# dylandreimerink/mimic

Measured on AMD Instinct MI355X. Metric: Mpkts/s (device-resident, one XDP program over 64-1500B batches), higher is better.
Workload: dtype u64; 1 GPU; cfg2: 1M x 64B xdp_md, 36-slot parse+hash DROP/PASS classifier, per-CPU array E=4 S=8; packets_per_gpu=1048576, vcpus_per_gpu=262144, schedule=interleaved, parallelism=dp1, batches_rotated=8, working_set_bytes=713031680, program_slots=36, engine=spread_own, batches_per_launch=8

## Files before the change

include/mimic_amd.h:

```cpp
#ifndef MIMIC_AMD_H
#define MIMIC_AMD_H

#if !defined(__HIPCC_RTC__)
#include <stddef.h>
#include <stdint.h>
#endif

#ifdef __cplusplus
extern "C" {
#endif

#define MIMIC_ABI_VERSION 4

#define MIMIC_EINVAL (-1)
#define MIMIC_ENOMEM (-2)
#define MIMIC_EDEVICE (-3)
#define MIMIC_ENOTSUP (-4)
#define MIMIC_ENOENT (-5)
#define MIMIC_EFAULT (-6)
#define MIMIC_ECANCELED (-7)
#define MIMIC_EDEADLINE (-8)

enum mimic_status {
    MIMIC_OK = 0,
// ... 79 lines not shown
    const uint32_t *pkt_len;
    const uint32_t *headroom;  uint32_t headroom_all;
    const uint32_t *tailroom;  uint32_t tailroom_all;
    const int32_t *ingress_ifindex; int32_t ingress_all;
    const int32_t *rx_queue_index;  int32_t rxq_all;
    const int32_t *egress_ifindex;  int32_t egress_all;
    const int32_t *cpu;
    uint64_t step_budget;
} mimic_xdp_batch;

typedef struct {
    uint64_t *r0;
    uint8_t *status;
    uint32_t *steps;
    int32_t *err_pc;
} mimic_xdp_results;

int mimic_abi_version(void);
const char *mimic_last_error(const mimic_vm *vm);

int mimic_vm_create(const mimic_vm_settings *settings, mimic_vm **out);
void mimic_vm_destroy(mimic_vm *vm);

int mimic_map_create(mimic_vm *vm, const mimic_map_spec *spec, uint32_t *map_id);
int mimic_map_update(mimic_vm *vm, uint32_t map_id, const void *key, const void *value, uint32_t flags, int32_t cpu);
int mimic_map_update_batch(mimic_vm *vm, uint32_t map_id, const void *keys, const void *values, uint32_t n,
                           uint32_t flags, int32_t cpu, int32_t *rc_out);
int mimic_map_lookup(mimic_vm *vm, uint32_t map_id, const void *key, int32_t cpu, uint32_t *addr_out);
int mimic_map_delete(mimic_vm *vm, uint32_t map_id, const void *key);
int mimic_map_keys(mimic_vm *vm, uint32_t map_id, void *out, size_t cap, uint32_t *n_out);
int mimic_map_entries(mimic_vm *vm, uint32_t map_id, void *keys_out, int32_t *slots_out, size_t cap_entries,
                      uint32_t *n_out);
int mimic_map_read_values(mimic_vm *vm, uint32_t map_id, int32_t cpu, void *out, size_t cap);
int mimic_map_reset(mimic_vm *vm, uint32_t map_id, void *hip_stream);
int mimic_map_read_values_range(mimic_vm *vm, uint32_t map_id, int32_t cpu_begin, int32_t cpu_end, void *out,
                                size_t cap);
int mimic_map_sum_u64(mimic_vm *vm, uint32_t map_id, int32_t cpu_begin, int32_t cpu_end, uint64_t *out, size_t cap);
int mimic_map_share(mimic_vm *vm, uint32_t map_id, mimic_vm *owner, uint32_t owner_map_id);
int mimic_map_addr(mimic_vm *vm, uint32_t map_id, uint32_t *addr_out);

int mimic_program_load(mimic_vm *vm, const char *name, const void *insns, uint32_t n_slots,
                       const mimic_reloc *relocs, uint32_t n_relocs, uint32_t *prog_id);
int mimic_program_addr(mimic_vm *vm, uint32_t prog_id, uint32_t *addr_out);

int mimic_mem_read(mimic_vm *vm, uint32_t addr, void *buf, uint32_t len);
int mimic_mem_load(mimic_vm *vm, uint32_t addr, int32_t size, uint64_t *out);
int mimic_stack_addr(mimic_vm *vm, uint32_t *addr_out);

int mimic_run_xdp(mimic_vm *vm, uint32_t prog_id, const mimic_xdp_batch *batch,
                  const mimic_xdp_results *results, void *hip_stream);
int mimic_run_xdp_many(mimic_vm *vm, uint32_t prog_id, const mimic_xdp_batch *batches,
                       const mimic_xdp_results *results, uint32_t k, void *hip_stream);
#define MIMIC_CTX_XDP 0
#define MIMIC_CTX_SKB 1
#define MIMIC_SKB_CUSTOM_SK 1u
#define MIMIC_SKB_CUSTOM_FLOWKEYS 2u
typedef struct {
    uint32_t flags;
    uint32_t sk_bound_dev_if, sk_family, sk_type, sk_protocol, sk_mark, sk_priority;
    uint32_t sk_src_port, sk_dst_port, sk_state;
    int32_t sk_rx_queue_mapping;
    uint8_t sk_ip_len[4];
    uint8_t sk_ip[4][16];
    uint16_t fk_nhoff, fk_thoff, fk_addr_proto;
    uint8_t fk_is_frag, fk_is_first_frag, fk_is_encap, fk_ip_proto;
    uint16_t fk_n_proto, fk_sport, fk_dport;
    uint32_t fk_flags, fk_flow_label;
} mimic_skb_custom;

typedef struct {
    uint32_t n;
    uint32_t schedule;
    uint8_t *pkt_data;
    const uint64_t *pkt_off;
    const uint32_t *pkt_len;
    uint32_t ifindex;
    int32_t pad;
    const int32_t *cpu;
    uint64_t step_budget;
    const mimic_skb_custom *custom;
    uint32_t *rooms_state;
} mimic_skb_batch;

int mimic_run_skb(mimic_vm *vm, uint32_t prog_id, const mimic_skb_batch *batch,
                  const mimic_xdp_results *results, void *hip_stream);
int mimic_skb_release(mimic_vm *vm);

typedef struct mimic_process mimic_process;
typedef struct {
    uint64_t r[11];
    int32_t pc;
    uint32_t prog_id;
    uint64_t steps;
    int32_t status;
    uint32_t exited;
} mimic_process_regs;
int mimic_process_new(mimic_vm *vm, uint32_t prog_id, const void *packet, uint32_t len, uint32_t headroom,
                      uint32_t tailroom, int32_t ingress_ifindex, int32_t rx_queue_index, int32_t egress_ifindex,
                      mimic_process **out);
int mimic_process_new_skb(mimic_vm *vm, uint32_t prog_id, const void *packet, uint32_t len, uint32_t ifindex,
                          mimic_process **out);
int mimic_process_new_skb_ctx(mimic_vm *vm, uint32_t prog_id, const void *packet, uint32_t len, uint32_t ifindex,
                              const mimic_skb_custom *custom, mimic_process **out);
int mimic_process_set_cpu(mimic_process *p, int32_t id);
int mimic_process_step(mimic_process *p, uint32_t n, mimic_process_regs *out);
int mimic_process_run(mimic_process *p, uint64_t budget, mimic_process_regs *out);
typedef struct mimic_ctx mimic_ctx;
int mimic_ctx_new(uint64_t timeout_ns, mimic_ctx **out);
void mimic_ctx_cancel(mimic_ctx *c);
int mimic_ctx_err(const mimic_ctx *c);
int mimic_ctx_pinned(const mimic_ctx *c);
void mimic_ctx_free(mimic_ctx *c);
int mimic_run_xdp_ctx(mimic_vm *vm, uint32_t prog_id, const mimic_xdp_batch *batch, const mimic_xdp_results *results,
                      void *hip_stream, mimic_ctx *ctx, mimic_ctx *const *ctx_per_packet);
int mimic_run_skb_ctx(mimic_vm *vm, uint32_t prog_id, const mimic_skb_batch *batch, const mimic_xdp_results *results,
                      void *hip_stream, mimic_ctx *ctx, mimic_ctx *const *ctx_per_packet);
int mimic_process_run_ctx(mimic_process *p, uint64_t budget, mimic_ctx *ctx, mimic_process_regs *out);
int mimic_process_run_many(mimic_process *const *ps, uint32_t n, const int32_t *cpus, mimic_ctx *const *ctxs,
                           mimic_process_regs *out);
void mimic_process_free_many(mimic_process *const *ps, uint32_t n);

int mimic_process_packet(mimic_process *p, void *buf, size_t cap);
void mimic_process_free(mimic_process *p);

int mimic_sync(mimic_vm *vm, void *hip_stream);
int mimic_last_steps(mimic_vm *vm, uint64_t *steps_out);

typedef struct {
    uint32_t n;
    uint32_t schedule;
    const uint8_t *pkt_data;
    const uint64_t *pkt_off;
    const uint32_t *pkt_len;
    uint32_t headroom_all, tailroom_all;
    int32_t ingress_all, rxq_all, egress_all;
    int32_t pad;
    const int32_t *cpu;
    uint64_t step_budget;
    uint8_t *pkt_out;
    uint64_t *r0;
    uint8_t *status;
} mimic_xdp_host_batch;
int mimic_run_xdp_host(mimic_vm *vm, uint32_t prog_id, const mimic_xdp_host_batch *hb, uint32_t chunks);
int mimic_run_xdp_host_ctx(mimic_vm *vm, uint32_t prog_id, const mimic_xdp_host_batch *hb, uint32_t chunks,
                           mimic_ctx *ctx);
int mimic_run_xdp_host_ctx_pp(mimic_vm *vm, uint32_t prog_id, const mimic_xdp_host_batch *hb, uint32_t chunks,
                              mimic_ctx *const *ctx_per_packet);
int mimic_host_register(void *p, size_t bytes);
int mimic_host_unregister(void *p);

int mimic_exec_mode(const mimic_vm *vm);
int mimic_set_spread(mimic_vm *vm, int32_t mode);
int mimic_last_exec(const mimic_vm *vm);
long mimic_jit_source_for(const void *const *progs, const uint32_t *n_slots, uint32_t n_progs, char *buf, size_t cap);
int mimic_jit_check(const char *src, char *log, size_t cap, size_t *code_size);
int mimic_jit_prebuild(const void *const *progs, const uint32_t *n_slots, uint32_t n_progs);
long mimic_jit_source_for_ctx(const void *const *progs, const uint32_t *n_slots, uint32_t n_progs, int32_t ctx_kind,
                              char *buf, size_t cap);
int mimic_jit_prebuild_ctx(const void *const *progs, const uint32_t *n_slots, uint32_t n_progs, int32_t ctx_kind);
long mimic_jit_source_vc(const void *const *progs, const uint32_t *n_slots, uint32_t n_progs, int32_t ctx_kind,
                         const uint32_t *vc_slots, uint32_t n_vc, char *buf, size_t cap);
long mimic_jit_source_spread(const void *const *progs, const uint32_t *n_slots, uint32_t n_progs, const uint32_t *pc,
                             uint32_t n_pc, const uint32_t *shapes, uint32_t n_shapes, uint32_t lds_rows,
                             int32_t *spread_out, char *buf, size_t cap);
int mimic_jit_cache_source(const char *src);
int mimic_jit_code(const char *src, void *code, size_t cap, size_t *code_size);

#ifdef __cplusplus
}
#endif
#endif
```

mimic_amd/_lib.py:

```python
from __future__ import annotations

import ctypes as C
import os

_HERE = os.path.dirname(os.path.abspath(__file__))
LIB_PATH = os.path.join(_HERE, os.path.basename(os.environ.get("MIMIC_LIB", "libmimic_amd.so")))

ABI_VERSION = 4

STATUS_NAMES = [
    "OK", "ERR_PC_OOB", "ERR_UNSUPPORTED_OP", "ERR_MEM_UNRESOLVED", "ERR_MEM_NOT_VMMEM",
    "ERR_MEM_BOUNDS", "ERR_MEM_NOT_DATASEC", "ERR_R10_WRITE", "ERR_HELPER_MAP_PTR",
    "ERR_HELPER_KEY", "ERR_HELPER_VALUE", "ERR_HELPER_MAP_OP", "ERR_HELPER_TAILCALL",
    "ERR_HELPER_UNIMPLEMENTED", "ERR_HELPER_CANT_EMULATE", "ERR_LDABS", "PANIC_DIV0",
    "PANIC_SHIFT", "PANIC_BADREG", "PANIC_CALLX", "PANIC_PC", "PANIC_HELPER_NEG",
    "ERR_STEP_LIMIT", "ERR_CALL_DEPTH", "ERR_ENGINE_HELPER", "ERR_NO_CPU", "ERR_CTX_ACCESS", "PANIC_SLICE",
    "ERR_CTX_LOAD", "ERR_CANCELED", "ERR_DEADLINE", "ERR_ENGINE_STATE",
]
STATUS = {n: i for i, n in enumerate(STATUS_NAMES)}
ECANCELED, EDEADLINE = -7, -8

SCHED_CHUNKED, SCHED_INTERLEAVED, SCHED_EXPLICIT = 0, 1, 2
MAP_F_DATASEC = 1


class VMSettings(C.Structure):
    _fields_ = [("vcpus", C.c_int32), ("stack_frame_size", C.c_int32), ("stack_frame_count", C.c_int32),
                ("max_tail_calls", C.c_int32), ("device", C.c_int32), ("vcpu_begin", C.c_int32),
                ("vcpu_count", C.c_int32), ("exec_mode", C.c_int32)]


class MapSpecC(C.Structure):
    _fields_ = [("name", C.c_char_p), ("type", C.c_uint32), ("key_size", C.c_uint32),
                ("value_size", C.c_uint32), ("max_entries", C.c_uint32), ("flags", C.c_uint32)]


class ProcessRegs(C.Structure):
    _fields_ = [("r", C.c_uint64 * 11), ("pc", C.c_int32), ("prog_id", C.c_uint32), ("steps", C.c_uint64),
                ("status", C.c_int32), ("exited", C.c_uint32)]


class Reloc(C.Structure):
    _fields_ = [("slot", C.c_uint32), ("map_id", C.c_uint32)]


class XDPBatch(C.Structure):
    _fields_ = [("n", C.c_uint32), ("schedule", C.c_uint32), ("pkt_data", C.c_void_p),
                ("pkt_off", C.c_void_p), ("pkt_len", C.c_void_p),
                ("headroom", C.c_void_p), ("headroom_all", C.c_uint32),
                ("tailroom", C.c_void_p), ("tailroom_all", C.c_uint32),
                ("ingress_ifindex", C.c_void_p), ("ingress_all", C.c_int32),
                ("rx_queue_index", C.c_void_p), ("rxq_all", C.c_int32),
                ("egress_ifindex", C.c_void_p), ("egress_all", C.c_int32),
                ("cpu", C.c_void_p), ("step_budget", C.c_uint64)]


class SKBBatch(C.Structure):
    _fields_ = [("n", C.c_uint32), ("schedule", C.c_uint32), ("pkt_data", C.c_void_p),
                ("pkt_off", C.c_void_p), ("pkt_len", C.c_void_p), ("ifindex", C.c_uint32), ("pad", C.c_int32),
                ("cpu", C.c_void_p), ("step_budget", C.c_uint64), ("custom", C.c_void_p), ("rooms_state", C.c_void_p)]


SKB_CUSTOM_SK, SKB_CUSTOM_FLOWKEYS = 1, 2
try:
    import numpy as _np

    SKB_CUSTOM_DTYPE = _np.dtype([
        ("flags", "<u4"), ("sk_bound_dev_if", "<u4"), ("sk_family", "<u4"), ("sk_type", "<u4"), ("sk_protocol", "<u4"),
        ("sk_mark", "<u4"), ("sk_priority", "<u4"), ("sk_src_port", "<u4"), ("sk_dst_port", "<u4"), ("sk_state", "<u4"),
        ("sk_rx_queue_mapping", "<i4"), ("sk_ip_len", "u1", (4,)), ("sk_ip", "u1", (4, 16)),
        ("fk_nhoff", "<u2"), ("fk_thoff", "<u2"), ("fk_addr_proto", "<u2"), ("fk_is_frag", "u1"),
        ("fk_is_first_frag", "u1"), ("fk_is_encap", "u1"), ("fk_ip_proto", "u1"), ("fk_n_proto", "<u2"),
        ("fk_sport", "<u2"), ("fk_dport", "<u2"), ("fk_flags", "<u4"), ("fk_flow_label", "<u4")])
    assert SKB_CUSTOM_DTYPE.itemsize == 136
except ImportError:
    SKB_CUSTOM_DTYPE = None


CTX_XDP, CTX_SKB = 0, 1


class XDPResults(C.Structure):
    _fields_ = [("r0", C.c_void_p), ("status", C.c_void_p), ("steps", C.c_void_p), ("err_pc", C.c_void_p)]


class XDPHostBatch(C.Structure):
    _fields_ = [("n", C.c_uint32), ("schedule", C.c_uint32), ("pkt_data", C.c_void_p),
                ("pkt_off", C.c_void_p), ("pkt_len", C.c_void_p),
                ("headroom_all", C.c_uint32), ("tailroom_all", C.c_uint32),
                ("ingress_all", C.c_int32), ("rxq_all", C.c_int32), ("egress_all", C.c_int32), ("pad", C.c_int32),
                ("cpu", C.c_void_p), ("step_budget", C.c_uint64), ("pkt_out", C.c_void_p),
                ("r0", C.c_void_p), ("status", C.c_void_p)]


EXPORTS = {
    "mimic_abi_version": (C.c_int, []),
    "mimic_last_error": (C.c_char_p, [C.c_void_p]),
    "mimic_vm_create": (C.c_int, [C.POINTER(VMSettings), C.POINTER(C.c_void_p)]),
    "mimic_vm_destroy": (None, [C.c_void_p]),
    "mimic_map_create": (C.c_int, [C.c_void_p, C.POINTER(MapSpecC), C.POINTER(C.c_uint32)]),
    "mimic_map_update": (C.c_int, [C.c_void_p, C.c_uint32, C.c_void_p, C.c_void_p, C.c_uint32, C.c_int32]),
    "mimic_map_lookup": (C.c_int, [C.c_void_p, C.c_uint32, C.c_void_p, C.c_int32, C.POINTER(C.c_uint32)]),
    "mimic_map_update_batch": (C.c_int, [C.c_void_p, C.c_uint32, C.c_void_p, C.c_void_p, C.c_uint32, C.c_uint32,
                                         C.c_int32, C.c_void_p]),
    "mimic_map_delete": (C.c_int, [C.c_void_p, C.c_uint32, C.c_void_p]),
    "mimic_exec_mode": (C.c_int, [C.c_void_p]),
    "mimic_set_spread": (C.c_int, [C.c_void_p, C.c_int32]),
    "mimic_process_new_skb_ctx": (C.c_int, [C.c_void_p, C.c_uint32, C.c_char_p, C.c_uint32, C.c_uint32, C.c_void_p,
                                            C.POINTER(C.c_void_p)]),
    "mimic_run_xdp_host": (C.c_int, [C.c_void_p, C.c_uint32, C.POINTER(XDPHostBatch), C.c_uint32]),
    "mimic_host_register": (C.c_int, [C.c_void_p, C.c_size_t]),
    "mimic_host_unregister": (C.c_int, [C.c_void_p]),
    "mimic_last_exec": (C.c_int, [C.c_void_p]),
    "mimic_jit_source_for": (C.c_long, [C.POINTER(C.c_void_p), C.POINTER(C.c_uint32), C.c_uint32, C.c_char_p,
                                         C.c_size_t]),
    "mimic_jit_check": (C.c_int, [C.c_char_p, C.c_char_p, C.c_size_t, C.POINTER(C.c_size_t)]),
    "mimic_jit_prebuild": (C.c_int, [C.POINTER(C.c_void_p), C.POINTER(C.c_uint32), C.c_uint32]),
    "mimic_map_keys": (C.c_int, [C.c_void_p, C.c_uint32, C.c_void_p, C.c_size_t, C.POINTER(C.c_uint32)]),
    "mimic_map_entries": (C.c_int, [C.c_void_p, C.c_uint32, C.c_void_p, C.c_void_p, C.c_size_t,
                                    C.POINTER(C.c_uint32)]),
    "mimic_map_read_values": (C.c_int, [C.c_void_p, C.c_uint32, C.c_int32, C.c_void_p, C.c_size_t]),
    "mimic_map_reset": (C.c_int, [C.c_void_p, C.c_uint32, C.c_void_p]),
    "mimic_map_read_values_range": (C.c_int, [C.c_void_p, C.c_uint32, C.c_int32, C.c_int32, C.c_void_p, C.c_size_t]),
    "mimic_map_sum_u64": (C.c_int, [C.c_void_p, C.c_uint32, C.c_int32, C.c_int32, C.c_void_p, C.c_size_t]),
    "mimic_map_addr": (C.c_int, [C.c_void_p, C.c_uint32, C.POINTER(C.c_uint32)]),
    "mimic_program_load": (C.c_int, [C.c_void_p, C.c_char_p, C.c_void_p, C.c_uint32, C.POINTER(Reloc),
                                     C.c_uint32, C.POINTER(C.c_uint32)]),
    "mimic_program_addr": (C.c_int, [C.c_void_p, C.c_uint32, C.POINTER(C.c_uint32)]),
    "mimic_mem_read": (C.c_int, [C.c_void_p, C.c_uint32, C.c_void_p, C.c_uint32]),
    "mimic_mem_load": (C.c_int, [C.c_void_p, C.c_uint32, C.c_int32, C.POINTER(C.c_uint64)]),
    "mimic_stack_addr": (C.c_int, [C.c_void_p, C.POINTER(C.c_uint32)]),
    "mimic_run_xdp": (C.c_int, [C.c_void_p, C.c_uint32, C.POINTER(XDPBatch), C.POINTER(XDPResults), C.c_void_p]),
    "mimic_run_xdp_many": (C.c_int, [C.c_void_p, C.c_uint32, C.POINTER(XDPBatch), C.POINTER(XDPResults), C.c_uint32,
                                     C.c_void_p]),
    "mimic_map_share": (C.c_int, [C.c_void_p, C.c_uint32, C.c_void_p, C.c_uint32]),
    "mimic_run_skb": (C.c_int, [C.c_void_p, C.c_uint32, C.POINTER(SKBBatch), C.POINTER(XDPResults), C.c_void_p]),
    "mimic_skb_release": (C.c_int, [C.c_void_p]),
    "mimic_jit_source_for_ctx": (C.c_long, [C.POINTER(C.c_void_p), C.POINTER(C.c_uint32), C.c_uint32, C.c_int32,
                                             C.c_char_p, C.c_size_t]),
    "mimic_jit_source_vc": (C.c_long, [C.POINTER(C.c_void_p), C.POINTER(C.c_uint32), C.c_uint32, C.c_int32,
                                       C.POINTER(C.c_uint32), C.c_uint32, C.c_char_p, C.c_size_t]),
    "mimic_jit_source_spread": (C.c_long, [C.POINTER(C.c_void_p), C.POINTER(C.c_uint32), C.c_uint32,
                                           C.POINTER(C.c_uint32), C.c_uint32, C.POINTER(C.c_uint32), C.c_uint32,
                                           C.c_uint32, C.POINTER(C.c_int32), C.c_char_p, C.c_size_t]),
    "mimic_jit_prebuild_ctx": (C.c_int, [C.POINTER(C.c_void_p), C.POINTER(C.c_uint32), C.c_uint32, C.c_int32]),
    "mimic_jit_cache_source": (C.c_int, [C.c_char_p]),
    "mimic_process_new": (C.c_int, [C.c_void_p, C.c_uint32, C.c_char_p, C.c_uint32, C.c_uint32, C.c_uint32,
                                    C.c_int32, C.c_int32, C.c_int32, C.POINTER(C.c_void_p)]),
    "mimic_process_new_skb": (C.c_int, [C.c_void_p, C.c_uint32, C.c_char_p, C.c_uint32, C.c_uint32, C.c_void_p]),
    "mimic_process_set_cpu": (C.c_int, [C.c_void_p, C.c_int32]),
    "mimic_process_step": (C.c_int, [C.c_void_p, C.c_uint32, C.c_void_p]),
    "mimic_process_run": (C.c_int, [C.c_void_p, C.c_uint64, C.c_void_p]),
    "mimic_process_packet": (C.c_int, [C.c_void_p, C.c_void_p, C.c_size_t]),
    "mimic_process_free": (None, [C.c_void_p]),
    "mimic_jit_code": (C.c_int, [C.c_char_p, C.c_void_p, C.c_size_t, C.POINTER(C.c_size_t)]),
    "mimic_sync": (C.c_int, [C.c_void_p, C.c_void_p]),
    "mimic_ctx_new": (C.c_int, [C.c_uint64, C.POINTER(C.c_void_p)]),
    "mimic_ctx_cancel": (None, [C.c_void_p]),
    "mimic_ctx_err": (C.c_int, [C.c_void_p]),
    "mimic_ctx_pinned": (C.c_int, [C.c_void_p]),
    "mimic_ctx_free": (None, [C.c_void_p]),
    "mimic_run_xdp_ctx": (C.c_int, [C.c_void_p, C.c_uint32, C.POINTER(XDPBatch), C.POINTER(XDPResults), C.c_void_p,
                                    C.c_void_p, C.c_void_p]),
    "mimic_run_skb_ctx": (C.c_int, [C.c_void_p, C.c_uint32, C.POINTER(SKBBatch), C.POINTER(XDPResults), C.c_void_p,
                                    C.c_void_p, C.c_void_p]),
    "mimic_process_run_ctx": (C.c_int, [C.c_void_p, C.c_uint64, C.c_void_p, C.POINTER(ProcessRegs)]),
    "mimic_process_run_many": (C.c_int, [C.c_void_p, C.c_uint32, C.c_void_p, C.c_void_p, C.POINTER(ProcessRegs)]),
    "mimic_process_free_many": (None, [C.c_void_p, C.c_uint32]),
    "mimic_run_xdp_host_ctx": (C.c_int, [C.c_void_p, C.c_uint32, C.POINTER(XDPHostBatch), C.c_uint32, C.c_void_p]),
    "mimic_run_xdp_host_ctx_pp": (C.c_int, [C.c_void_p, C.c_uint32, C.POINTER(XDPHostBatch), C.c_uint32, C.c_void_p]),
    "mimic_last_steps": (C.c_int, [C.c_void_p, C.POINTER(C.c_uint64)]),
}

_lib = None


def load() -> C.CDLL:
    global _lib
    if _lib is not None:
        return _lib
    if not os.path.exists(LIB_PATH):
        raise ImportError(f"{LIB_PATH} is missing: run __graft_entry__.build() (hipcc --offload-arch=gfx950)")
    try:
        import torch
    except ImportError:
        pass
    lib = C.CDLL(LIB_PATH)
    for name, (res, args) in EXPORTS.items():
        fn = getattr(lib, name)
        fn.restype = res
        fn.argtypes = args
    if lib.mimic_abi_version() != ABI_VERSION:
        raise ImportError("libmimic_amd.so ABI version mismatch")
    _lib = lib
    return lib
```

mimic_amd/csrc/engine.cpp:

```cpp
#include <hip/hip_runtime.h>

#include <algorithm>
#include <atomic>
#include <cstdarg>
#include <cstdlib>
#include <cstdio>
#include <cstring>
#include <map>
#include <string>
#include <chrono>
#include <condition_variable>
#include <memory>
#include <mutex>
#include <thread>
#include <unordered_map>
#include <vector>

#include "../../include/mimic_amd.h"
#include "blkcache.h"
#include "layout.h"
#include "hashmap.h"
#include "jit.h"
#include "skb.h"

extern "C" int mimic_launch_xdp(const KParams *kp, const KParams *d_kp, hipStream_t st);
extern "C" int mimic_launch_xdp_resume(const KParams *kp, hipStream_t st);

extern "C" int mimic_launch_hash_rebuild(uint8_t *arena, const DMap *m, uint32_t force, hipStream_t st);
extern "C" int mimic_launch_hash_reset(uint8_t *arena, const DMap *m, hipStream_t st);
extern "C" int mimic_launch_hash_normalize(uint8_t *arena, const DMap *m, hipStream_t st);
extern "C" int mimic_launch_hash_compact(uint8_t *arena, const DMap *m, hipStream_t st);
extern "C" int mimic_launch_spread_reduce(const void *part, uint32_t nblocks, uint32_t lanes, uint32_t roww, uint32_t n,
                                          uint8_t *dst, uint64_t stride, hipStream_t st);
extern "C" int mimic_launch_sum_u64(const uint8_t *base, uint64_t stride, uint32_t nvals, uint32_t cpus, uint64_t *out,
                                    hipStream_t st);
extern "C" int mimic_launch_skb_gather(const uint8_t *const *mem, uint32_t n, uint64_t *drv, uint64_t *prefix,
                                       mimic_skb_custom *cust, const uint8_t *has_cust, hipStream_t st);
extern "C" int mimic_launch_skb_prep(const uint8_t *pkt_data, const uint64_t *pkt_off, const uint32_t *pkt_len,
                                     uint32_t n, uint64_t *rec, uint32_t rec_q, uint64_t *prefix, uint64_t *state,
                                     uint64_t init_base, uint32_t use_init, uint32_t *rooms_state, hipStream_t st);

namespace {

#define MIRROR_PAGE 8192u
#define MIRROR_BULK 32u
struct HashMirror {
    bool valid = false, dirty = false;
    std::vector<uint64_t> rec;
    std::vector<int32_t> ring;
    HashCtl ctl{};
    std::vector<uint8_t> rec_pg, ring_pg;
    bool all = true;
    uint32_t faults = 0;
};

struct ShareGroup {
    struct Member {
        void *vm;
        uint32_t map;
        uint8_t *arena;
    };
    std::vector<Member> members;
    bool owner_gone = false;
};

struct HostMap {
    std::string name;
    uint32_t type, family, key_size, value_size, max_entries, datasec;
    uint32_t obj_addr;
    uint32_t backing_addr;
    uint32_t addr_period;
    uint32_t ncpu;
    uint64_t dev_off;
    uint64_t dev_stride;
    uint64_t keys_dev_off, ht_dev_off;
    uint32_t keys_addr, ht_cap, rec_q, nlocks, fl_cap;
    mutable bool may_tomb = false;
    mutable bool pop_dirty = false;
    std::shared_ptr<HashMirror> mir;
    mutable std::shared_ptr<ShareGroup> share;
    mutable bool chunk = false;
};

bool vc_row_ok(uint32_t family, uint32_t max_entries, uint32_t value_size) {
    const uint64_t rb = (uint64_t)max_entries * value_size;
    return family == FAM_PERCPU_ARRAY && rb > 0 && rb <= MIMIC_VC_MAX_ROW && (rb & 7) == 0;
}

struct HostProg {
    std::string name;
    std::vector<DInsn> ins;
    uint32_t addr;
};

struct HipFence : BlkFence {
    hipEvent_t ev = nullptr;
    hipStream_t st = nullptr;
    void wait() override {
        if (hipEventSynchronize(ev) != hipSuccess) {
            (void)hipGetLastError();
            hipStreamSynchronize(st);
        }
    }
    ~HipFence() override {
        if (ev) hipEventDestroy(ev);
    }
};

}

struct mimic_vm {
    mimic_vm_settings s;
    std::string err;
    hipStream_t stream = nullptr;
    uint32_t next_addr = MIMIC_MEM_START;
    std::vector<HostMap> maps;
    std::vector<HostProg> progs;
    std::vector<Seg> segs;
    uint8_t *arena = nullptr;
    uint64_t arena_size = 0, arena_cap = 0;
    DInsn *d_insns = nullptr;
    DProg *d_progs = nullptr;
    Seg *d_segs = nullptr;
    DMap *d_maps = nullptr;
    bool tables_dirty = true;
    bool prog_deletes = false;
    bool prog_updates = false;
    uint8_t *priv = nullptr;
    uint64_t priv_bytes = 0;
    uint32_t priv_lanes = 0;
    uint32_t *d_sched_start = nullptr, *d_sched_pkts = nullptr;
    uint64_t sched_cap_start = 0, sched_cap_pkts = 0;
    uint64_t *d_lane_steps = nullptr;
    uint32_t lane_steps_cap = 0;
    DeferRec *d_defer = nullptr;
    uint32_t *d_defer_any = nullptr;
    uint32_t defer_cap = 0, defer_epoch = 0;
    uint32_t last_lanes = 0;
    hipStream_t last_stream = nullptr;
    int exec_mode = MIMIC_EXEC_JIT;
    std::vector<DInsn> h_all;
    std::vector<DProg> h_dp;
    hipFunction_t jit_fn[2] = {nullptr, nullptr};
    JitInfo jit_info[2]{};
    hipFunction_t jit_fn_cx[2] = {nullptr, nullptr};
    JitInfo jit_info_cx[2]{};
    int64_t proc_jit_after = 32;
    uint64_t proc_runs = 0;
    int proc_jit = 0;
    hipFunction_t jit_fn_proc = nullptr;
    JitInfo jit_info_proc{};
    int spread_state = 0;
    hipFunction_t jit_fn_spread = nullptr;
    JitInfo jit_info_spread{};
    int spread_own_state = 0;
    hipFunction_t jit_fn_spread_own = nullptr;
    JitInfo jit_info_spread_own{};
    uint32_t spread_own_rows = 0;
    uint32_t *d_spread_bad = nullptr;
    void *d_spread_part = nullptr;
    uint64_t spread_part_cap = 0;
    bool spread_used = false;
    bool comb_used = false;
    struct PendWrite {
        uint64_t off;
        uint32_t n, at;
    };
    std::vector<PendWrite> pend;
    std::vector<uint8_t> pend_data;
    std::unordered_map<uint64_t, size_t> pend_at;
    bool host_dirty = false;
    int spread_mode = -1;
    bool spread_lds = false;
    int last_exec = 0;
    static constexpr int KP_SLOTS = 64;
    KParams *d_kp = nullptr, *h_kp = nullptr;
    hipEvent_t kp_ev[KP_SLOTS] = {};
    bool kp_used[KP_SLOTS] = {};
    int kp_next = 0, kp_last = -1;
    hipStream_t kp_last_stream = nullptr;
    static constexpr int NB = 4;
    struct Slot {
        uint8_t *buf = nullptr;
        uint64_t *off = nullptr;
        uint32_t *len = nullptr;
        uint64_t *r0 = nullptr;
        uint8_t *st = nullptr;
        size_t cap_bytes = 0, cap_n = 0;
        hipEvent_t e_in = nullptr, e_k = nullptr, e_out = nullptr;
        bool used = false;
    } slot[NB];
    hipStream_t s_h2d = nullptr, s_h2d2 = nullptr, s_d2h = nullptr;
    hipStream_t kp_copy_stream = nullptr;
    hipEvent_t kp_copy_ev = nullptr;
    hipStream_t s_kp = nullptr;
    hipEvent_t kp_side_ev = nullptr;
    SkbRec *d_skb_rec = nullptr;
    uint64_t *d_skb_drv = nullptr;
    uint64_t *d_skb_prefix = nullptr, *d_skb_state = nullptr;
    size_t skb_cap = 0;
    uint8_t *d_many = nullptr;
    size_t many_cap = 0;
    BlkCache blk{256ull << 20};
    std::recursive_mutex run_mu;
    SeqClock seq;
    uint32_t proc_gen = 0;
    bool skb_leaked = false;
    hipStream_t skb_stream = nullptr;
    bool skb_release_pending = false;
    hipEvent_t skb_ev = nullptr;
    const uint32_t **d_cancel_pp = nullptr;
    size_t cancel_pp_cap = 0;
    hipStream_t cancel_pp_stream = nullptr;
};

struct mimic_ctx {
    uint32_t *word = nullptr;
    uint32_t *dword = nullptr;
    bool pinned = false;
    std::mutex mu;
    std::condition_variable cv;
    bool closing = false;
    std::thread timer;
    std::vector<hipEvent_t> uses;
};
static void ctx_set(mimic_ctx *c, uint32_t v) {
    uint32_t z = 0;
    __atomic_compare_exchange_n(c->word, &z, v, false, __ATOMIC_SEQ_CST, __ATOMIC_SEQ_CST);
}
static uint32_t ctx_get(const mimic_ctx *c) { return __atomic_load_n(c->word, __ATOMIC_SEQ_CST); }


static int fail(mimic_vm *vm, int code, const char *fmt, ...) {
    if (vm) {
        char buf[512];
        va_list ap;
        va_start(ap, fmt);
        vsnprintf(buf, sizeof buf, fmt, ap);
        va_end(ap);
        vm->err = buf;
    }
    return code;
}

#define HIP_OK(vm, call)                                                                        \
    do {                                                                                        \
        hipError_t e_ = (call);                                                                 \
        if (e_ != hipSuccess) return fail((vm), MIMIC_EDEVICE, "%s: %s", #call, hipGetErrorString(e_)); \
    } while (0)

static int skb_settle(mimic_vm *vm);

static int kp_slot(mimic_vm *vm, const KParams &kp, hipStream_t st, const KParams **out) {
    if (!vm->d_kp) {
        HIP_OK(vm, hipMalloc(&vm->d_kp, sizeof(KParams) * mimic_vm::KP_SLOTS));
        HIP_OK(vm, hipHostMalloc(&vm->h_kp, sizeof(KParams) * mimic_vm::KP_SLOTS));
        for (auto &e : vm->kp_ev) HIP_OK(vm, hipEventCreateWithFlags(&e, hipEventDisableTiming));
    }
    int slot = vm->kp_last;
    if (slot < 0 || st != vm->kp_last_stream || memcmp(&vm->h_kp[slot], &kp, sizeof kp) != 0) {
        slot = vm->kp_next;
        vm->kp_next = (slot + 1) % mimic_vm::KP_SLOTS;
        if (vm->kp_used[slot]) HIP_OK(vm, hipEventSynchronize(vm->kp_ev[slot]));
        vm->h_kp[slot] = kp;
        if (vm->kp_copy_stream) {
            HIP_OK(vm, hipMemcpyAsync(vm->d_kp + slot, vm->h_kp + slot, sizeof kp, hipMemcpyHostToDevice, vm->kp_copy_stream));
            HIP_OK(vm, hipEventRecord(vm->kp_copy_ev, vm->kp_copy_stream));
            HIP_OK(vm, hipStreamWaitEvent(st, vm->kp_copy_ev, 0));
        } else {
            if (!vm->s_kp) {
                HIP_OK(vm, hipStreamCreateWithFlags(&vm->s_kp, hipStreamNonBlocking));
                HIP_OK(vm, hipEventCreateWithFlags(&vm->kp_side_ev, hipEventDisableTiming));
            }
            HIP_OK(vm, hipMemcpyAsync(vm->d_kp + slot, vm->h_kp + slot, sizeof kp, hipMemcpyHostToDevice, vm->s_kp));
            HIP_OK(vm, hipEventRecord(vm->kp_side_ev, vm->s_kp));
            HIP_OK(vm, hipStreamWaitEvent(st, vm->kp_side_ev, 0));
        }
        vm->kp_last = slot;
        vm->kp_last_stream = st;
    }
    *out = vm->d_kp + slot;
    return slot;
}

static uint32_t stack_size(const mimic_vm *vm) {
    return (uint32_t)(vm->s.stack_frame_size * vm->s.stack_frame_count);
}

static uint32_t add_entry(mimic_vm *vm, uint32_t size) {
    uint32_t a = vm->next_addr;
    vm->next_addr = a + size + 1;
    return a;
}

static int arena_reserve(mimic_vm *vm, uint64_t bytes, uint64_t *off) {
    uint64_t need = (vm->arena_size + 255) & ~255ull;
    uint64_t end = need + bytes;
    if (end > vm->arena_cap) {
        uint64_t cap = std::max<uint64_t>(end, vm->arena_cap * 2);
        cap = std::max<uint64_t>(cap, 1 << 20);
        uint8_t *n = nullptr;
        HIP_OK(vm, hipMalloc(&n, cap));
        HIP_OK(vm, hipMemset(n, 0, cap));
        if (vm->arena) {
            HIP_OK(vm, hipMemcpy(n, vm->arena, vm->arena_size, hipMemcpyDeviceToDevice));
            HIP_OK(vm, hipFree(vm->arena));
        }
        vm->arena = n;
        vm->arena_cap = cap;
    }
    *off = need;
    vm->arena_size = end;
    return 0;
}

static int helper_class(int32_t n) {
    static const int ce[] = {4, 14, 15, 16, 17, 22, 24, 27, 35, 36, 42, 45, 46, 47, 55, 56, 67, 69, 80,
                             112, 113, 114, 115, 119, 120, 122, 123, 128, 129, 141, 148, 151};
    static const int em[] = {1, 2, 3, 5, 7, 8, 9, 12, 25, 38, 65, 87, 88, 89, 125, 160};
    for (int v : ce) if (v == n) return 2;
    for (int v : em) if (v == n) return 1;
    return 0;
}

static uint32_t predecode(const DInsn &x, int64_t i, int64_t n) {
    const uint32_t op = x.w & 0xff, dst = (x.w >> 8) & 0xf, src = (x.w >> 12) & 0xf;
    const int64_t off = (int16_t)(x.w >> 16);
// ... 1565 lines not shown
    kp.priv = step ? step->priv : vm->priv;
    kp.priv_xdp_q = xdp_q;
    kp.priv_frame_q = frame_q;
    kp.priv_key_q = key_q;
    kp.budget = step ? step->budget : (b->step_budget ? b->step_budget : MIMIC_DEFAULT_BUDGET);
    kp.step = step ? step->state : nullptr;
    kp.step_gen = step ? step->gen : 0u;
    if (step) {
        kp.step_img = step->img;
        kp.step_dst = step->img_dst;
        kp.step_img_n = step->img_n;
        kp.step_ins_n = (uint32_t)std::min<size_t>(vm->h_all.size(), 2048);
    }
    kp.n = b->n;
    kp.sched = b->schedule;
    kp.pkt_data = b->pkt_data;
    kp.pkt_off = b->pkt_off;
    kp.pkt_len = b->pkt_len;
    kp.headroom_arr = b->headroom;
    kp.tailroom_arr = b->tailroom;
    kp.ingress_arr = b->ingress_ifindex;
    kp.rxq_arr = b->rx_queue_index;
    kp.egress_arr = b->egress_ifindex;
    kp.headroom = b->headroom_all;
    kp.tailroom = b->tailroom_all;
    kp.ingress = b->ingress_all;
    kp.rxq = b->rxq_all;
    kp.egress = b->egress_all;
    kp.r0 = res->r0;
    kp.status = res->status;
    kp.steps = res->steps;
    kp.err_pc = res->err_pc;
    kp.lane_steps = vm->d_lane_steps;
    if (cx && cx->all) {
        kp.cancel = cx->all->dword;
        kp.cancel_any = 1;
    } else if (cx && cx->dev_pp && b->n) {
        kp.cancel_pp = cx->dev_pp;
        kp.cancel_any = 1;
    } else if (cx && cx->per_packet && b->n) {
        std::vector<const uint32_t *> w(b->n);
        bool any = false;
        for (uint32_t i = 0; i < b->n; i++) {
            w[i] = cx->per_packet[i] ? cx->per_packet[i]->dword : nullptr;
            any |= w[i] != nullptr;
        }
        if (any) {
            if (vm->cancel_pp_stream) hipStreamSynchronize(vm->cancel_pp_stream);
            hipStreamSynchronize(st);
            vm->cancel_pp_stream = st;
            if (b->n > vm->cancel_pp_cap) {
                hipFree(vm->d_cancel_pp);
                vm->d_cancel_pp = nullptr;
                HIP_OK(vm, hipMalloc(&vm->d_cancel_pp, (size_t)b->n * sizeof(void *)));
                vm->cancel_pp_cap = b->n;
            }
            HIP_OK(vm, hipMemcpy(vm->d_cancel_pp, w.data(), (size_t)b->n * sizeof(void *), hipMemcpyHostToDevice));
            kp.cancel_pp = vm->d_cancel_pp;
            kp.cancel_any = 1;
        }
    }
    switch (b->schedule) {
    case MIMIC_SCHED_CHUNKED:
        kp.per_lane = lanes ? (uint32_t)(((uint64_t)b->n + lanes - 1) / lanes) : 0;
        break;
    case MIMIC_SCHED_INTERLEAVED:
        kp.sched_shift = lanes ? (uint32_t)(first_index % lanes) : 0;
        kp.per_lane = lanes ? (uint32_t)(((uint64_t)b->n + kp.sched_shift + lanes - 1) / lanes) : 0;
        break;
    case MIMIC_SCHED_EXPLICIT: {
        if (!b->cpu && b->n) return fail(vm, MIMIC_EINVAL, "explicit schedule needs cpu[]");
        std::vector<uint32_t> start(lanes + 1, 0), pk(b->n);
        std::vector<uint32_t> lane_of(b->n);
        for (uint32_t i = 0; i < b->n; i++) {
            const int32_t id = b->cpu[i];
            int64_t c = (int64_t)id - vm->s.vcpu_begin;
            if (id == -1) c = cpu_lanes;
            else if (id == vm->s.vcpus) c = cpu_lanes + 1;
            else if (c < 0 || c >= (int64_t)cpu_lanes)
                return fail(vm, MIMIC_EINVAL, "packet %u: cpu %d not on this engine", i, id);
            lane_of[i] = (uint32_t)c;
            start[c + 1]++;
        }
        uint32_t mx = 0;
        for (uint32_t c = 0; c < lanes; c++) {
            mx = std::max(mx, start[c + 1]);
            start[c + 1] += start[c];
        }
        std::vector<uint32_t> fill(start.begin(), start.end() - 1);
        for (uint32_t i = 0; i < b->n; i++) pk[fill[lane_of[i]]++] = i;
        hipStreamSynchronize(st);
        if (start.size() > vm->sched_cap_start) {
            hipFree(vm->d_sched_start);
            vm->d_sched_start = nullptr;
            HIP_OK(vm, hipMalloc(&vm->d_sched_start, start.size() * 4));
            vm->sched_cap_start = start.size();
        }
        if (pk.size() > vm->sched_cap_pkts || !vm->d_sched_pkts) {
            hipFree(vm->d_sched_pkts);
            vm->d_sched_pkts = nullptr;
            HIP_OK(vm, hipMalloc(&vm->d_sched_pkts, std::max<size_t>(pk.size(), 1) * 4));
            vm->sched_cap_pkts = std::max<size_t>(pk.size(), 1);
        }
        HIP_OK(vm, hipMemcpy(vm->d_sched_start, start.data(), start.size() * 4, hipMemcpyHostToDevice));
        if (!pk.empty()) HIP_OK(vm, hipMemcpy(vm->d_sched_pkts, pk.data(), pk.size() * 4, hipMemcpyHostToDevice));
        kp.sched_start = vm->d_sched_start;
        kp.sched_pkts = vm->d_sched_pkts;
        kp.per_lane = mx;
        break;
    }
    default:
        return fail(vm, MIMIC_EINVAL, "unknown schedule %u", b->schedule);
    }
    bool jit = vm->exec_mode == MIMIC_EXEC_JIT && (!step || proc_jit);
    if (jit && !proc_jit && !vm->jit_fn[ctx]) {
        std::string log;
        const std::vector<std::pair<uint32_t, uint32_t>> vc = vc_slots_of(vm);
        if (mimic_jit_compile(vm->s.device, mimic_jit_source(vm->h_dp, vm->h_all, ctx, &vm->jit_info[ctx], &vc),
                              &vm->jit_fn[ctx], &log))
            return fail(vm, MIMIC_EDEVICE, "JIT build failed: %s", log.c_str());
        const JitInfo &j0 = vm->jit_info[ctx];
        int ls0 = 0;
        if (j0.early_loads && j0.cold_inline &&
            hipFuncGetAttribute(&ls0, HIP_FUNC_ATTRIBUTE_LOCAL_SIZE_BYTES, vm->jit_fn[ctx]) == hipSuccess && ls0 > 0) {
            JitInfo j1;
            hipFunction_t f1 = nullptr;
            int ls1 = 0;
            if (!mimic_jit_compile(vm->s.device, mimic_jit_source(vm->h_dp, vm->h_all, ctx, &j1, &vc, true), &f1, &log) &&
                hipFuncGetAttribute(&ls1, HIP_FUNC_ATTRIBUTE_LOCAL_SIZE_BYTES, f1) == hipSuccess && ls1 < ls0) {
                vm->jit_fn[ctx] = f1;
                vm->jit_info[ctx] = j1;
            }
        }
    }
    if (jit && !proc_jit) {
        const uint64_t bound = mimic_jit_step_bound(vm->jit_info[ctx], kp.max_tail_calls);
        if (bound && kp.budget < bound) jit = false;
    }
    bool spread = false, own = false;
    if (jit && !step && !skb && b->n > 0 && (b->schedule == MIMIC_SCHED_CHUNKED || b->schedule == MIMIC_SCHED_INTERLEAVED)) {
        const char *sv = getenv("MIMIC_SPREAD");
        const int knob = vm->spread_mode >= 0 ? vm->spread_mode : sv && *sv ? atoi(sv) : -1;
        const char *ov = getenv("MIMIC_SPREAD_OWN");
        const bool own_pref = !(ov && ov[0] == '0');
        if (knob != 0 && own_pref && kp.per_lane >= 2 && kp.per_lane <= 256) {
            rc = spread_build_own(vm);
            if (rc) return rc;
            const uint32_t P = kp.per_lane, cl = chip_lanes(vm);
            const char *qv = getenv("MIMIC_SPREAD_OWN_Q");
            uint32_t q = qv && *qv ? (uint32_t)atoi(qv) : (uint32_t)std::max<uint64_t>(1, ((uint64_t)b->n + cl - 1) / cl);
            q = std::max<uint32_t>(1, std::min(q, P));
            while (q > 1 && (P % q || 256u * q / P > vm->spread_own_rows)) q--;
            kp.own_q = q;
            own = vm->spread_own_state > 0 && P % q == 0 && 256u * q / P <= vm->spread_own_rows && 256u * q / P >= 1u &&
                  mimic_jit_step_bound(vm->jit_info_spread_own, kp.max_tail_calls) <= kp.budget;
            spread = own;
        }
        if (!own && (knob == 1 || (knob != 0 && (uint64_t)b->n >= 8ull * cpu_lanes))) {
            rc = spread_build(vm);
            if (rc) return rc;
            spread = vm->spread_state > 0 && mimic_jit_step_bound(vm->jit_info_spread, kp.max_tail_calls) <= kp.budget;
            if (knob != 1 && !vm->spread_lds && cpu_lanes > 16384) spread = false;
        }
    }
    const bool cxk = jit && kp.cancel_any;
    if (cxk) {
        spread = own = false;
        if (!vm->jit_fn_cx[ctx]) {
            const std::vector<std::pair<uint32_t, uint32_t>> vc = vc_slots_of(vm);
            std::string log;
            if (mimic_jit_compile(vm->s.device,
                                  mimic_jit_source(vm->h_dp, vm->h_all, ctx, &vm->jit_info_cx[ctx], &vc,
                                                   !vm->jit_info[ctx].early_loads, nullptr, true),
                                  &vm->jit_fn_cx[ctx], &log))
                return fail(vm, MIMIC_EDEVICE, "JIT build failed: %s", log.c_str());
        }
    }
    const JitInfo &ji = proc_jit ? vm->jit_info_proc : own ? vm->jit_info_spread_own : spread ? vm->jit_info_spread
                        : cxk ? vm->jit_info_cx[ctx] : vm->jit_info[ctx];
    hipFunction_t jfn = proc_jit ? vm->jit_fn_proc : own ? vm->jit_fn_spread_own : spread ? vm->jit_fn_spread
                        : cxk ? vm->jit_fn_cx[ctx] : vm->jit_fn[ctx];
    if (proc_jit && (!jfn || !ji.proc_ok)) return fail(vm, MIMIC_EDEVICE, "process: no single-process JIT kernel (engine)");
    uint32_t run_lanes = lanes;
    if (spread) {
        const uint32_t orows = own ? 256u / (kp.per_lane / kp.own_q) : 1u;
        const uint32_t blocks = own ? (cpu_lanes + orows - 1) / orows
                                    : (uint32_t)(((uint64_t)b->n + spread_ppb() - 1) / spread_ppb());
        run_lanes = blocks * 256u;
        rc = priv_ensure(vm, q_per_lane, run_lanes, st);
        if (rc) return rc;
        if (run_lanes > vm->lane_steps_cap) {
            hipStreamSynchronize(st);
            hipFree(vm->d_lane_steps);
            vm->d_lane_steps = nullptr;
            HIP_OK(vm, hipMalloc(&vm->d_lane_steps, (uint64_t)run_lanes * sizeof(uint64_t)));
            vm->lane_steps_cap = run_lanes;
        }
        if (!vm->d_spread_bad) {
            HIP_OK(vm, hipMalloc(&vm->d_spread_bad, 64));
            HIP_OK(vm, hipMemset(vm->d_spread_bad, 0, 64));
        }
        kp.lanes = run_lanes;
        kp.priv = vm->priv;
        kp.priv_lanes = vm->priv_lanes;
        kp.lane_steps = vm->d_lane_steps;
        kp.spread_bad = vm->d_spread_bad;
        vm->spread_used = true;
        kp.spread_part = nullptr;
        if (!own && ji.spread_rows && ji.spread_rows == cpu_lanes && ji.spread_n &&
            (uint64_t)cpu_lanes * ji.spread_roww <= spread_ppb()) {
            const uint64_t need = (uint64_t)blocks * ji.spread_rows * ji.spread_roww * ji.spread_n;
            if (need > vm->spread_part_cap) {
                HIP_OK(vm, hipStreamSynchronize(st));
                hipFree(vm->d_spread_part);
                vm->d_spread_part = nullptr;
                HIP_OK(vm, hipMalloc(&vm->d_spread_part, need));
                vm->spread_part_cap = need;
            }
            kp.spread_part = vm->d_spread_part;
        }
    }
    if (skb && step && step->skb_rec) {
        kp.ctx_kind = CTX_SKB;
        kp.skb_ifindex = skb->ifindex;
        kp.skb_rec = step->skb_rec;
        kp.skb_prefix = step->skb_prefix;
        kp.skb_base = step->skb_base;
        kp.skb_custom = step->skb_custom;
    } else if (skb && skb->pre_drv) {
        rc = skb_ensure(vm, b->n, st);
        if (rc) return rc;
        kp.ctx_kind = CTX_SKB;
        kp.skb_ifindex = skb->ifindex;
        kp.skb_rec = vm->d_skb_rec;
        kp.skb_drv = skb->pre_drv;
        kp.skb_prefix = skb->pre_prefix;
        kp.skb_base = skb->pre_base;
        kp.skb_custom = skb->custom;
        vm->skb_stream = st;
    } else if (skb) {
        rc = skb_prepare(vm, b, st, nullptr, skb->rooms_state);
        if (rc) return rc;
        kp.skb_rooms_state = skb->rooms_state;
        kp.ctx_kind = CTX_SKB;
        kp.skb_ifindex = skb->ifindex;
        kp.skb_rec = vm->d_skb_rec;
        kp.skb_drv = vm->d_skb_drv;
        kp.skb_prefix = vm->d_skb_prefix;
        kp.skb_base = vm->d_skb_state + 1;
        kp.skb_custom = skb->custom;
    }
    kp.hash_pop_only = vm->prog_deletes ? 0u : 1u;
    kp.hash_ro = (vm->prog_deletes || vm->prog_updates) ? 0u : 1u;
    for (auto &m : vm->maps) {
        if (!is_hash(m)) continue;
        if (m.share) {
            if ((rc = share_check(vm, m))) return rc;
            for (auto &mb : m.share->members) {
                mimic_vm *o = (mimic_vm *)mb.vm;
                if (o != vm && o->host_dirty && (rc = flush_host(o))) return fail(vm, rc, "shared map: %s", o->err.c_str());
            }
            share_stale(m);
        }
        const DMap dm = to_dmap(m);
        if (vm->prog_deletes && m.pop_dirty) {
            if (mimic_launch_hash_normalize(vm->arena, &dm, st))
                return fail(vm, MIMIC_EDEVICE, "launch: %s", hipGetErrorString(hipGetLastError()));
            m.pop_dirty = false;
        }
        if (!vm->prog_deletes) m.pop_dirty = true;
        if (vm->prog_deletes) m.may_tomb = true;
        if (m.mir && (vm->prog_updates || vm->prog_deletes || m.may_tomb)) m.mir->valid = false;
        if (!m.may_tomb) continue;
        if (mimic_launch_hash_rebuild(vm->arena, &dm, 0, st))
            return fail(vm, MIMIC_EDEVICE, "launch: %s", hipGetErrorString(hipGetLastError()));
    }
    vm->last_exec = jit ? (own ? MIMIC_EXEC_SPREAD_OWN : spread ? MIMIC_EXEC_SPREAD : MIMIC_EXEC_JIT) : MIMIC_EXEC_INTERP;
    if (jit && ji.defer) {
        if (lanes > vm->defer_cap || !vm->d_defer_any) {
            hipStreamSynchronize(st);
            hipFree(vm->d_defer);
            vm->d_defer = nullptr;
            HIP_OK(vm, hipMalloc(&vm->d_defer, (uint64_t)plan * sizeof(DeferRec)));
            HIP_OK(vm, hipMemset(vm->d_defer, 0, (uint64_t)plan * sizeof(DeferRec)));
            vm->defer_cap = plan;
            if (!vm->d_defer_any) {
                HIP_OK(vm, hipMalloc(&vm->d_defer_any, 64));
                HIP_OK(vm, hipMemset(vm->d_defer_any, 0, 64));
            }
        }
        if (++vm->defer_epoch == 0) vm->defer_epoch = 1;
        kp.defer = vm->d_defer;
        kp.defer_any = vm->d_defer_any;
        kp.defer_epoch = vm->defer_epoch;
    }
    if (jit && ji.hash_combine) vm->comb_used = true;
    if (mr) {
        mr->used = jit && own && !ji.defer && mr->k >= 1 && mr->k <= MIMIC_MANY_MAX;
        if (mr->used) {
            kp.many_n = mr->k;
            for (uint32_t q = 0; q < mr->k; q++)
                kp.many[q] = BatchRef{mr->b[q].pkt_data, mr->b[q].pkt_off, mr->b[q].pkt_len, mr->r[q].r0, mr->r[q].status,
                                      mr->r[q].steps, mr->r[q].err_pc, 0};
        }
    }
    if (jit) {
        if (mimic_jit_launch(jfn, &kp, st))
            return fail(vm, MIMIC_EDEVICE, "launch: %s", hipGetErrorString(hipGetLastError()));
        if (ji.defer && mimic_launch_xdp_resume(&kp, st))
            return fail(vm, MIMIC_EDEVICE, "launch: %s", hipGetErrorString(hipGetLastError()));
    } else if (step) {
        if (mimic_launch_xdp(&kp, nullptr, st))
            return fail(vm, MIMIC_EDEVICE, "launch: %s", hipGetErrorString(hipGetLastError()));
    } else {
        const KParams *dkp = nullptr;
        const int slot = kp_slot(vm, kp, st, &dkp);
        if (slot < 0) return slot;
        if (mimic_launch_xdp(&kp, dkp, st))
            return fail(vm, MIMIC_EDEVICE, "launch: %s", hipGetErrorString(hipGetLastError()));
        HIP_OK(vm, hipEventRecord(vm->kp_ev[slot], st));
        vm->kp_used[slot] = true;
    }
    if (jit && ji.hash_chunk) {
        for (const HostMap &m : vm->maps) {
            if (!m.chunk) continue;
            const DMap dm = to_dmap(m);
            if (mimic_launch_hash_compact(vm->arena, &dm, st))
                return fail(vm, MIMIC_EDEVICE, "launch: %s", hipGetErrorString(hipGetLastError()));
        }
    }
    if (jit && kp.spread_part) {
        const DMap dm = to_dmap(vm->maps[ji.spread_map]);
        if (mimic_launch_spread_reduce(kp.spread_part, kp.lanes / 256u, kp.cpu_lanes, ji.spread_roww, ji.spread_n,
                                       vm->arena + dm.dev_off + (uint64_t)kp.vcpu_begin * dm.dev_stride, dm.dev_stride, st))
            return fail(vm, MIMIC_EDEVICE, "launch: %s", hipGetErrorString(hipGetLastError()));
    }
    if (kp.cancel_any) {
        auto mark = [&](mimic_ctx *c) -> int {
            std::lock_guard<std::mutex> lk(c->mu);
            std::vector<hipEvent_t> keep;
            for (hipEvent_t e : c->uses) {
                if (hipEventQuery(e) == hipSuccess) hipEventDestroy(e);
                else keep.push_back(e);
            }
            c->uses.swap(keep);
            hipEvent_t ev = nullptr;
            HIP_OK(vm, hipEventCreateWithFlags(&ev, hipEventDisableTiming));
            HIP_OK(vm, hipEventRecord(ev, st));
            c->uses.push_back(ev);
            return 0;
        };
        if (cx->all) {
            if ((rc = mark(cx->all))) return rc;
        } else {
            std::vector<mimic_ctx *> u;
            for (uint32_t i = 0; i < b->n; i++)
                if (cx->per_packet[i]) u.push_back(cx->per_packet[i]);
            std::sort(u.begin(), u.end());
            u.erase(std::unique(u.begin(), u.end()), u.end());
            for (mimic_ctx *c : u)
                if ((rc = mark(c))) return rc;
        }
    }
    vm->last_lanes = run_lanes;
    vm->last_stream = st;
    return 0;
}

}

namespace {
constexpr size_t PD_LEN = 8, PD_SKB = 64;
constexpr size_t PD_PKT = (PD_SKB + sizeof(SkbRec) + 24 + sizeof(mimic_skb_custom) + 63) & ~(size_t)63;
constexpr size_t PH_RES = (sizeof(StepState) + 63) & ~(size_t)63;
constexpr size_t PH_R0 = PH_RES, PH_ST = PH_RES + 8, PH_STEPS = PH_RES + 16, PH_EPC = PH_RES + 20, PH_WORD = PH_RES + 24;
constexpr size_t PH_IMG = PH_RES + 64;
}

struct mimic_process {
    mimic_vm *vm = nullptr;
    uint32_t prog = 0;
    uint32_t H = 0, T = 0, len = 0;
    int32_t ingress = 0, rxq = 0, egress = 0;
    uint8_t *d_pkt = nullptr;
    uint8_t *d_skbmem = nullptr;
    StepState *hs = nullptr;
    StepState *hs_dev = nullptr;
    uint8_t *hres = nullptr, *hres_dev = nullptr;
    uint64_t priv_bytes = 0;
    StepState h;
    int32_t cpu = -1;
    uint32_t gen = 0;
    uint32_t static_next = 0;
    uint8_t *arena = nullptr;
    bool skb = false;
    bool skb_custom = false;
    uint32_t ifindex = 0;
    Blk mem;
    Blk priv;
    uint64_t last_seq = 0;
    bool uploaded = false;
    size_t img_n = 0;
};

static bool proc_alloc(mimic_vm *vm, size_t n, bool host, Blk *out) {
    if (vm->blk.take(n, host, out)) return true;
    out->cls = BlkCache::size_class(n);
    if (hipMalloc(&out->dev, out->cls) != hipSuccess) {
        (void)hipGetLastError();
        *out = Blk{};
        return false;
    }
    if (host) {
        void *h = nullptr, *d = nullptr;
        if (hipHostMalloc(&h, out->cls, hipHostMallocMapped | hipHostMallocCoherent) != hipSuccess) {
            (void)hipGetLastError();
            hipFree(out->dev);
            *out = Blk{};
            return false;
        }
        if (hipHostGetDevicePointer(&d, h, 0) != hipSuccess) {
            (void)hipGetLastError();
            d = h;
        }
        out->host = (uint8_t *)h;
        out->hdev = (uint8_t *)d;
    }
    return true;
}
// ... 389 lines not shown
                 o_steps = o_st + al(n), o_epc = o_steps + al((size_t)n * 4), total = o_epc + al((size_t)n * 4);
    if (total > vm->many_cap) {
        HIP_OK(vm, hipStreamSynchronize(st));
        hipFree(vm->d_many);
        vm->d_many = nullptr;
        HIP_OK(vm, hipMalloc(&vm->d_many, total));
        vm->many_cap = total;
    }
    uint8_t *D = vm->d_many;
    std::vector<uint8_t> host(o_drv);
    std::vector<int32_t> cpu(n);
    std::vector<uint8_t> hc(n);
    for (uint32_t i = 0; i < n; i++) {
        const mimic_process *p = ps[i];
        const uint64_t off = (uint64_t)(p->d_pkt - lo);
        const uint32_t len = p->len;
        const uint8_t *m = p->d_skbmem;
        memcpy(host.data() + o_off + 8 * (size_t)i, &off, 8);
        memcpy(host.data() + o_len + 4 * (size_t)i, &len, 4);
        memcpy(host.data() + o_mem + 8 * (size_t)i, &m, 8);
        cpu[i] = p->cpu;
        hc[i] = p->skb_custom ? 1 : 0;
    }
    HIP_OK(vm, hipMemcpyAsync(D, host.data(), o_drv, hipMemcpyHostToDevice, st));
    HIP_OK(vm, hipMemsetAsync(D + o_base, 0, 8, st));
    if (any_cust) HIP_OK(vm, hipMemcpyAsync(D + o_hc, hc.data(), n, hipMemcpyHostToDevice, st));
    if (mimic_launch_skb_gather((const uint8_t *const *)(D + o_mem), n, (uint64_t *)(D + o_drv), (uint64_t *)(D + o_pre),
                                any_cust ? (mimic_skb_custom *)(D + o_cu) : nullptr, D + o_hc, st))
        return fail(vm, MIMIC_EDEVICE, "gather: %s", hipGetErrorString(hipGetLastError()));
    mimic_xdp_batch b{};
    b.n = n;
    b.schedule = MIMIC_SCHED_EXPLICIT;
    b.pkt_data = lo;
    b.pkt_off = (const uint64_t *)(D + o_off);
    b.pkt_len = (const uint32_t *)(D + o_len);
    b.cpu = cpu.data();
    b.step_budget = ~0ull >> 1;
    mimic_xdp_results r{};
    r.r0 = (uint64_t *)(D + o_r0);
    r.status = D + o_st;
    r.steps = (uint32_t *)(D + o_steps);
    r.err_pc = (int32_t *)(D + o_epc);
    SkbRun skr{ifindex, any_cust ? (const mimic_skb_custom *)(D + o_cu) : nullptr};
    skr.pre_drv = (const uint64_t *)(D + o_drv);
    skr.pre_prefix = (const uint64_t *)(D + o_pre);
    skr.pre_base = (const uint64_t *)(D + o_base);
    CtxRun cx{nullptr, ctxs};
    int rc = run_xdp_impl(vm, prog, &b, &r, st, 0, &skr, nullptr, ctxs ? &cx : nullptr);
    if (rc) return rc;
    std::vector<uint8_t> res(total - o_r0);
    HIP_OK(vm, hipMemcpyAsync(res.data(), D + o_r0, res.size(), hipMemcpyDeviceToHost, st));
    HIP_OK(vm, proc_sync(vm));
    for (uint32_t i = 0; i < n; i++) {
        mimic_process *p = ps[i];
        uint64_t r0;
        uint32_t steps;
        int32_t epc;
        memcpy(&r0, res.data() + 8 * (size_t)i, 8);
        memcpy(&steps, res.data() + (o_steps - o_r0) + 4 * (size_t)i, 4);
        memcpy(&epc, res.data() + (o_epc - o_r0) + 4 * (size_t)i, 4);
        const uint8_t status = res[(o_st - o_r0) + i];
        memset(p->h.r, 0, sizeof p->h.r);
        p->h.r[0] = r0;
        p->h.pc = status ? epc : -1;
        p->h.prog = prog;
        p->h.steps = steps;
        p->h.status = status;
        p->h.started = 1;
        p->h.finished = 1;
        p->static_next = vm->next_addr;
        p->arena = vm->arena;
        process_regs(p, out ? out + i : nullptr);
    }
    return 0;
}

int mimic_process_packet(mimic_process *p, void *buf, size_t cap) {
    if (!p || !buf) return MIMIC_EINVAL;
    const uint64_t M = (uint64_t)p->H + p->len + p->T;
    if (cap < M) return fail(p->vm, MIMIC_EINVAL, "buffer too small");
    mimic_vm *vm = p->vm;
    std::lock_guard<std::recursive_mutex> lk(vm->run_mu);
    if (!p->uploaded) {
        memcpy(buf, p->mem.host + PH_IMG + PD_PKT, M);
        return (int)M;
    }
    hipSetDevice(vm->s.device);
    const hipError_t e = hipMemcpyAsync(buf, p->d_pkt, M, hipMemcpyDeviceToHost, vm->stream);
    proc_enq(p);
    const hipError_t es = proc_sync(vm);
    if (e != hipSuccess || es != hipSuccess) return fail(vm, MIMIC_EDEVICE, "packet: %s", hipGetErrorString(e != hipSuccess ? e : es));
    return (int)M;
}

void mimic_process_free(mimic_process *p) {
    if (!p) return;
    hipSetDevice(p->vm->s.device);
    process_release(p, proc_fence(p->vm, p->last_seq));
    delete p;
}

void mimic_process_free_many(mimic_process *const *ps, uint32_t n) {
    mimic_vm *last = nullptr;
    std::shared_ptr<BlkFence> f;
    bool have = false;
    for (uint32_t i = 0; i < n; i++) {
        mimic_process *p = ps[i];
        if (!p) continue;
        if (p->vm != last) {
            last = p->vm;
            hipSetDevice(last->s.device);
            have = false;
            f.reset();
        }
        const bool busy = !last->seq.idle(p->last_seq);
        if (busy && !have) {
            f = proc_fence(last, p->last_seq);
            have = true;
        }
        process_release(p, busy ? f : nullptr);
        delete p;
    }
}

int mimic_sync(mimic_vm *vm, void *hip_stream) {
    if (!vm) return MIMIC_EINVAL;
    hipSetDevice(vm->s.device);
    hipStream_t st = hip_stream ? (hipStream_t)hip_stream : vm->stream;
    HIP_OK(vm, hipStreamSynchronize(st));
    return spread_check(vm);
}

int mimic_last_steps(mimic_vm *vm, uint64_t *steps_out) {
    if (!vm || !steps_out) return MIMIC_EINVAL;
    hipSetDevice(vm->s.device);
    *steps_out = 0;
    if (!vm->last_lanes) return 0;
    if (vm->last_stream) HIP_OK(vm, hipStreamSynchronize(vm->last_stream));
    std::vector<uint64_t> h(vm->last_lanes);
    HIP_OK(vm, hipMemcpy(h.data(), vm->d_lane_steps, h.size() * 8, hipMemcpyDeviceToHost));
    uint64_t t = 0;
    for (uint64_t v : h) t += v;
    *steps_out = t;
    return spread_check(vm);
}

int mimic_exec_mode(const mimic_vm *vm) { return vm ? vm->exec_mode : MIMIC_EINVAL; }
int mimic_set_spread(mimic_vm *vm, int32_t mode) {
    if (!vm || mode < -1 || mode > 1) return MIMIC_EINVAL;
    vm->spread_mode = mode;
    return 0;
}
int mimic_last_exec(const mimic_vm *vm) { return vm ? vm->last_exec : MIMIC_EINVAL; }

long mimic_jit_source_for(const void *const *progs, const uint32_t *n_slots, uint32_t n_progs, char *buf, size_t cap) {
    return mimic_jit_source_for_ctx(progs, n_slots, n_progs, MIMIC_CTX_XDP, buf, cap);
}

long mimic_jit_source_for_ctx(const void *const *progs, const uint32_t *n_slots, uint32_t n_progs, int32_t ctx_kind,
                              char *buf, size_t cap) {
    return mimic_jit_source_vc(progs, n_slots, n_progs, ctx_kind, nullptr, 0, buf, cap);
}

long mimic_jit_source_vc(const void *const *progs, const uint32_t *n_slots, uint32_t n_progs, int32_t ctx_kind,
                         const uint32_t *vc_slots, uint32_t n_vc, char *buf, size_t cap) {
    const bool proc = (ctx_kind & 0x100) != 0, no_early_loads = (ctx_kind & 0x200) != 0;
    ctx_kind &= 0xff;
    if (ctx_kind != MIMIC_CTX_XDP && ctx_kind != MIMIC_CTX_SKB) return MIMIC_EINVAL;
    if (proc && ctx_kind != MIMIC_CTX_XDP) return MIMIC_EINVAL;
    std::vector<HostProg> hp(n_progs);
    for (uint32_t p = 0; p < n_progs; p++) {
        std::string err;
        if (decode_program((const uint8_t *)progs[p], n_slots[p], hp[p].ins, &err)) return MIMIC_EINVAL;
    }
    std::vector<DInsn> all;
    std::vector<DProg> dp;
    build_host_tables(hp, all, dp);
    std::vector<std::pair<uint32_t, uint32_t>> vc;
    for (uint32_t q = 0; q < n_vc; q++) {
        const uint32_t p = vc_slots[3 * q], s = vc_slots[3 * q + 1], rb = vc_slots[3 * q + 2];
        if (p >= dp.size() || s >= dp[p].n) return MIMIC_EINVAL;
        vc.push_back({dp[p].base + s, rb});
    }
    const std::string src = mimic_jit_source(dp, all, (uint32_t)ctx_kind, nullptr, &vc, no_early_loads, nullptr, false, proc);
    if (buf && cap > src.size()) memcpy(buf, src.c_str(), src.size() + 1);
    return (long)src.size();
}

long mimic_jit_source_spread(const void *const *progs, const uint32_t *n_slots, uint32_t n_progs, const uint32_t *pc,
                             uint32_t n_pc, const uint32_t *shapes, uint32_t n_shapes, uint32_t lds_rows,
                             int32_t *spread_out, char *buf, size_t cap) {
    std::vector<HostProg> hp(n_progs);
    for (uint32_t p = 0; p < n_progs; p++) {
        std::string err;
        if (decode_program((const uint8_t *)progs[p], n_slots[p], hp[p].ins, &err)) return MIMIC_EINVAL;
    }
    std::vector<DInsn> all;
    std::vector<DProg> dp;
    build_host_tables(hp, all, dp);
    SpreadReq req;
    for (uint32_t q = 0; q < n_pc; q++) {
        const uint32_t p = pc[3 * q], sl = pc[3 * q + 1];
        if (p >= dp.size() || sl >= dp[p].n) return MIMIC_EINVAL;
        req.slot_map[dp[p].base + sl] = pc[3 * q + 2];
    }
    for (uint32_t q = 0; q < n_shapes; q++) req.shape[shapes[3 * q]] = {shapes[3 * q + 1], shapes[3 * q + 2]};
    req.lds_rows = lds_rows & 0x7fffffffu;
    req.own = (lds_rows >> 31) != 0;
    JitInfo info{};
    const std::string src = mimic_jit_source(dp, all, MIMIC_CTX_XDP, &info, nullptr, false, &req);
    if (spread_out) *spread_out = info.spread ? 1 : 0;
    if (buf && cap > src.size()) memcpy(buf, src.c_str(), src.size() + 1);
    return (long)src.size();
}

int mimic_jit_prebuild(const void *const *progs, const uint32_t *n_slots, uint32_t n_progs) {
    return mimic_jit_prebuild_ctx(progs, n_slots, n_progs, MIMIC_CTX_XDP);
}

int mimic_jit_prebuild_ctx(const void *const *progs, const uint32_t *n_slots, uint32_t n_progs, int32_t ctx_kind) {
    if (ctx_kind != MIMIC_CTX_XDP && ctx_kind != MIMIC_CTX_SKB) return MIMIC_EINVAL;
    std::vector<HostProg> hp(n_progs);
    for (uint32_t p = 0; p < n_progs; p++) {
        std::string err;
        if (decode_program((const uint8_t *)progs[p], n_slots[p], hp[p].ins, &err)) return MIMIC_EINVAL;
    }
    std::vector<DInsn> all;
    std::vector<DProg> dp;
    build_host_tables(hp, all, dp);
    std::string log;
    return mimic_jit_prebuild_source(mimic_jit_source(dp, all, (uint32_t)ctx_kind, nullptr), &log) ? MIMIC_EINVAL : 0;
}

int mimic_jit_check(const char *src, char *log, size_t cap, size_t *code_size) {
    std::string lg;
    const int rc = mimic_jit_check_source(src ? src : "", &lg, code_size);
    if (log && cap) {
        const size_t n = std::min(cap - 1, lg.size());
        memcpy(log, lg.data(), n);
        log[n] = 0;
    }
    return rc ? MIMIC_EINVAL : 0;
}

int mimic_jit_cache_source(const char *src) {
    if (!src) return MIMIC_EINVAL;
    std::string log;
    return mimic_jit_prebuild_source(src, &log) ? MIMIC_EINVAL : 0;
}

int mimic_jit_code(const char *src, void *code, size_t cap, size_t *code_size) {
    if (!src || !code_size) return MIMIC_EINVAL;
    std::vector<char> co;
    std::string log;
    if (mimic_jit_build_code(src, co, &log)) return MIMIC_EINVAL;
    *code_size = co.size();
    if (code && cap >= co.size()) memcpy(code, co.data(), co.size());
    return 0;
}

int mimic_host_register(void *p, size_t bytes) {
    if (!p || !bytes) return MIMIC_EINVAL;
    return hipHostRegister(p, bytes, hipHostRegisterDefault) == hipSuccess ? 0 : MIMIC_EDEVICE;
}

int mimic_host_unregister(void *p) {
    if (!p) return MIMIC_EINVAL;
    return hipHostUnregister(p) == hipSuccess ? 0 : MIMIC_EDEVICE;
}

struct HostWindow {
    uint64_t lo = ~0ull, hi = 0;
    bool ascending = true;
};
__attribute__((target("avx2"))) static HostWindow host_window(const mimic_xdp_host_batch *hb, uint32_t a, uint32_t m,
                                                             uint64_t room) {
    const uint64_t *off = hb->pkt_off + a;
    const uint32_t *len = hb->pkt_len + a;
    uint64_t lo = ~0ull, hi = 0, bad = 0;
    for (uint32_t i = 0; i < m; i++) {
        const uint64_t o = off[i], e = o + len[i] + room;
        lo = o < lo ? o : lo;
        hi = e > hi ? e : hi;
    }
    for (uint32_t i = 1; i < m; i++) bad |= (uint64_t)(off[i] < off[i - 1] + len[i - 1] + room);
    HostWindow w;
    w.lo = lo;
    w.hi = hi;
    w.ascending = bad == 0;
    return w;
}

static int slot_reserve(mimic_vm *vm, mimic_vm::Slot &sl, size_t bytes, size_t n) {
    if (bytes <= sl.cap_bytes && n <= sl.cap_n) return 0;
    if (sl.used) HIP_OK(vm, hipEventSynchronize(sl.e_out));
    if (bytes > sl.cap_bytes) {
        hipFree(sl.buf);
        sl.buf = nullptr;
        sl.cap_bytes = std::max(bytes, sl.cap_bytes + sl.cap_bytes / 2);
        HIP_OK(vm, hipMalloc(&sl.buf, sl.cap_bytes));
    }
    if (n > sl.cap_n) {
        for (void *q : {(void *)sl.off, (void *)sl.len, (void *)sl.r0, (void *)sl.st}) hipFree(q);
        sl.off = nullptr;
        sl.len = nullptr;
        sl.r0 = nullptr;
        sl.st = nullptr;
        sl.cap_n = std::max(n, sl.cap_n + sl.cap_n / 2);
        HIP_OK(vm, hipMalloc(&sl.off, 8 * sl.cap_n));
        HIP_OK(vm, hipMalloc(&sl.len, 4 * sl.cap_n));
        HIP_OK(vm, hipMalloc(&sl.r0, 8 * sl.cap_n));
        HIP_OK(vm, hipMalloc(&sl.st, sl.cap_n));
    }
    return 0;
}

static int run_xdp_host_impl(mimic_vm *vm, uint32_t prog_id, const mimic_xdp_host_batch *hb, uint32_t chunks,
                             mimic_ctx *ctx, mimic_ctx *const *ctx_per_packet);
int mimic_run_xdp_host(mimic_vm *vm, uint32_t prog_id, const mimic_xdp_host_batch *hb, uint32_t chunks) {
    return run_xdp_host_impl(vm, prog_id, hb, chunks, nullptr, nullptr);
}
int mimic_run_xdp_host_ctx(mimic_vm *vm, uint32_t prog_id, const mimic_xdp_host_batch *hb, uint32_t chunks,
                           mimic_ctx *ctx) {
    return run_xdp_host_impl(vm, prog_id, hb, chunks, ctx, nullptr);
}
int mimic_run_xdp_host_ctx_pp(mimic_vm *vm, uint32_t prog_id, const mimic_xdp_host_batch *hb, uint32_t chunks,
                              mimic_ctx *const *ctx_per_packet) {
    return run_xdp_host_impl(vm, prog_id, hb, chunks, nullptr, ctx_per_packet);
}
static int run_xdp_host_impl(mimic_vm *vm, uint32_t prog_id, const mimic_xdp_host_batch *hb, uint32_t chunks,
                             mimic_ctx *ctx, mimic_ctx *const *ctx_pp) {
    if (!vm || !hb) return MIMIC_EINVAL;
    const uint32_t n = hb->n;
    if (n == 0) return 0;
    if (!hb->pkt_data || !hb->pkt_off || !hb->pkt_len || !hb->r0 || !hb->status)
        return fail(vm, MIMIC_EINVAL, "missing host arrays");
    hipSetDevice(vm->s.device);
    const uint64_t room = (uint64_t)hb->headroom_all + hb->tailroom_all;
    if (chunks == 0) {
        const uint64_t first = hb->pkt_off[0], last = hb->pkt_off[n - 1] + hb->pkt_len[n - 1] + room;
        const uint64_t bytes = last > first ? last - first : (uint64_t)n * (room + 1500);
        chunks = (uint32_t)std::min<uint64_t>(64, std::max<uint64_t>(2, bytes >> 24));
    }
    chunks = std::max<uint32_t>(1, std::min(chunks, n));
    if (hb->pkt_out && !host_window(hb, 0, n, room).ascending)
        return fail(vm, MIMIC_EINVAL, "pkt_out needs ascending, non-overlapping packets");
    std::vector<int32_t> cpu_chunked;
    uint32_t sched = hb->schedule;
    const int32_t *cpu = hb->cpu;
    if (sched == MIMIC_SCHED_CHUNKED) {
        const uint32_t lanes = (uint32_t)vm->s.vcpu_count;
        const uint64_t per = ((uint64_t)n + lanes - 1) / lanes;
        cpu_chunked.resize(n);
        for (uint32_t i = 0; i < n; i++) cpu_chunked[i] = vm->s.vcpu_begin + (int32_t)(i / per);
        cpu = cpu_chunked.data();
        sched = MIMIC_SCHED_EXPLICIT;
    }
    if (sched == MIMIC_SCHED_EXPLICIT && !cpu) return fail(vm, MIMIC_EINVAL, "explicit schedule needs cpu[]");
    bool pp_any = false;
    if (ctx_pp) {
        std::vector<const uint32_t *> w(n);
        for (uint32_t i = 0; i < n; i++) {
            w[i] = ctx_pp[i] ? ctx_pp[i]->dword : nullptr;
            pp_any |= w[i] != nullptr;
// ... 92 lines not shown
```

mimic_amd/csrc/jit.cpp:

```cpp
#include <hip/hip_runtime.h>
#include <hip/hiprtc.h>

#include <algorithm>
#include <cinttypes>
#include <cstdarg>
#include <cstdio>
#include <cstring>
#include <cstdlib>
#include <unistd.h>
#include <map>
#include <mutex>
#include <set>
#include <string>
#include <vector>

#include "../../include/mimic_amd.h"
#include "layout.h"
#include "jit.h"

namespace {

#include "jit_headers.inc"

struct Emitter {
    std::string s;
    void line(const char *fmt, ...) __attribute__((format(printf, 2, 3))) {
        char buf[1024];
        va_list ap;
        va_start(ap, fmt);
        vsnprintf(buf, sizeof buf, fmt, ap);
        va_end(ap);
        s += buf;
        s += '\n';
    }
};

struct ProgView {
    uint32_t id, n, base;
    const DInsn *ins;
};

uint32_t insn_op(const DInsn &x) { return x.w & 0xff; }
uint32_t insn_dst(const DInsn &x) { return (x.w >> 8) & 0xf; }
uint32_t insn_src(const DInsn &x) { return (x.w >> 12) & 0xf; }
int32_t insn_off(const DInsn &x) { return (int16_t)(x.w >> 16); }

bool ends_block(const DInsn &x) {
    switch (AUX_H(x.aux)) {
    case H_ERR: case H_JA: case H_JCC: case H_EXIT: case H_CALL_LOCAL: return true;
    case H_CALL: return (uint32_t)x.k == 12;
    default: return false;
    }
}

int64_t jump_target(const DInsn &x, int64_t i) {
    return insn_op(x) == 0x85 ? i + (int64_t)(int32_t)(uint32_t)x.k : i + insn_off(x) + 1;
}

bool off(const char *name) { const char *v = getenv(name); return !(v && v[0] == '0'); }
bool on(const char *name) { const char *v = getenv(name); return v && v[0] == '1'; }
int num(const char *name, int dflt) { const char *v = getenv(name); return v ? atoi(v) : dflt; }

class Gen {
  public:
    Gen(const std::vector<ProgView> &progs, uint32_t ctx_kind) : P(progs), ctx(ctx_kind) {
        fast_paths = off("MIMIC_JIT_FAST");
        prefetch = off("MIMIC_JIT_PREFETCH");
        xpf_knob = on("MIMIC_JIT_XPF");
        lpf_knob = on("MIMIC_JIT_LPF");
        lds_stack_q = (uint32_t)std::min(32, std::max(0, num("MIMIC_JIT_LDSSTK", 16)));
        dispatch_knob = off("MIMIC_JIT_DISPATCH");
        vc_knob = off("MIMIC_JIT_VC");
        forward = off("MIMIC_JIT_FWD");
        ntres = off("MIMIC_JIT_NTRES");
        combine_knob = off("MIMIC_JIT_COMBINE");
        hchunk_knob = num("MIMIC_JIT_HCHUNK", 32);
        skb_fields = off("MIMIC_JIT_SKBFIELD");
        skb_lds_knob = off("MIMIC_JIT_SKBLDS");
        sm_lds_knob = off("MIMIC_JIT_SMLDS");
        inc_knob = off("MIMIC_JIT_INC");
        hash_fast = off("MIMIC_JIT_HASH");
        ret_dispatch = getenv("MIMIC_JIT_RETDISPATCH") ? on("MIMIC_JIT_RETDISPATCH") : !fast_paths;
        tail_inline = off("MIMIC_JIT_TAIL");
        census = on("MIMIC_JIT_CENSUS");
        elide = off("MIMIC_JIT_ELIDE");
        window = off("MIMIC_JIT_WINDOW");
        speculate = num("MIMIC_JIT_SPEC", 8);
        waves = num("MIMIC_JIT_WAVES", 0);
        const char *cm = getenv("MIMIC_JIT_COLD");
        cold_mode = !cm ? 0 : !strcmp(cm, "call") ? 1 : !strcmp(cm, "inline") ? 2 : !strcmp(cm, "defer") ? 3 : 0;
        for (auto &p : P)
            for (uint32_t i = 0; i < p.n; i++) {
                const DInsn &x = p.ins[i];
                if (AUX_H(x.aux) == H_CALL && (uint32_t)x.k == 12) any_tail = true;
                if (AUX_H(x.aux) == H_CALL_LOCAL) any_local = true;
            }
        all_leaders = any_tail && any_local;
        bool back = false;
        uint32_t mx = 0;
        for (auto &p : P) {
            mx = std::max(mx, p.n);
            for (uint32_t i = 0; i < p.n; i++) {
                const DInsn &x = p.ins[i];
                const uint32_t h = AUX_H(x.aux);
                if ((h == H_JA || h == H_JCC) && (x.aux & AUX_JT_OK) && jump_target(x, i) <= (int64_t)i) back = true;
            }
        }
        careful_copies = back || any_local;
        max_n = mx;
    }

    bool careful_copies = true;
    uint32_t max_n = 0;
    bool fast_paths = true;
    int cold_mode = 0;
    bool skb_fields = true;
    bool skb_lds_knob = true;
    bool skb_lds = false;
    bool inc_knob = true;
    bool sm_lds_knob = true;
    static constexpr uint32_t kSrecQ = 21;
    bool hash_fast = true;
    bool tail_inline = true;
    bool ret_dispatch = false;
    bool census = false;
    bool elide = true;
    bool window = true;
    int speculate = 8;
    bool combine_knob = true;
    bool hash_combine = false;
    int hchunk_knob = 32;
    bool hash_chunk = false;
    bool ntres = true;
    bool forward = true;
    int waves = 0;
    bool prefetch = true;
    bool xpf_knob = false;
    bool lpf_knob = false;
    bool lpf_on = false;
    bool lds_stack_on = false;
    static constexpr uint32_t kLpfD = 4;
    bool vc_knob = true;
    uint32_t lds_stack_q = 16;
    bool vc_on = false;
    const SpreadReq *spread_req = nullptr;
    bool ctx_check = false;
    bool proc = false;
    bool spread_on = false;
    bool spread_own = false;
    uint32_t spread_map = 0, spread_n = 0, spread_row = 0;
    std::map<uint32_t, uint32_t> vc_ok;
    uint32_t vc_slot = 0;
    uint32_t vc_rb = 0;
    bool vc_lds = false;
    struct Xpf {
        bool on = false;
        uint32_t prog = 0, hp = 0, base = 0, words = 0;
        int64_t off = 0;
    } xpf;
    bool cold_inline = true;
    bool defer_mode = false;
    std::vector<std::vector<uint16_t>> live;
    uint32_t cold_sites = 0;
    static constexpr uint32_t kColdInlineSites = 48;
    bool has_tail() const { return any_tail; }
    bool has_early_loads() const { return !spec_use.empty(); }
    bool dispatch_knob = true;
    bool dispatch_on() const { return dispatch_knob && any_tail; }
    std::string nonempty_cases() const {
        std::string c;
        for (auto &q : P)
            if (q.n) c += "    case " + std::to_string(q.id) + "u:";
        return c;
    }
    uint32_t ctx = CTX_XDP;

    std::string source() {
        uint32_t sites = 0;
        for (auto &p : P)
            for (uint32_t i = 0; i < p.n; i++) {
                const uint32_t h = AUX_H(p.ins[i].aux);
                if (h == H_LDX || h == H_ST || h == H_STX || h == H_CALL || h == H_LDABS || h == H_SLOW) sites++;
            }
        if (careful_copies) sites *= 2;
        cold_sites = sites;
        cold_inline = !proc && (cold_mode == 2 || (cold_mode == 0 && sites <= kColdInlineSites));
        defer_mode = !cold_inline && (cold_mode == 3 || cold_mode == 0) && !census && fast_paths && !proc;
        if (fast_paths) analyze_live();
        analyze_vc();
        if (forward)
            for (auto &p : P) analyze_fwd(p);
        if (forward && elide)
            for (auto &p : P) analyze_elide(p);
        if (speculate && fast_paths && !all_leaders)
            for (auto &p : P) analyze_spec(p);
        spread_on = analyze_spread();
        spread_own = spread_on && spread_req->own;
        if (spread_on) vc_on = false;
        const bool skb_lds_planned = ctx == CTX_SKB && fast_paths && skb_fields && skb_lds_knob;
        if (lds_stack_q && fast_paths && !skb_lds_planned) {
            bool any = false;
            for (auto &p : P)
                for (uint32_t i = 0; i < p.n; i++) {
                    const DInsn &x = p.ins[i];
                    const uint32_t h = AUX_H(x.aux);
                    if ((h == H_ST || h == H_STX) && insn_dst(x) == 10 && !elided.count({p.id, i})) any = true;
                }
            if (any) E.line("#define MIMIC_LDS_STACK_Q %u", lds_stack_q);
            lds_stack_on = any;
        }
        if (defer_mode && sm_lds_knob) E.line("#define MIMIC_SM_LDS 1");
        if (const char *dv = getenv("MIMIC_JIT_DEFS")) {
            std::string all(dv), d;
            for (size_t a = 0; a <= all.size(); a++) {
                if (a < all.size() && all[a] != ',') { d += all[a]; continue; }
                const size_t eq = d.find('=');
                if (!d.empty()) E.line("#define %s %s", d.substr(0, eq).c_str(), eq == std::string::npos ? "" : d.substr(eq + 1).c_str());
                d.clear();
            }
        }
        E.line("#define PKT_ST(p_, n_, v_) st_n(p_, n_, v_)");
        E.line("#define CNT_ADD(p_, n_, v_) atomic_add_n(p_, n_, v_)");
        if (spread_on) E.line("#define MIMIC_SPREAD 1");
        if (spread_own) E.line("#define MIMIC_SPREAD_OWN 1");
        E.line("#define MIMIC_CTX_FIXED %u", ctx);
        E.line("#define MIMIC_COLD_INLINE %d", cold_inline ? 1 : 0);
        {
            bool writes = false;
            for (auto &p : P)
                for (uint32_t i = 0; i < p.n; i++)
                    if (AUX_H(p.ins[i].aux) == H_CALL && ((uint32_t)p.ins[i].k == 2 || (uint32_t)p.ins[i].k == 3)) writes = true;
            E.line("#define MIMIC_HASH_RO %d", writes ? 0 : 1);
            bool deletes = false;
            for (auto &p : P)
                for (uint32_t i = 0; i < p.n; i++)
                    if (AUX_H(p.ins[i].aux) == H_CALL && (uint32_t)p.ins[i].k == 3) deletes = true;
            E.line("#define MIMIC_HASH_POPONLY %d", deletes ? 0 : 1);
            hash_combine = combine_knob && writes && !deletes && cold_inline && fast_paths;
            if (hash_combine) E.line("#define MIMIC_HASH_COMBINE 1");
            hash_chunk = hash_combine && !proc && hchunk_knob > 0;
            if (hash_chunk) E.line("#define MIMIC_HASH_CHUNK 1\n#define MIMIC_HCHUNK %uu", (uint32_t)hchunk_knob);
        }
        E.line("#include \"runtime.h\"");
        if (spread_on) {
            E.line("#define SPREAD_MAP %uu        // the per-CPU array the fused increments go to", spread_map);
            E.line("#define SPREAD_N %uu          // counter width (bytes)", spread_n);
            E.line("#define SPREAD_ROWW %uu       // counters per vCPU row (E * S / N)", spread_row / spread_n);
            E.line("#define SPREAD_ROWS %uu       // LDS table rows (0: agent-scope atomics into the map)", spread_req->lds_rows);
            E.line("#define SPREAD_PPB %uu        // packets per block", spread_req->ppb);
            E.line("typedef %s spread_t;", spread_n == 8 ? "unsigned long long" : "uint32_t");
            E.line("#if SPREAD_ROWS");
            E.line("#define spread_add(k_) __hip_atomic_fetch_add(&sacc_[srow_ * SPREAD_ROWW + (uint32_t)(ga_ - L.t_lo) / SPREAD_N], (spread_t)(k_), __ATOMIC_RELAXED, __HIP_MEMORY_SCOPE_WORKGROUP)");
            E.line("#else");
            E.line("#define spread_add(k_) __hip_atomic_fetch_add((GAS spread_t *)(L.t_ptr + (uint32_t)(ga_ - L.t_lo)), (spread_t)(k_), __ATOMIC_RELAXED, __HIP_MEMORY_SCOPE_AGENT)");
            E.line("#endif");
        }
        if (proc) {
            E.line("#define PGID_ kp.entry_prog");
            E.line("#define TERM(s_, pc_) do { st_ = (int)(s_); epc_ = (int32_t)(pc_); pg_ = PGID_; goto L_term; } while (0)");
        } else {
            E.line("#define TERM(s_, pc_) do { st_ = (int)(s_); epc_ = (int32_t)(pc_); goto L_term; } while (0)");
        }
        E.line("#define SPILL() do { sp_.L = L; sp_.r[0] = r0; sp_.r[1] = r1; sp_.r[2] = r2; sp_.r[3] = r3; sp_.r[4] = r4; "
               "sp_.r[5] = r5; sp_.r[6] = r6; } while (0)");
        E.line("#define FILL() do { r0 = sp_.r[0]; r1 = sp_.r[1]; r2 = sp_.r[2]; r3 = sp_.r[3]; r4 = sp_.r[4]; r5 = sp_.r[5]; "
               "L.sm0 = sp_.L.sm0; L.sm1 = sp_.L.sm1; L.xdp_dirty = sp_.L.xdp_dirty; L.t_lo = sp_.L.t_lo; L.t_n = sp_.L.t_n; "
               "L.t_ptr = sp_.L.t_ptr; } while (0)");
        E.line("#define COLD_CALL(call_, pc_) do { VC_FLUSH(); SPILL(); call_; FILL(); if (sp_.st) TERM(sp_.st, pc_); } while (0)");
        E.line("#define DFR(pc_, prog_) do { dr_->pc = (int32_t)(pc_); dr_->prog = (prog_); dr_->steps = steps - 1u; goto L_defer; } while (0)");
        if (vc_on && vc_lds)
            E.line("#define VC_FLUSH() do { if (vcd_) { lvc_writeback(vcp_, vcb_, lvt_); vcd_ = 0u; } vcv_ = 0u; } while (0)");
        else if (vc_on)
            E.line("#define VC_FLUSH() do { if (vcd_) { vc_writeback(vcp_, vcb_, vc0_, vc1_, vc2_, vc3_); vcd_ = 0u; } vcv_ = 0u; } while (0)");
        else
            E.line("#define VC_FLUSH() do { } while (0)");
        const int wv = proc ? 0 : waves > 0 ? waves : (cold_inline ? 4 : 0);
        E.line("extern \"C\" __global__ __launch_bounds__(256) %svoid mimic_jit_kernel(const KParams kp_arg_) {",
               wv > 0 ? ("__attribute__((amdgpu_waves_per_eu(" + std::to_string(wv) + "))) ").c_str() : "");
        E.line("  (void)kp_arg_;   // the first (only) kernel argument: at offset 0 of the kernarg segment");
        E.line("  const KParams __attribute__((address_space(4))) *kp4_ = (const KParams __attribute__((address_space(4))) *)__builtin_amdgcn_kernarg_segment_ptr();");
        E.line("  asm volatile(\"\" : \"+s\"(kp4_));");
        E.line("  const KParams *kpp = (const KParams *)kp4_;");
        E.line("  const KParams &kp = *kpp;");
        E.line("  const uint32_t g = blockIdx.x * blockDim.x + threadIdx.x;");
        if (hash_chunk) E.line("  h_chunk_init(%s);   // (its waves: those the early return below keeps)", spread_on ? "0xffffffffu" : "kp.lanes");
        if (hash_combine) E.line("  h_comb_init();   // before any thread of the block can leave");
        if (!spread_on) E.line("  if (g >= kp.lanes) return;");
        skb_lds = ctx == CTX_SKB && fast_paths && skb_fields && skb_lds_knob;
        if (skb_lds) E.line("  __shared__ uint64_t srec_[%uu * 256u];", kSrecQ);
        E.line("  Lane L;");
        E.line("  Spill sp_;");
        if (census) {
            E.line("  uint32_t coldn_ = 0;");
            E.line("#define COLD_CALL_K(k_, call_, pc_) do { coldn_ += 1u << (k_); COLD_CALL(call_, pc_); } while (0)");
        }
        E.line("  L.lane = g;");
        if (spread_own) {
            E.line("  const uint32_t oP_ = kp.per_lane, oQ_ = kp.own_q, oS_ = oP_ / oQ_, oR_ = 256u / oS_;");
            E.line("  const uint32_t orow_ = threadIdx.x %% oR_, oj_ = threadIdx.x / oR_, olane_ = blockIdx.x * oR_ + orow_;");
            E.line("  const uint32_t osh_ = olane_ >= kp.sched_shift ? olane_ - kp.sched_shift : olane_ + kp.cpu_lanes - kp.sched_shift;");
            E.line("#define OWN_IDX_I(k_) ((oj_ < oS_ && olane_ < kp.cpu_lanes && (uint64_t)(oj_ + (k_) * oS_) * kp.cpu_lanes + osh_ < kp.n) ? (uint32_t)((uint64_t)(oj_ + (k_) * oS_) * kp.cpu_lanes + osh_) : NO_PKT)");
            E.line("#define OWN_IDX_C(k_) ((threadIdx.x + 256u * (k_) < oR_ * oP_ && (uint64_t)blockIdx.x * oR_ * oP_ + threadIdx.x + 256u * (k_) < kp.n) ? (uint32_t)((uint64_t)blockIdx.x * oR_ * oP_ + threadIdx.x + 256u * (k_)) : NO_PKT)");
            E.line("#define OWN_IDX(k_) (kp.sched == SCHED_CHUNKED ? OWN_IDX_C(k_) : OWN_IDX_I(k_))");
            E.line("  const uint32_t oi_ = OWN_IDX(0u);");
            E.line("  const bool ochk_ = kp.sched == SCHED_CHUNKED;");
            E.line("  const uint64_t ostr64_ = ochk_ ? 256ull : (uint64_t)oS_ * kp.cpu_lanes;");
            E.line("  const uint64_t oend_ = (uint64_t)blockIdx.x * oR_ * oP_ + (uint32_t)(oR_ * oP_);");
            E.line("  uint32_t ofl_ = __builtin_amdgcn_readfirstlane((kp.headroom_arr || kp.tailroom_arr || kp.ingress_arr || kp.rxq_arr || kp.egress_arr ? 1u : 0u) | (kp.headroom | kp.tailroom ? 2u : 0u));");
            E.line("  uint32_t ocpu_ = kp.vcpu_begin + olane_, oep_ = kp.entry_prog, or10_ = kp.static_next + kp.frame_size;");
            E.line("  uint32_t ostr_ = ostr64_ < 0xffffffffull ? (uint32_t)ostr64_ : 0xffffffffu;");
            E.line("  uint32_t olim_ = ochk_ && oend_ < kp.n ? (uint32_t)oend_ : kp.n;");
            E.line("  asm volatile(\"\" : \"+s\"(ostr_), \"+s\"(olim_), \"+s\"(ofl_), \"+s\"(oep_), \"+s\"(or10_));");
            E.line("  asm volatile(\"\" : \"+v\"(ocpu_));");
            E.line("  uint32_t oin_ = (uint32_t)kp.ingress, orx_ = (uint32_t)kp.rxq, oeg_ = (uint32_t)kp.egress;");
            E.line("  asm volatile(\"\" : \"+s\"(oin_), \"+s\"(orx_), \"+s\"(oeg_));");
            E.line("%s", kOwnHoist);
            E.line("  const DMap SM_ = cget(kp.maps, SPREAD_MAP);");
            E.line("  __shared__ spread_t sacc_[SPREAD_ROWS * SPREAD_ROWW];");
            E.line("  for (uint32_t w_ = threadIdx.x; w_ < SPREAD_ROWS * SPREAD_ROWW; w_ += 256u) sacc_[w_] = 0;");
            E.line("  __shared__ BatchRef obr_[MIMIC_MANY_MAX];");
            E.line("  if (threadIdx.x < (kp.many_n ? kp.many_n : 1u)) obr_[threadIdx.x] = kp.many_n ? cget(kp.many, threadIdx.x) : BatchRef{kp.pkt_data, kp.pkt_off, kp.pkt_len, kp.r0, kp.status, kp.steps, kp.err_pc, 0};");
            E.line("  __syncthreads();");
            E.line("  uint32_t srow_ = orow_, sbase_ = 0;");
            E.line("  const bool ofw_ = threadIdx.x < oR_ * SPREAD_ROWW && blockIdx.x * oR_ + threadIdx.x / SPREAD_ROWW < kp.cpu_lanes;");
            E.line("  GAS spread_t *const ofd_ = (GAS spread_t *)(kp.arena + SM_.dev_off + (size_t)(kp.vcpu_begin + blockIdx.x * oR_ + threadIdx.x / SPREAD_ROWW) * SM_.dev_stride) + threadIdx.x %% SPREAD_ROWW;");
            E.line("  const spread_t ofv_ = ofw_ ? *ofd_ : (spread_t)0;");
        } else if (spread_on) {
            E.line("  const uint32_t blo_ = blockIdx.x * SPREAD_PPB, bhi_ = blo_ + SPREAD_PPB < kp.n ? blo_ + SPREAD_PPB : kp.n;");
            E.line("  const uint32_t lam0_ = spread_lane(kp, blo_);");
            E.line("  const DMap SM_ = cget(kp.maps, SPREAD_MAP);");
            E.line("#if SPREAD_ROWS");
            E.line("  __shared__ spread_t sacc_[SPREAD_ROWS * SPREAD_ROWW];");
            E.line("  for (uint32_t w_ = threadIdx.x; w_ < SPREAD_ROWS * SPREAD_ROWW; w_ += 256u) sacc_[w_] = 0;");
            E.line("  __syncthreads();");
            E.line("#endif");
            E.line("  uint32_t srow_ = 0, sbase_ = 0;");
            E.line("  const uint32_t lstep_ = 256u %% kp.cpu_lanes;");
            E.line("  uint32_t lam_ = spread_lane(kp, blo_ + threadIdx.x);");
        } else {
            E.line("  L.cpu = lane_cpu(kp, g);");
        }
        if (vc_on) {
            if (vc_lds) {
                E.line("  __shared__ uint32_t lvc_[(%uu / 4u + 2u) * 256u];", vc_rb);
                E.line("  uint32_t *const lvt_ = lvc_ + threadIdx.x;");
                E.line("  constexpr uint32_t vcb_ = %uu;   // the row's bytes", vc_rb);
                E.line("  uint32_t vcv_ = 0u, vcd_ = 0u, vclo_ = 0u; uint8_t *vcp_ = nullptr;");
                E.line("  { const uint32_t mh_ = AUX_MAPHINT(cget(kp.insns, %uu).aux);", vc_slot);
                E.line("    if (mh_) lvc_open(kp, cget(kp.maps, mh_ - 1u), L.cpu, vcb_, vcp_, vclo_, vcv_, lvt_); }");
            } else {
                E.line("  uint64_t vc0_ = 0, vc1_ = 0, vc2_ = 0, vc3_ = 0; uint32_t vcv_ = 0u, vcd_ = 0u, vclo_ = 0u, vcb_ = 0u; uint8_t *vcp_ = nullptr;");
                E.line("  { const uint32_t mh_ = AUX_MAPHINT(cget(kp.insns, %uu).aux);", vc_slot);
                E.line("    if (mh_) vc_open(kp, cget(kp.maps, mh_ - 1u), L.cpu, vcp_, vclo_, vcb_, vcv_, vc0_, vc1_, vc2_, vc3_); }");
            }
        }
        E.line("  uint32_t ex_begin = 0, ex_count = 0;");
        E.line("  if (kp.sched == SCHED_EXPLICIT) { ex_begin = *gp(kp.sched_start + g); ex_count = *gp(kp.sched_start + g + 1) - ex_begin; }");
        E.line("  uint64_t lane_steps = 0;");
        E.line("  const uint32_t P = kp.static_next + kp.stack_size + 1;");
        if (ctx == CTX_SKB) E.line("  const uint32_t SK_ = P;   // the sk_buff entry (skb.h)");
        E.line("  uint32_t ga_ = 0;   // the address of the current memory access");
        if (ret_dispatch && any_local) E.line("  uint32_t ret_ = 0;   // the slot a popped frame returns to (R<p>_)");
        for (auto &f : fwd_store) E.line("  uint32_t fwd%u_%u_ = 0;   // value of the stack store at P%u slot %u", f.first, f.second, f.first, f.second);
        for (auto &u : spec_use)
            E.line("  %s sp%u_%u_ = 0;   // packet load of P%u slot %u, issued early", u.second == 8 ? "uint64_t" : "uint32_t",
                   u.first.first, u.first.second, u.first.first, u.first.second);
        if (!spec_use.empty()) E.line("  uint32_t spv_ = 1;   // 0 once a store through R10 left the stack: early values void");
        const bool pf = ctx == CTX_XDP && prefetch;
        if (!spec_use.empty() && !spread_on) analyze_xpf();
        lpf_on = pf && xpf.on && lpf_knob && !xpf_knob && !spread_on && !vc_lds && !lds_stack_on && !defer_mode &&
                 !hash_combine && lpf_safe();
        if (!lpf_on && !xpf_knob) xpf.on = false;
        if (spread_own) {
            if (pf) E.line("  uint64_t noff_ = 0, poff_ = 0; uint32_t nlen_ = 0, plen_ = 0;");
            E.line("  const uint32_t nb_ = kp.many_n ? kp.many_n : 1u;");
            E.line("  bool bpre_ = false;   // this batch's first descriptor came with the previous batch's last packet");
            E.line("  for (uint32_t bt_ = 0; bt_ < nb_; bt_++) {");
            E.line("  const BatchRef br_ = kp.many_n ? cget(kp.many, bt_) : BatchRef{kp.pkt_data, kp.pkt_off, kp.pkt_len, kp.r0, kp.status, kp.steps, kp.err_pc, 0};");
        }
        if (lpf_on) {
            const uint32_t D = kLpfD, XW = xpf.words;
            E.line("  // lane prefetch: packets 0..%u of the lane, descriptors + P%u slot %u window (data + %u, %u words)", D - 1,
                   xpf.prog, xpf.hp, (uint32_t)xpf.off, XW);
            E.line("  __shared__ uint64_t lpfo_[%uu * 256u];", D);
            E.line("  __shared__ uint32_t lpfl_[%uu * 256u];", D);
            E.line("  __shared__ uint64_t lpfw_[%uu * 256u];", D * XW);
            E.line("  uint32_t lpf_n_ = 0u, xc_ok_ = 0u;");
            E.line("  if (kp.entry_prog == %uu && !kp.headroom_arr && !kp.tailroom_arr && kp.headroom == 0u && kp.tailroom == 0u) {", xpf.prog);
            for (uint32_t d = 0; d < D; d++) {
                E.line("    const uint32_t lx%u_ = pkt_index(kp, g, %uu, ex_begin, ex_count);", d, d);
                E.line("    uint64_t lo%u_ = 0; uint32_t ll%u_ = 0;", d, d);
                E.line("    if (lx%u_ != NO_PKT) { lo%u_ = *gp(kp.pkt_off + lx%u_); ll%u_ = *gp(kp.pkt_len + lx%u_); }", d, d, d, d, d);
            }
            for (uint32_t d = 0; d < D; d++) {
                for (uint32_t q = 0; q < XW; q++) E.line("    uint64_t lw%u_%u_ = 0;", d, q);
                E.line("    const bool lk%u_ = lx%u_ != NO_PKT && %uu <= ll%u_;", d, d, (uint32_t)xpf.off + 8 * XW, d);
                E.line("    if (lk%u_) {", d);
                E.line("      const uint8_t *xp_ = kp.pkt_data + lo%u_ + %uu;", d, (uint32_t)xpf.off);
                for (uint32_t q = 0; q < XW; q++) E.line("      lw%u_%u_ = ld_n(xp_ + %uu, 8u);", d, q, 8 * q);
                E.line("    }");
            }
            for (uint32_t d = 0; d < D; d++) {
                E.line("    lpfo_[%uu * 256u + threadIdx.x] = lo%u_;", d, d);
                E.line("    lpfl_[%uu * 256u + threadIdx.x] = ll%u_ | (lk%u_ ? 0x80000000u : 0u);", d, d, d);
                for (uint32_t q = 0; q < XW; q++) E.line("    lpfw_[%uu * 256u + threadIdx.x] = lw%u_%u_;", d * XW + q, d, q);
            }
            E.line("    lpf_n_ = lx0_ == NO_PKT ? 0u : lx1_ == NO_PKT ? 1u : lx2_ == NO_PKT ? 2u : lx3_ == NO_PKT ? 3u : 4u;");
            E.line("  }");
            static_assert(kLpfD == 4, "the lpf_n_ line above");
        } else if (pf && xpf.on) {
            E.line("  const bool xpf_on_ = kp.entry_prog == %uu && !kp.headroom_arr;   // P%u slot %u window, data + %u, %u words",
                   xpf.prog, xpf.prog, xpf.hp, (uint32_t)xpf.off, xpf.words);
            E.line("  uint64_t noff_ = 0, noff2_ = 0; uint32_t nlen_ = 0, nlen2_ = 0, nidx_ = NO_PKT, nidx2_ = NO_PKT, xn_ok_ = 0u, xc_ok_ = 0u;");
            for (uint32_t q = 0; q < xpf.words; q++) E.line("  uint64_t xn%u_ = 0;", q);
            E.line("  nidx_ = pkt_index(kp, g, 0u, ex_begin, ex_count);");
            E.line("  if (nidx_ != NO_PKT) { noff_ = *gp(kp.pkt_off + nidx_); nlen_ = *gp(kp.pkt_len + nidx_); }");
            emit_xpf_issue("  ");
            E.line("  nidx2_ = nidx_ != NO_PKT ? pkt_next(kp, nidx_, 1u, ex_begin, ex_count) : NO_PKT;");
            E.line("  if (nidx2_ != NO_PKT) { noff2_ = *gp(kp.pkt_off + nidx2_); nlen2_ = *gp(kp.pkt_len + nidx2_); }");
        } else if (pf) {
            if (spread_own)
                E.line("  if (!bpre_ && oi_ != NO_PKT) { poff_ = *gp(br_.pkt_off + oi_); plen_ = *gp(br_.pkt_len + oi_); } bpre_ = false;");
            else
                E.line("  uint64_t noff_ = 0; uint32_t nlen_ = 0;");
            if (spread_own) {
            } else if (spread_on)
                E.line("  { const uint32_t n_ = blo_ + threadIdx.x; if (n_ < bhi_) { noff_ = *gp(kp.pkt_off + n_); nlen_ = *gp(kp.pkt_len + n_); } }");
            else
                E.line("  { const uint32_t n_ = pkt_index(kp, g, 0u, ex_begin, ex_count); if (n_ != NO_PKT) { noff_ = *gp(kp.pkt_off + n_); nlen_ = *gp(kp.pkt_len + n_); } }");
        }
        if (spread_own) {
            E.line("  uint32_t oni_ = oi_;   // the thread's next packet");
            E.line("  for (uint32_t j = 0; j < oQ_; j++) {   // the thread's packets of its lane, in order");
            E.line("    const uint32_t i = oni_;");
            E.line("    if (i == NO_PKT) break;");
            E.line("    oni_ = NO_PKT;");
            E.line("    if (j + 1u < oQ_) { const uint64_t x_ = (uint64_t)i + ostr_; if (x_ < olim_) oni_ = (uint32_t)x_; }");
        } else if (spread_on) {
            E.line("  for (uint32_t j = 0; j < SPREAD_PPB / 256u; j++) {");
            E.line("    const uint32_t i = blo_ + j * 256u + threadIdx.x;");
            E.line("    if (i >= bhi_) break;");
        } else {
            E.line("  for (uint32_t j = 0; j < kp.per_lane; j++) {");
            E.line("    uint32_t i;");
            E.line("    if (kp.sched == SCHED_CHUNKED) { const uint64_t ii = (uint64_t)g * kp.per_lane + j; if (ii >= kp.n) break; i = (uint32_t)ii; }");
            E.line("    else if (kp.sched == SCHED_INTERLEAVED) { const uint64_t ii = (uint64_t)j * kp.lanes + (g >= kp.sched_shift ? g - kp.sched_shift : g + kp.lanes - kp.sched_shift); if (ii >= kp.n) break; i = (uint32_t)ii; }");
            E.line("    else { if (j >= ex_count) break; i = ld_nt(kp.sched_pkts + ex_begin + j); }");
        }
        if (lpf_on) {
            E.line("    uint64_t poff_; uint32_t plen_;");
            for (uint32_t q = 0; q < xpf.words; q++) E.line("    uint64_t xc%u_ = 0;", q);
            E.line("    if (j < lpf_n_) {   // parked in LDS when the lane started");
            E.line("      poff_ = lpfo_[j * 256u + threadIdx.x];");
            E.line("      const uint32_t lw_ = lpfl_[j * 256u + threadIdx.x];");
            E.line("      plen_ = lw_ & 0x7fffffffu;");
            E.line("      xc_ok_ = lw_ >> 31;");
            for (uint32_t q = 0; q < xpf.words; q++)
                E.line("      if (xc_ok_) xc%u_ = lpfw_[(j * %uu + %uu) * 256u + threadIdx.x];", q, xpf.words, q);
            E.line("    } else {");
            E.line("      poff_ = *gp(kp.pkt_off + i); plen_ = *gp(kp.pkt_len + i); xc_ok_ = 0u;");
            E.line("    }");
        } else if (pf && xpf.on) {
            E.line("    const uint64_t poff_ = noff_; const uint32_t plen_ = nlen_;");
            E.line("    xc_ok_ = xn_ok_;");
            for (uint32_t q = 0; q < xpf.words; q++) E.line("    const uint64_t xc%u_ = xn%u_;", q, q);
            E.line("    noff_ = noff2_; nlen_ = nlen2_; nidx_ = nidx2_;");
            emit_xpf_issue("    ");
            E.line("    nidx2_ = nidx_ != NO_PKT ? pkt_next(kp, nidx_, j + 2u, ex_begin, ex_count) : NO_PKT;");
            E.line("    if (nidx2_ != NO_PKT) { noff2_ = *gp(kp.pkt_off + nidx2_); nlen2_ = *gp(kp.pkt_len + nidx2_); }");
        } else if (pf) {
            if (!spread_own) E.line("    const uint64_t poff_ = noff_; const uint32_t plen_ = nlen_;");
            if (spread_own) {
                E.line("    if (j + 1u < oQ_) { if (oni_ != NO_PKT) { noff_ = *gp(br_.pkt_off + oni_); nlen_ = *gp(br_.pkt_len + oni_); } }");
                E.line("    else if (bt_ + 1u < nb_ && oi_ != NO_PKT) { const BatchRef &nx_ = obr_[bt_ + 1u]; noff_ = *gp(nx_.pkt_off + oi_); nlen_ = *gp(nx_.pkt_len + oi_); bpre_ = true; }");
            }
            else if (spread_on) E.line("    { const uint32_t n_ = i + 256u; if (n_ < bhi_) { noff_ = *gp(kp.pkt_off + n_); nlen_ = *gp(kp.pkt_len + n_); } }");
            else E.line("    { const uint32_t n_ = pkt_next(kp, i, j + 1, ex_begin, ex_count); if (n_ != NO_PKT) { noff_ = *gp(kp.pkt_off + n_); nlen_ = *gp(kp.pkt_len + n_); } }");
        }
        E.line("    const KParams &kq_ = kp;");
        if (spread_own) {
            E.line("    { const uint32_t ol_ = ochk_ ? i / oP_ : olane_;");
            E.line("      srow_ = ol_ - blockIdx.x * oR_;");
            E.line("      L.cpu = (int32_t)(ocpu_ - olane_ + ol_);");
            E.line("      sbase_ = SM_.backing_addr + (uint32_t)L.cpu * SM_.addr_period; }");
        } else if (spread_on) {
            E.line("    { if (kp.sched == SCHED_CHUNKED) lam_ = i / kp.per_lane;");
            E.line("      else if (j) { lam_ += lstep_; if (lam_ >= kp.cpu_lanes) lam_ -= kp.cpu_lanes; }");
            E.line("      L.cpu = (int32_t)(kp.vcpu_begin + lam_);");
            E.line("      srow_ = lam_ >= lam0_ ? lam_ - lam0_ : lam_ + kp.cpu_lanes - lam0_;");
            E.line("      sbase_ = SM_.backing_addr + (uint32_t)L.cpu * SM_.addr_period; }");
        }
        if (ctx == CTX_SKB) {
            E.line("    uint64_t r1 = 0;");
            if (skb_lds)
                E.line("    const int ls_ = skb_load_lds(kp, L, i, r1, srec_ + %uu * threadIdx.x);", kSrecQ);
            else
                E.line("    const int ls_ = skb_load(kp, L, i, r1);");
        } else {
            if (spread_own) {
                E.line("    uint32_t H = 0u, T = 0u;");
                E.line("    L.ingress = oin_; L.rxq = orx_; L.egress = oeg_;");
                E.line("    if (ofl_) {");
                E.line("      H = kq_.headroom_arr ? ld_nt(kq_.headroom_arr + i) : kq_.headroom;");
                E.line("      T = kq_.tailroom_arr ? ld_nt(kq_.tailroom_arr + i) : kq_.tailroom;");
                E.line("      if (kq_.ingress_arr) L.ingress = (uint32_t)ld_nt(kq_.ingress_arr + i);");
                E.line("      if (kq_.rxq_arr) L.rxq = (uint32_t)ld_nt(kq_.rxq_arr + i);");
                E.line("      if (kq_.egress_arr) L.egress = (uint32_t)ld_nt(kq_.egress_arr + i);");
                E.line("    }");
            } else {
            E.line("    const uint32_t H = kq_.headroom_arr ? ld_nt(kq_.headroom_arr + i) : kq_.headroom;");
            E.line("    const uint32_t T = kq_.tailroom_arr ? ld_nt(kq_.tailroom_arr + i) : kq_.tailroom;");
            }
            if (pf) {
                E.line("    const uint32_t len = plen_;");
                E.line("    L.pkt = %s + poff_;", spread_own ? "br_.pkt_data" : "kq_.pkt_data");
            } else if (spread_own) {
                E.line("    const uint32_t len = *gp(br_.pkt_len + i);");
                E.line("    L.pkt = br_.pkt_data + *gp(br_.pkt_off + i);");
            } else {
                E.line("    const uint32_t len = *gp(kq_.pkt_len + i);");
                E.line("    L.pkt = kq_.pkt_data + *gp(kq_.pkt_off + i);");
            }
            E.line("    L.M = H + len + T;");
            E.line("    L.pa = P;");
            E.line("    L.rec = nullptr;");
            if (spread_own) E.line("    if (ofl_) {");
            E.line("    for (uint32_t b = 0; b < H; b++) *gp(L.pkt + b) = 0;");
            E.line("    for (uint32_t b = 0; b < T; b++) *gp(L.pkt + H + len + b) = 0;");
            if (spread_own) E.line("    }");
            E.line("    L.data = P + H;");
            E.line("    L.data_end = P + H + len;");
            if (!spread_own) {
            E.line("    L.ingress = (uint32_t)(kq_.ingress_arr ? ld_nt(kq_.ingress_arr + i) : kq_.ingress);");
            E.line("    L.rxq = (uint32_t)(kq_.rxq_arr ? ld_nt(kq_.rxq_arr + i) : kq_.rxq);");
            E.line("    L.egress = (uint32_t)(kq_.egress_arr ? ld_nt(kq_.egress_arr + i) : kq_.egress);");
            }
            E.line("    uint64_t r1 = P + L.M + 1;");
        }
        E.line("    SM0(L) = 0; SM1(L) = 0; L.xdp_dirty = 0; L.nframes = 0; L.tailcalls = 0; L.t_lo = 0; L.t_n = 0; L.t_ptr = nullptr;");
        E.line("    uint64_t r0 = 0, r2 = 0, r3 = 0, r4 = 0, r5 = 0, r6 = 0, r7 = 0, r8 = 0, r9 = 0;");
        if (spread_own) E.line("    uint32_t lr10_ = or10_; asm volatile(\"\" : \"+s\"(lr10_));");
        E.line("    uint64_t r10 = %s;", spread_own ? "lr10_" : "kp.static_next + kp.frame_size");
        E.line("    uint32_t steps = 0;");
        if (census) E.line("    coldn_ = 0;");
        if (!spec_use.empty()) E.line("    spv_ = 1;");
        E.line("    int st_ = 0;");
        E.line("    int32_t epc_ = -1;");
        if (proc) E.line("    uint32_t pg_ = kp.entry_prog;");
        if (ctx == CTX_SKB) E.line("    if (ls_) TERM(ls_, -1);");
        if (ctx_check) E.line("    { const uint32_t cz_ = ctx_done(kq_, i); if (cz_) TERM(MIMIC_ERR_CANCELED - 1u + cz_, 0); }");
        if (dispatch_on()) {
            E.line("    uint32_t cur_;   // no initializer: the TERM gotos above jump past it");
            E.line("    cur_ = %s;", spread_own ? "oep_" : "kp.entry_prog");
            E.line("    switch (cur_) {");
            for (auto &p : P)
                if (p.n == 0) E.line("    case %u: steps = 1; TERM(MIMIC_ERR_PC_OOB, 0);", p.id);
            E.line("%s", nonempty_cases().c_str());
            E.line("      break;");
            E.line("    default: TERM(MIMIC_ERR_PC_OOB, 0);");
            E.line("    }");
            E.line("  D_:");
            E.line("    switch (cur_) {");
            for (auto &p : P)
                if (p.n) E.line("    case %u: goto P%u_0;", p.id, p.id);
            E.line("    default: TERM(MIMIC_ERR_ENGINE_HELPER, -1);");
            E.line("    }");
        } else {
            E.line("    switch (%s) {", spread_own ? "oep_" : "kp.entry_prog");
            for (auto &p : P) {
                if (p.n == 0) E.line("    case %u: steps = 1; TERM(MIMIC_ERR_PC_OOB, 0);", p.id);
                else E.line("    case %u: goto P%u_0;", p.id, p.id);
            }
            E.line("    default: TERM(MIMIC_ERR_PC_OOB, 0);");
            E.line("    }");
        }
        for (auto &p : P) program(p);
        E.line("    TERM(MIMIC_ERR_ENGINE_HELPER, -1);");
        if (defer_mode) {
            E.line("  L_defer:");
            E.line("    VC_FLUSH();");
            E.line("    defer_finish(kp, L, g, i, j, lane_steps);");
            E.line("    break;");
        }
        E.line("  L_term:");
        if (spread_own && pf) E.line("    poff_ = noff_; plen_ = nlen_; asm volatile(\"\" : \"+v\"(poff_), \"+v\"(plen_));");
        E.line("    {");
        {
            const char *rb = spread_own ? "lb_" : "kq_";
            if (spread_own) E.line("    const BatchRef &lb_ = obr_[bt_];");
            if (ntres) {
                E.line("    if (%s.r0) st_nt(%s.r0 + i, r0);", rb, rb);
                E.line("    if (%s.status) st_nt(%s.status + i, (uint8_t)st_);", rb, rb);
            } else {
                E.line("    if (%s.r0) *gp(%s.r0 + i) = r0;", rb, rb);
                E.line("    if (%s.status) *gp(%s.status + i) = (uint8_t)st_;", rb, rb);
            }
            if (census) E.line("    if (%s.steps) st_nt(%s.steps + i, coldn_);   // census: slow-path calls, not steps", rb, rb);
            else E.line("    if (%s.steps) st_nt(%s.steps + i, steps);", rb, rb);
            E.line("    if (%s.err_pc) st_nt(%s.err_pc + i, epc_);", rb, rb);
        }
        E.line("    }");
        if (proc) {
            E.line("    if (kq_.step) { StepState *S_ = kq_.step;");
            E.line("      S_->r[0] = r0; S_->r[1] = r1; S_->r[2] = r2; S_->r[3] = r3; S_->r[4] = r4; S_->r[5] = r5;");
            E.line("      S_->r[6] = r6; S_->r[7] = r7; S_->r[8] = r8; S_->r[9] = r9; S_->r[10] = r10;");
            E.line("      S_->pc = epc_; S_->prog = pg_; S_->steps = steps; S_->status = st_; S_->started = 1u; S_->finished = 1u; }");
        }
        E.line("    lane_steps += steps;");
        E.line("  }");
        if (spread_own) E.line("  }   // batches");
        if (vc_on) E.line("  VC_FLUSH();");
        if (spread_own) {
            E.line("  __syncthreads();");
            E.line("  if (ofw_ && sacc_[threadIdx.x]) *ofd_ = ofv_ + sacc_[threadIdx.x];");
            E.line("  for (uint32_t w_ = threadIdx.x + 256u; w_ < oR_ * SPREAD_ROWW; w_ += 256u) {   // rows past 256 words");
            E.line("    const spread_t v_ = sacc_[w_];");
            E.line("    if (!v_) continue;");
            E.line("    const uint32_t r_ = w_ / SPREAD_ROWW, q_ = w_ - r_ * SPREAD_ROWW;");
            E.line("    GAS spread_t *d_ = (GAS spread_t *)(kp.arena + SM_.dev_off + (size_t)(kp.vcpu_begin + blockIdx.x * oR_ + r_) * SM_.dev_stride) + q_;");
            E.line("    *d_ += v_;");
            E.line("  }");
        } else if (spread_on) {
            E.line("#if SPREAD_ROWS");
            E.line("  __syncthreads();");
            E.line("  if (kp.spread_part && kp.cpu_lanes == SPREAD_ROWS) {");
            E.line("    spread_t *pt_ = (spread_t *)kp.spread_part + (size_t)blockIdx.x * (SPREAD_ROWS * SPREAD_ROWW);");
            E.line("    for (uint32_t w_ = threadIdx.x; w_ < SPREAD_ROWS * SPREAD_ROWW; w_ += 256u) {");
            E.line("      const uint32_t r_ = w_ / SPREAD_ROWW, q_ = w_ - r_ * SPREAD_ROWW;");
            E.line("      const uint32_t lr_ = lam0_ + r_ < SPREAD_ROWS ? lam0_ + r_ : lam0_ + r_ - SPREAD_ROWS;");
            E.line("      pt_[lr_ * SPREAD_ROWW + q_] = sacc_[w_];");
            E.line("    }");
            E.line("  } else");
            E.line("  for (uint32_t w_ = threadIdx.x; w_ < SPREAD_ROWS * SPREAD_ROWW; w_ += 256u) {");
            E.line("    const spread_t v_ = sacc_[w_];");
            E.line("    if (!v_) continue;");
            E.line("    const uint32_t r_ = w_ / SPREAD_ROWW, q_ = w_ - r_ * SPREAD_ROWW;");
            E.line("    const uint32_t lr_ = lam0_ + r_ < kp.cpu_lanes ? lam0_ + r_ : lam0_ + r_ - kp.cpu_lanes;");
            E.line("    spread_t *d_ = (spread_t *)(kp.arena + SM_.dev_off + (size_t)(kp.vcpu_begin + lr_) * SM_.dev_stride) + q_;");
            E.line("    __hip_atomic_fetch_add((GAS spread_t *)d_, v_, __ATOMIC_RELAXED, __HIP_MEMORY_SCOPE_AGENT);");
            E.line("  }");
            E.line("#endif");
        }
        E.line("  if (kp.lane_steps) st_nt(kp.lane_steps + g, lane_steps);");
        if (hash_chunk) E.line("  h_chunk_fini();   // the block's last wave hands its chunk's remainder back");
        E.line("}");
        if (spread_own) {
            std::string hs;
            char b[512];
            for (uint32_t s : own_k) {
                snprintf(b, sizeof b, "  uint64_t hk%u_ = cget(kp.insns, %uu).k; asm volatile(\"\" : \"+s\"(hk%u_));\n", s, s, s);
                hs += b;
            }
            for (uint32_t s : own_h) {
                snprintf(b, sizeof b, "  uint32_t hh%u_ = AUX_MAPHINT(cget(kp.insns, %uu).aux); asm volatile(\"\" : \"+s\"(hh%u_));\n", s, s, s);
                hs += b;
            }
            if (!hs.empty()) hs.pop_back();
            const size_t q = E.s.find(kOwnHoist);
            E.s.replace(q, strlen(kOwnHoist), hs);
        }
        if (census) {
            static const char *kinds[] = {"cold_load(", "cold_store(", "cold_lookup(", "cold_update(", "cold_delete(",
                                          "cold_tailcall(", "cold_ldabs(", "cold_adjust_tail("};
            for (int k = 0; k < 8; k++) {
                const std::string from = std::string("COLD_CALL(") + kinds[k], to = "COLD_CALL_K(" + std::to_string(4 * k) + ", " + kinds[k];
                for (size_t q = E.s.find(from); q != std::string::npos; q = E.s.find(from, q + to.size())) E.s.replace(q, from.size(), to);
            }
        }
        return E.s;
    }

  private:
    const std::vector<ProgView> &P;
    Emitter E;
    const char *pa() const { return ctx == CTX_SKB ? "L.pa" : "P"; }
    std::string ord(const std::string &v, uint32_t n) const {
        return ctx == CTX_SKB && n > 1 ? "bswap_n(" + v + ", " + std::to_string(n) + "u)" : v;
    }
    static constexpr uint32_t SKB_HEADROOM_J = 32;
    bool any_tail = false, any_local = false, all_leaders = false;
    static constexpr const char *kOwnHoist = "  //@own_hoist@";
    std::set<uint32_t> own_k, own_h;
    uint32_t blk_start = 0;
    uint32_t cur_prog = 0;

    std::vector<uint32_t> leaders(const ProgView &p) const {
        std::set<uint32_t> lead = {0};
        for (uint32_t i = 0; i < p.n; i++) {
            const DInsn &x = p.ins[i];
            const uint32_t h = AUX_H(x.aux);
            if ((h == H_JA || h == H_JCC || h == H_CALL_LOCAL) && (x.aux & AUX_JT_OK))
                lead.insert((uint32_t)jump_target(x, i));
            if (ends_block(x) && i + 1 < p.n) lead.insert(i + 1);
            if (all_leaders) lead.insert(i);
        }
        return std::vector<uint32_t>(lead.begin(), lead.end());
    }

    std::map<std::pair<uint32_t, uint32_t>, uint32_t> fwd_call;
    std::set<std::pair<uint32_t, uint32_t>> fwd_store;
    std::set<std::pair<uint32_t, uint32_t>> elided;
    void analyze_elide(const ProgView &p) {
        if (any_tail || any_local || p.n == 0) return;
        const std::vector<uint32_t> Lb = leaders(p);
        std::map<uint32_t, size_t> blk;
        for (size_t b = 0; b < Lb.size(); b++) blk[Lb[b]] = b;
        std::vector<uint32_t> in(Lb.size(), 0);
        std::vector<bool> seen(Lb.size(), false);
        in[0] = 1u << 10;
        seen[0] = true;
        auto transfer = [&](uint32_t t, const DInsn &x) {
            const uint32_t h = AUX_H(x.aux), d = insn_dst(x), sr = insn_src(x), op = insn_op(x);
            if (d > 10) return t;
            if (h == H_ALU64 || h == H_ALU32) {
                const bool mov = (op & 0xf0) == 0xb0;
                const bool src_t = (x.aux & AUX_X) && sr <= 10 && ((t >> sr) & 1);
                const bool res = mov ? src_t : (((t >> d) & 1) || src_t);
                return res ? (t | (1u << d)) : (t & ~(1u << d));
            }
            if (h == H_LDX || h == H_LDIMM) return t & ~(1u << d);
            if (h == H_CALL) return t & ~1u;
            return t;
        };
        for (bool changed = true; changed;) {
            changed = false;
            for (size_t b = 0; b < Lb.size(); b++) {
                if (!seen[b]) continue;
                const uint32_t s0 = Lb[b], e = b + 1 < Lb.size() ? Lb[b + 1] : p.n;
                uint32_t t = in[b];
                for (uint32_t i = s0; i < e; i++) {
                    const DInsn &x = p.ins[i];
                    const uint32_t h = AUX_H(x.aux), sr = insn_src(x);
                    if (h == H_LDX && sr <= 10 && ((t >> sr) & 1)) return;
                    if (h == H_STX && sr <= 10 && ((t >> sr) & 1)) return;
                    if (h == H_SLOW || h == H_LDABS || h == H_CALL_LOCAL) return;
                    if (h == H_CALL && !((uint32_t)x.k == 1 && fwd_call.count({p.id, i})) && (uint32_t)x.k != 8) return;
                    t = transfer(t, x);
                }
                const DInsn &last = p.ins[e - 1];
                const uint32_t h = AUX_H(last.aux);
                std::vector<int64_t> succ;
                if ((!ends_block(last) || h == H_JCC) && (last.aux & AUX_FALL_OK)) succ.push_back(e);
                if ((h == H_JA || h == H_JCC) && (last.aux & AUX_JT_OK)) succ.push_back(jump_target(last, e - 1));
                for (int64_t sx : succ) {
                    auto it = blk.find((uint32_t)sx);
                    if (it == blk.end()) continue;
                    const uint32_t nin = in[it->second] | t;
                    if (!seen[it->second] || nin != in[it->second]) {
                        in[it->second] = nin;
                        seen[it->second] = true;
                        changed = true;
                    }
                }
            }
        }
        for (auto &f : fwd_store)
            if (f.first == p.id && AUX_H(p.ins[f.second].aux) == H_STX && insn_dst(p.ins[f.second]) == 10) elided.insert(f);
    }
    void analyze_fwd(const ProgView &p) {
        if (!fast_paths || p.n == 0) return;
        const std::vector<uint32_t> Lb = leaders(p);
        for (size_t b = 0; b < Lb.size(); b++) {
            const uint32_t s0 = Lb[b], e = b + 1 < Lb.size() ? Lb[b + 1] : p.n;
// ... 1091 lines not shown
        E.line("    r1 = 0; r2 = 0; r3 = 0; r4 = 0; r5 = 0;");
    }

    void slow(const ProgView &p, uint32_t i) {
        (void)p;
        const DInsn &x = p.ins[i];
        const uint32_t op = insn_op(x), d = insn_dst(x), s = insn_src(x), cls = op & 7, hi = op & 0xf0;
        const bool xsrc = (op & 0x08) != 0;
        const int32_t off = insn_off(x);
        if (cls == 1) {
            static const uint32_t szs[4] = {4, 2, 1, 8};
            E.line("    %s", cold("cold_load(kp, sp_, " + addr(s, off) + ", " + std::to_string(szs[(op >> 3) & 3]) + "u)", i).c_str());
            E.line("    TERM(%s, %u);", d > 10 ? "MIMIC_PANIC_BADREG" : "MIMIC_ERR_R10_WRITE", i);
            return;
        }
        if (hi == 0xd0) {
            if (d > 10) {
                E.line("    TERM(MIMIC_PANIC_BADREG, %u);", i);
                return;
            }
            const std::string D = reg(d);
            std::string v = D;
            if (x.k == 16) v = xsrc ? "(" + D + " & 0xffffull)" : "(((" + D + " >> 8) & 0xffull) | ((" + D + " & 0xffull) << 8))";
            else if (x.k == 32) v = xsrc ? "(" + D + " & 0xffffffffull)" : "(uint64_t)__builtin_bswap32((uint32_t)" + D + ")";
            else if (x.k == 64) v = xsrc ? "(" + D + " >> 32)" : "(uint64_t)__builtin_bswap32((uint32_t)(" + D + " >> 32))";
            if (d == 10) E.line("    TERM(MIMIC_ERR_R10_WRITE, %u);", i);
            else E.line("    %s = %s;", D.c_str(), v.c_str());
            return;
        }
        const bool is64 = cls == 7;
        E.line("    if (%s == 0) TERM(MIMIC_PANIC_DIV0, %u);", is64 ? reg(s).c_str() : ("(uint32_t)" + reg(s)).c_str(), i);
        if (d == 10) E.line("    TERM(MIMIC_ERR_R10_WRITE, %u);", i);
        else E.line("    %s = %s(0x%02xu, %s, %s);", reg(d).c_str(), is64 ? "alu64" : "alu32", hi, reg(d).c_str(), reg(s).c_str());
    }
};

std::string cache_name(const std::string &src, const char *const *opts, int nopts) {
    uint64_t a = 1469598103934665603ull, b = 0x9e3779b97f4a7c15ull;
    auto mix = [&](const char *p, size_t n) {
        for (size_t i = 0; i < n; i++) {
            a = (a ^ (uint8_t)p[i]) * 1099511628211ull;
            b = (b + (uint8_t)p[i]) * 0xff51afd7ed558ccdull;
            b ^= b >> 29;
        }
    };
    mix(src.data(), src.size());
    for (int i = 0; i < nopts; i++) mix(opts[i], strlen(opts[i]) + 1);
    for (int i = 0; i < kJitHeaderCount; i++) mix(kJitHeaderSrc[i], strlen(kJitHeaderSrc[i]));
    int maj = 0, min = 0;
    hiprtcVersion(&maj, &min);
    char v[32];
    snprintf(v, sizeof v, "rtc%d.%d", maj, min);
    mix(v, strlen(v));
    char out[48];
    snprintf(out, sizeof out, "%016" PRIx64 "%016" PRIx64 ".hsaco", a, b);
    return out;
}

std::string cache_path(const std::string &name) {
    const char *d = getenv("MIMIC_JIT_CACHE");
    if (!d || !*d) return "";
    return std::string(d) + "/" + name;
}

bool read_file(const std::string &path, std::vector<char> &out) {
    FILE *f = fopen(path.c_str(), "rb");
    if (!f) return false;
    fseek(f, 0, SEEK_END);
    const long n = ftell(f);
    fseek(f, 0, SEEK_SET);
    out.resize(n > 0 ? (size_t)n : 0);
    const bool ok = n > 0 && fread(out.data(), 1, (size_t)n, f) == (size_t)n;
    fclose(f);
    return ok;
}

void write_file_atomic(const std::string &path, const std::vector<char> &data) {
    const std::string tmp = path + ".tmp" + std::to_string((long)getpid());
    FILE *f = fopen(tmp.c_str(), "wb");
    if (!f) return;
    const bool ok = fwrite(data.data(), 1, data.size(), f) == data.size();
    fclose(f);
    if (ok) rename(tmp.c_str(), path.c_str());
    else remove(tmp.c_str());
}

const char *const kOpts[] = {"--offload-arch=gfx950", "-O3", "-std=c++17", "-Wno-unused-label", "-Wno-unused-variable", "-Wno-c++20-extensions"};
const int kNOpts = (int)(sizeof kOpts / sizeof *kOpts);

int build_code(const std::string &src, std::vector<char> &code, std::string *log) {
    const std::string path = cache_path(cache_name(src, kOpts, kNOpts));
    if (!path.empty() && read_file(path, code)) return 0;
    setenv("AMD_COMGR_CACHE", "0", 0);
    hiprtcProgram prog;
    if (hiprtcCreateProgram(&prog, src.c_str(), "mimic_jit.hip", kJitHeaderCount, kJitHeaderSrc, kJitHeaderNames) !=
        HIPRTC_SUCCESS) {
        *log = "hiprtcCreateProgram failed";
        return -1;
    }
    const hiprtcResult rc = hiprtcCompileProgram(prog, kNOpts, kOpts);
    size_t ls = 0;
    hiprtcGetProgramLogSize(prog, &ls);
    std::string lg(ls + 1, '\0');
    if (ls) hiprtcGetProgramLog(prog, &lg[0]);
    if (rc != HIPRTC_SUCCESS) {
        *log = "hipRTC: " + std::string(hiprtcGetErrorString(rc)) + "\n" + lg;
        hiprtcDestroyProgram(&prog);
        return -1;
    }
    size_t cs = 0;
    hiprtcGetCodeSize(prog, &cs);
    code.resize(cs);
    hiprtcGetCode(prog, code.data());
    hiprtcDestroyProgram(&prog);
    if (!path.empty()) write_file_atomic(path, code);
    return 0;
}

struct CacheKey {
    int device;
    std::string src;
    bool operator<(const CacheKey &o) const { return device != o.device ? device < o.device : src < o.src; }
};
std::mutex g_mu;
std::map<CacheKey, hipFunction_t> g_cache;

}

std::string mimic_jit_source(const std::vector<DProg> &progs, const std::vector<DInsn> &all, uint32_t ctx_kind,
                             JitInfo *info, const std::vector<std::pair<uint32_t, uint32_t>> *vc_slots, bool no_early_loads,
                             const SpreadReq *spread, bool ctx_check, bool proc) {
    std::vector<ProgView> v;
    for (size_t p = 0; p < progs.size(); p++) v.push_back(ProgView{(uint32_t)p, progs[p].n, progs[p].base, all.data() + progs[p].base});
    Gen g(v, ctx_kind);
    if (vc_slots)
        for (auto &v : *vc_slots)
            if (v.second > 0 && v.second <= MIMIC_VC_MAX_ROW && !(v.second & 7)) g.vc_ok[v.first] = v.second;
    if (no_early_loads) g.speculate = 0;
    g.spread_req = spread;
    static const bool ctx_env = getenv("MIMIC_JIT_CTXCHECK") && getenv("MIMIC_JIT_CTXCHECK")[0] == '1';
    g.ctx_check = ctx_check || ctx_env;
    g.proc = proc;
    if (proc) g.inc_knob = false;
    std::string src = g.source();
    if (info) {
        info->checks_budget = g.careful_copies;
        info->max_n = g.max_n;
        info->tail_calls = g.has_tail();
        info->early_loads = g.has_early_loads();
        info->cold_inline = g.cold_inline;
        info->defer = g.defer_mode;
        info->spread = g.spread_on;
        info->spread_own = g.spread_own;
        info->hash_combine = g.hash_combine;
        info->hash_chunk = g.hash_chunk;
        info->proc = proc;
        info->proc_ok = proc && ctx_kind == CTX_XDP && !g.careful_copies && !g.defer_mode && !g.spread_on && !g.census;
        info->spread_map = g.spread_map;
        info->spread_n = g.spread_n;
        info->spread_roww = g.spread_n ? g.spread_row / g.spread_n : 0;
        info->spread_rows = g.spread_on && spread ? spread->lds_rows : 0;
    }
    return src;
}

uint64_t mimic_jit_step_bound(const JitInfo &info, uint32_t max_tail_calls) {
    if (info.checks_budget) return 0;
    return (info.tail_calls ? (uint64_t)max_tail_calls + 1 : 1) * ((uint64_t)info.max_n + 1);
}

int mimic_jit_compile(int device, const std::string &src, hipFunction_t *fn, std::string *log) {
    std::lock_guard<std::mutex> lk(g_mu);
    const CacheKey key{device, src};
    auto it = g_cache.find(key);
    if (it != g_cache.end()) {
        *fn = it->second;
        return 0;
    }
    std::vector<char> code;
    if (build_code(src, code, log)) return -1;
    hipModule_t mod;
    hipError_t e = hipModuleLoadData(&mod, code.data());
    if (e != hipSuccess) {
        *log = std::string("hipModuleLoadData: ") + hipGetErrorString(e);
        return -1;
    }
    e = hipModuleGetFunction(fn, mod, "mimic_jit_kernel");
    if (e != hipSuccess) {
        *log = std::string("hipModuleGetFunction: ") + hipGetErrorString(e);
        return -1;
    }
    g_cache[key] = *fn;
    return 0;
}

int mimic_jit_build_code(const std::string &src, std::vector<char> &code, std::string *log) {
    return build_code(src, code, log);
}

int mimic_jit_prebuild_source(const std::string &src, std::string *log) {
    std::vector<char> code;
    return build_code(src, code, log);
}

int mimic_jit_launch(hipFunction_t fn, const KParams *kp, hipStream_t st) {
    const uint32_t blocks = (kp->lanes + 255) / 256;
    if (blocks == 0) return 0;
    void *args[] = {(void *)kp};
    return hipModuleLaunchKernel(fn, blocks, 1, 1, 256, 1, 1, 0, st, args, nullptr) == hipSuccess ? 0 : -1;
}

int mimic_jit_check_source(const std::string &src, std::string *log, size_t *code_size) {
    setenv("AMD_COMGR_CACHE", "0", 0);
    hiprtcProgram prog;
    if (hiprtcCreateProgram(&prog, src.c_str(), "mimic_jit.hip", kJitHeaderCount, kJitHeaderSrc, kJitHeaderNames) !=
        HIPRTC_SUCCESS)
        return -1;
    const hiprtcResult rc = hiprtcCompileProgram(prog, kNOpts, kOpts);
    size_t ls = 0;
    hiprtcGetProgramLogSize(prog, &ls);
    std::string lg(ls + 1, '\0');
    if (ls) hiprtcGetProgramLog(prog, &lg[0]);
    *log = lg;
    if (code_size) hiprtcGetCodeSize(prog, code_size);
    hiprtcDestroyProgram(&prog);
    return rc == HIPRTC_SUCCESS ? 0 : -1;
}
```

mimic_amd/csrc/jit.h:

```cpp
#pragma once
#include <hip/hip_runtime.h>

#include <map>
#include <string>
#include <vector>

#include "layout.h"

struct JitInfo {
    bool checks_budget;
    uint32_t max_n;
    bool tail_calls;
    bool early_loads;
    bool cold_inline;
    bool defer;
    bool spread;
    bool spread_own;
    bool hash_combine;
    bool hash_chunk;
    bool proc, proc_ok;
    uint32_t spread_map, spread_n, spread_roww, spread_rows;
};
struct SpreadReq {
    std::map<uint32_t, uint32_t> slot_map;
    std::map<uint32_t, std::pair<uint32_t, uint32_t>> shape;
    uint32_t lds_rows = 0;
    uint32_t ppb = 1024;
    bool own = false;
};
#define MIMIC_VC_MAX_ROW 128u
std::string mimic_jit_source(const std::vector<DProg> &progs, const std::vector<DInsn> &all, uint32_t ctx_kind,
                             JitInfo *info, const std::vector<std::pair<uint32_t, uint32_t>> *vc_slots = nullptr,
                             bool no_early_loads = false,
                             const SpreadReq *spread = nullptr, bool ctx_check = false, bool proc = false);
uint64_t mimic_jit_step_bound(const JitInfo &info, uint32_t max_tail_calls);
int mimic_jit_compile(int device, const std::string &src, hipFunction_t *fn, std::string *log);
int mimic_jit_launch(hipFunction_t fn, const KParams *kp, hipStream_t st);
int mimic_jit_check_source(const std::string &src, std::string *log, size_t *code_size);
int mimic_jit_build_code(const std::string &src, std::vector<char> &code, std::string *log);
int mimic_jit_prebuild_source(const std::string &src, std::string *log);
```

mimic_amd/csrc/layout.h:

```cpp
#pragma once
#include <stdint.h>
#if defined(__HIPCC__) || defined(__HIP__) || defined(__HIPCC_RTC__)
#define HHD_LAYOUT static __host__ __device__ inline
#else
#define HHD_LAYOUT static inline
#endif

#define MIMIC_MAX_FRAMES 32u
#define MIMIC_DEFAULT_BUDGET (1ull << 22)
#define MIMIC_MEM_START 0x10000u
#define MIMIC_PC_BITS 24u
#define MIMIC_XDP_MD_SIZE 24u
#define MIMIC_FRAME_QWORDS 5u

enum SegKind : uint32_t {
    SEG_PLAIN = 1,
    SEG_ARRAY_OBJ = 2,
    SEG_MAP_OBJ = 3,
    SEG_PROG = 4,
    SEG_PERCPU_ARRAY = 5,
    SEG_PERCPU_VALUES = 6,
};

enum MapFamily : uint32_t { FAM_ARRAY = 1, FAM_PERCPU_ARRAY = 2, FAM_HASH = 3, FAM_PERCPU_HASH = 4 };
// ... 17 lines not shown
    uint32_t addr_period;
    uint32_t ncpu;
    uint64_t dev_off;
    uint64_t dev_stride;
    uint64_t keys_dev_off;
    uint32_t keys_addr;
    uint32_t ht_cap;
    uint64_t ht_dev_off;
    uint32_t rec_q;
    uint32_t nlocks;
    uint32_t fl_cap;
    uint32_t hflags;
};
#define HT_F_CHUNK 1u
#define HT_CHUNK_MAXE (1u << 17)
#define HT_LEFT_CAP 16384u

#define HT_USED_SHARDS 16
struct HashCtl {
    unsigned long long head;
    uint32_t comb_fault;
    uint32_t pad0[29];
    unsigned long long tail;
    int32_t avail;
    uint32_t used0;
    uint32_t pad1[28];
    uint32_t used_sh[HT_USED_SHARDS * 32];
    uint32_t cminv;
    uint32_t full;
    uint32_t cdone;
    uint32_t nleft;
    uint32_t pad2[28];
    uint32_t live_sh[HT_USED_SHARDS * 32];
};
HHD_LAYOUT uint64_t ht_ext_bytes(uint32_t E) {
    const uint64_t e32 = ((uint64_t)E + 1023) & ~1023ull;
    return e32 + e32 * 4 + (uint64_t)HT_LEFT_CAP * 8;
}
#define HT_EMPTY 0xffffffffu
#define HT_TOMB 0xfffffffeu
#define HT_BUSY 0xfffffffdu

struct DProg {
    uint32_t base;
    uint32_t n;
    uint32_t addr;
    uint32_t pad;
};

enum Handler : uint32_t {
    H_SLOW = 0,
    H_ERR = 1,
    H_NOP = 2,
    H_ALU64 = 3,
    H_ALU32 = 4,
    H_LDIMM = 5,
    H_JA = 6,
    H_JCC = 7,
    H_LDX = 8,
    H_ST = 9,
    H_STX = 10,
    H_EXIT = 11,
    H_CALL = 12,
    H_CALL_LOCAL = 13,
    H_LDABS = 14,
};
#define AUX_H(a) ((a) & 0xffu)
#define AUX_FALL_OK (1u << 8)
#define AUX_JT_OK (1u << 9)
#define AUX_JT_NEG (1u << 10)
#define AUX_W32 (1u << 11)
#define AUX_X (1u << 12)
#define AUX_ARG(a) (((a) >> 16) & 0xffu)
#define AUX_SZ(a) ((a) >> 24)
#define AUX_MAPHINT(a) ((a) >> 16)
struct DInsn {
    uint32_t w;
    uint32_t aux;
    uint64_t k;
};

enum Sched : uint32_t { SCHED_CHUNKED = 0, SCHED_INTERLEAVED = 1, SCHED_EXPLICIT = 2 };

enum CtxKind : uint32_t { CTX_XDP = 0, CTX_SKB = 1 };
struct SkbRec;

#define MIMIC_MANY_MAX 8u
struct BatchRef {
    uint8_t *pkt_data;
    const uint64_t *pkt_off;
    const uint32_t *pkt_len;
    uint64_t *r0;
    uint8_t *status;
    uint32_t *steps;
    int32_t *err_pc;
    uint64_t pad;
};

struct KParams {
    const DInsn *insns;
    const DProg *progs;
    const Seg *segs;
    const DMap *maps;
    uint8_t *arena;
    uint32_t nprogs, nsegs, nmaps, entry_prog;
    uint32_t static_next;
    uint32_t stack_size;
    uint32_t frame_size;
    uint32_t chunk_shift;
    uint32_t max_tail_calls;
    uint32_t total_vcpus;
    uint32_t vcpu_begin;
    uint32_t lanes;
    uint32_t priv_lanes;
    uint8_t *priv;
    uint32_t priv_xdp_q;
    uint32_t priv_frame_q;
    uint32_t priv_key_q;
    uint32_t cpu_lanes;
    uint64_t budget;
    uint32_t n;
    uint32_t sched;
    uint32_t per_lane;
    uint32_t sched_shift;
    uint8_t *pkt_data;
    const uint64_t *pkt_off;
    const uint32_t *pkt_len;
    const uint32_t *headroom_arr;
    const uint32_t *tailroom_arr;
    const int32_t *ingress_arr;
    const int32_t *rxq_arr;
    const int32_t *egress_arr;
    uint32_t headroom, tailroom;
    int32_t ingress, rxq, egress;
    uint32_t step_gen;
    const uint32_t *sched_start;
    const uint32_t *sched_pkts;
    uint64_t *r0;
    uint8_t *status;
    uint32_t *steps;
    int32_t *err_pc;
    uint64_t *lane_steps;
    uint32_t ctx_kind;
    uint32_t skb_ifindex;
    SkbRec *skb_rec;
    const uint64_t *skb_prefix;
    const uint64_t *skb_base;
    struct StepState *step;
    uint32_t hash_pop_only;
    uint32_t hash_ro;
    struct DeferRec *defer;
    uint32_t *defer_any;
    uint32_t defer_epoch;
    uint32_t reserved0;
    uint32_t *spread_bad;
    const void *skb_custom;
    const uint64_t *skb_drv;
    void *spread_part;
    const uint32_t *cancel;
    const uint32_t *const *cancel_pp;
    uint32_t cancel_any;
    uint32_t own_q;
    uint32_t many_n;
    struct BatchRef many[MIMIC_MANY_MAX];
    const uint8_t *step_img;
    uint8_t *step_dst;
    uint32_t step_img_n;
    uint32_t step_ins_n;
    uint32_t *skb_rooms_state;
};
static_assert(sizeof(KParams) == 968, "KParams: the kernarg layout of every JIT kernel");
static_assert(__builtin_offsetof(KParams, reserved0) == 356 && __builtin_offsetof(KParams, spread_bad) == 360,
              "KParams: the fields around the reserved word keep their offsets");

struct DeferRec {
    uint64_t r[11];
    int32_t pc;
    uint32_t prog;
    uint32_t steps;
    uint32_t j;
    uint64_t lane_steps;
    uint64_t sm0, sm1;
    uint32_t xdp_dirty, nframes, tailcalls;
    uint32_t flag;
};

struct StepState {
    uint64_t r[11];
    int32_t pc;
    uint32_t prog;
    uint32_t steps;
    int32_t status;
    uint32_t started;
    uint32_t finished;
    int32_t cpu;
    uint32_t gen;
    uint8_t lane[256];
};
```

mimic_amd/jit.py:

```python
from __future__ import annotations

import ctypes as C
import os
import subprocess
import sys
import tempfile
from typing import Dict, Iterable, List, Sequence, Tuple

from . import _lib

CTX_XDP, CTX_SKB = 0, 1


def _progs_args(raws: Sequence[bytes]):
    bufs = [C.create_string_buffer(bytes(r), max(len(r), 1)) for r in raws]
    arr = (C.c_void_p * max(len(raws), 1))(*[C.cast(b, C.c_void_p) for b in bufs])
    ns = (C.c_uint32 * max(len(raws), 1))(*[len(r) // 8 for r in raws])
    return bufs, arr, ns


def kernel_source(raws: Sequence[bytes], ctx: int = CTX_XDP, vc: Sequence[Tuple[int, int, int]] = (), spread=None,
                  proc: bool = False, no_early_loads: bool = False) -> str:
    if spread is not None:
        return spread_source(raws, *spread)[0]
    lib = _lib.load()
    keep, arr, ns = _progs_args(raws)
    flat = [v for t in vc for v in t]
    vca = (C.c_uint32 * max(len(flat), 1))(*flat)
    kind = ctx | (0x100 if proc else 0) | (0x200 if no_early_loads else 0)
    n = lib.mimic_jit_source_vc(arr, ns, len(raws), kind, vca, len(vc), None, 0)
    if n < 0:
        raise ValueError(f"cannot decode programs ({n})")
    buf = C.create_string_buffer(n + 1)
    lib.mimic_jit_source_vc(arr, ns, len(raws), kind, vca, len(vc), buf, n + 1)
    return buf.value.decode()


def vc_slots(progs: Sequence[Tuple[bytes, Sequence]], maps: Sequence[dict]) -> List[Tuple[int, int, int]]:
    by_name = {m["name"]: m for m in maps}
    out = []
    for pi, (raw, rel) in enumerate(progs):
        for r in rel:
            slot, name = r[0], r[1]
            m = by_name.get(name)
            if m is None or m["type"] != 6:
                continue
            rb = m["max_entries"] * m["value_size"]
            if not (0 < rb <= 128 and rb % 8 == 0):
                continue
            src, off = raw[8 * slot + 1] >> 4, int.from_bytes(raw[8 * slot + 2:8 * slot + 4], "little", signed=True)
            if src == 1 or (src == 2 and off == 0):
                out.append((pi, slot, rb))
    return out


def spread_spec(progs: Sequence[Tuple[bytes, Sequence]], maps: Sequence[dict], vcpus: int, ppb: int = 1024,
                own: bool = False):
    by_name = {m["name"]: (i, m) for i, m in enumerate(maps)}
    pc, shapes = [], {}
    for pi, (raw, rel) in enumerate(progs):
        for r in rel:
            slot, name = r[0], r[1]
            if name not in by_name or by_name[name][1]["type"] != 6:
                continue
            mid, m = by_name[name]
            if (m["max_entries"] * m["value_size"]) % 8:
                continue
            src, off = raw[8 * slot + 1] >> 4, int.from_bytes(raw[8 * slot + 2:8 * slot + 4], "little", signed=True)
            if src == 1 or (src == 2 and off == 0):
                pc.append((pi, slot, mid))
                shapes[mid] = (mid, m["max_entries"] * m["value_size"], m["value_size"])
    row = max((s[1] for s in shapes.values()), default=0)
    if own:
        return pc, list(shapes.values()), (min(256, 32768 // row) if row else 0) | (1 << 31)
    rows = min(ppb, vcpus)
    return pc, list(shapes.values()), rows if rows * row <= 32768 else 0


def spread_source(raws: Sequence[bytes], pc, shapes, lds_rows: int) -> Tuple[str, bool]:
    lib = _lib.load()
    keep, arr, ns = _progs_args(raws)
    pcf = [v for t in pc for v in t]
    shf = [v for t in shapes for v in t]
    pca = (C.c_uint32 * max(len(pcf), 1))(*pcf)
    sha = (C.c_uint32 * max(len(shf), 1))(*shf)
    ok = C.c_int32()
    n = lib.mimic_jit_source_spread(arr, ns, len(raws), pca, len(pc), sha, len(shapes), lds_rows, C.byref(ok), None, 0)
    if n < 0:
        raise ValueError(f"cannot decode programs ({n})")
    buf = C.create_string_buffer(n + 1)
    lib.mimic_jit_source_spread(arr, ns, len(raws), pca, len(pc), sha, len(shapes), lds_rows, C.byref(ok), buf, n + 1)
    return buf.value.decode(), bool(ok.value)


def code_object(src: str) -> bytes:
    lib = _lib.load()
    size = C.c_size_t()
    if lib.mimic_jit_code(src.encode(), None, 0, C.byref(size)) != 0:
        raise RuntimeError("hipRTC compile failed")
    buf = C.create_string_buffer(size.value)
    lib.mimic_jit_code(src.encode(), buf, size.value, C.byref(size))
    return buf.raw[:size.value]


def _notes(elf: bytes):
    import struct

    shoff, = struct.unpack_from("<Q", elf, 0x28)
    shentsize, shnum = struct.unpack_from("<HH", elf, 0x3A)
    for i in range(shnum):
        sh = shoff + i * shentsize
        stype, = struct.unpack_from("<I", elf, sh + 4)
        if stype != 7:
            continue
        off, size = struct.unpack_from("<QQ", elf, sh + 0x18)
        p, end = off, off + size
        while p + 12 <= end:
            nsz, dsz, typ = struct.unpack_from("<III", elf, p)
            name = elf[p + 12:p + 12 + nsz].rstrip(b"\0").decode()
            d0 = p + 12 + ((nsz + 3) & ~3)
            yield name, typ, elf[d0:d0 + dsz]
            p = d0 + ((dsz + 3) & ~3)


def kernel_resources(code: bytes, kernel: str = "mimic_jit_kernel") -> Dict[str, int]:
    import msgpack

    for name, typ, desc in _notes(code):
        if name != "AMDGPU" or typ != 32:
            continue
        md = msgpack.unpackb(desc, raw=False)
        for k in md.get("amdhsa.kernels", []):
            if k.get(".name") != kernel:
                continue
            total, a = int(k.get(".vgpr_count", 0)), int(k.get(".agpr_count", 0))
            alloc = max(8, (total + 7) & ~7)
            return {"vgpr": total - a, "agpr": a, "vgpr_total": total, "sgpr": int(k.get(".sgpr_count", 0)),
                    "vgpr_spill": int(k.get(".vgpr_spill_count", 0)), "sgpr_spill": int(k.get(".sgpr_spill_count", 0)),
                    "scratch": int(k.get(".private_segment_fixed_size", 0)),
                    "lds": int(k.get(".group_segment_fixed_size", 0)), "waves_per_simd": min(8, 512 // alloc)}
    raise KeyError(f"kernel {kernel} not in the code object's metadata")


def _cache_dir() -> str:
    d = os.environ.get("MIMIC_JIT_CACHE", "")
    if not d:
        raise RuntimeError("MIMIC_JIT_CACHE is not set: prewarming needs an on-disk kernel cache")
    os.makedirs(d, exist_ok=True)
    return d


def prewarm(kernels: Iterable[Tuple], workers: int = 0) -> Dict[str, float]:
    import time

    t0 = time.time()
    _cache_dir()
    kernels = list(kernels)
    srcs: Dict[str, Tuple] = {}
    for k in kernels:
        srcs.setdefault(kernel_source(list(k[0]), *k[1:]), k)
    info = _compile_parallel(list(srcs), workers)
    alt: Dict[str, None] = {}
    for src, k in srcs.items():
        if "issued early" in src and "amdgpu_waves_per_eu(4)" in src:
            try:
                if kernel_resources(code_object(src))["scratch"] > 0:
                    alt[kernel_source(list(k[0]), *k[1:], no_early_loads=True)] = None
            except RuntimeError:
                pass
    info2 = _compile_parallel(list(alt), workers)
    return {"kernels": len(srcs) + len(alt), "seconds": time.time() - t0,
            "worker_failures": info["worker_failures"] + info2["worker_failures"],
            "failed_after_retry": info["failed_after_retry"] + info2["failed_after_retry"]}


def _compile_parallel(srcs, workers: int) -> Dict[str, int]:
    todo = sorted(srcs, key=len, reverse=True)
    if not todo:
        return {"worker_failures": 0, "failed_after_retry": 0}
    if workers <= 0:
        workers = max(1, min(16, os.cpu_count() or 1) - 1)
    workers = min(workers, len(todo))
    with tempfile.TemporaryDirectory(prefix="mimic_jitwarm_") as tmp:
        lists = [[] for _ in range(workers)]
        for k, s in enumerate(todo):
            path = os.path.join(tmp, f"k{k}.hip")
            with open(path, "w") as f:
                f.write(s)
            lists[k % workers].append(path)
        root = os.path.dirname(os.path.dirname(os.path.abspath(__file__)))

        def launch(w):
            env = dict(os.environ)
            env["TMPDIR"] = os.path.join(tmp, f"t{w}")
            os.makedirs(env["TMPDIR"], exist_ok=True)
            return subprocess.Popen([sys.executable, "-m", "mimic_amd.jit", os.path.join(tmp, f"w{w}.txt")],
                                    env=env, cwd=root)

        for w, paths in enumerate(lists):
            with open(os.path.join(tmp, f"w{w}.txt"), "w") as f:
                f.write("\n".join(paths))
        rcs = [p.wait() for p in [launch(w) for w in range(workers)]]
        retry = [w for w, rc in enumerate(rcs) if rc]
        rcs2 = [p.wait() for p in [launch(w) for w in retry]]
    return {"worker_failures": len(retry), "failed_after_retry": sum(1 for rc in rcs2 if rc)}


def _worker(list_file: str) -> int:
    lib = _lib.load()
    rc = 0
    with open(list_file) as f:
        for path in f.read().split():
            with open(path) as g:
                if lib.mimic_jit_cache_source(g.read().encode()) != 0:
                    print(f"mimic_amd.jit: compile failed: {path}", file=sys.stderr)
                    rc = 1
    return rc


if __name__ == "__main__":
    sys.exit(_worker(sys.argv[1]))
```

mimic_amd/vm.py:

```python
from __future__ import annotations

import base64
import ctypes as C
import json
import os
from dataclasses import dataclass, field
from enum import IntEnum
from typing import Dict, Iterable, List, Optional, Sequence, Tuple

from . import _lib as L


class MimicError(RuntimeError):
    pass


class MapType(IntEnum):
    Hash = 1
    Array = 2
    ProgramArray = 3
    PerfEventArray = 4
    PerCPUHash = 5
    PerCPUArray = 6

# ... 527 lines not shown
                    stream=None, sync: bool = True, ctx: Optional["Context"] = None,
                    ctx_per_packet: Optional[Sequence[Optional["Context"]]] = None) -> "XDPResults":
        if results is None:
            results = XDPResults.empty(batch.n, batch.pkt_data.device)
        b = batch._c()
        r = results._c()
        st = stream.cuda_stream if stream is not None else None
        h, arr, _keep = _ctx_args(ctx, ctx_per_packet, batch.n)
        if h is not None or arr is not None:
            rc = self.lib.mimic_run_xdp_ctx(self.h, prog_id, b, r, st, h, arr)
        else:
            rc = self.lib.mimic_run_xdp(self.h, prog_id, b, r, st)
        if rc:
            _check(self.h, rc, "RunXDPBatch")
        if sync:
            _check(self.h, self.lib.mimic_sync(self.h, st), "sync")
        else:
            results._inflight = (batch, _keep)
        return results

    def RunXDPMany(self, prog_id: int, batches: Sequence["XDPBatch"], results: Optional[Sequence["XDPResults"]] = None,
                   stream=None, sync: bool = True) -> List["XDPResults"]:
        if results is None:
            results = [XDPResults.empty(b.n, b.pkt_data.device) for b in batches]
        k = len(batches)
        bs, rs = (L.XDPBatch * max(k, 1))(), (L.XDPResults * max(k, 1))()
        for q, (bt, rt) in enumerate(zip(batches, results)):
            bt._c()
            rt._c()
            bs[q], rs[q] = bt._cstruct_obj, rt._cstruct_obj
        st = stream.cuda_stream if stream is not None else None
        rc = self.lib.mimic_run_xdp_many(self.h, prog_id, bs, rs, k, st)
        if rc:
            _check(self.h, rc, "RunXDPMany")
        if sync:
            _check(self.h, self.lib.mimic_sync(self.h, st), "sync")
        else:
            for bt, rt in zip(batches, results):
                rt._inflight = bt
        return list(results)

    def RunSKBBatch(self, prog_id: int, batch: "SKBBatch", results: Optional["XDPResults"] = None,
                    stream=None, sync: bool = True, ctx: Optional["Context"] = None,
                    ctx_per_packet: Optional[Sequence[Optional["Context"]]] = None) -> "XDPResults":
        if results is None:
            results = XDPResults.empty(batch.n, batch.pkt_data.device)
        st = stream.cuda_stream if stream is not None else None
        h, arr, _keep = _ctx_args(ctx, ctx_per_packet, batch.n)
        if h is not None or arr is not None:
            rc = self.lib.mimic_run_skb_ctx(self.h, prog_id, batch._c(), results._c(), st, h, arr)
        else:
            rc = self.lib.mimic_run_skb(self.h, prog_id, batch._c(), results._c(), st)
        if rc:
            _check(self.h, rc, "RunSKBBatch")
        if sync:
            _check(self.h, self.lib.mimic_sync(self.h, st), "sync")
        else:
            results._inflight = (batch, _keep)
        return results

    def CleanupProcesses(self, procs: Sequence["Process"]) -> None:
        nat = [p._native for p in procs if p._native is not None]
        if nat and getattr(self, "h", None):
            self.lib.mimic_process_free_many((C.c_void_p * len(nat))(*nat), len(nat))
        for p in procs:
            p._native = None

    def RunProcesses(self, procs: Sequence["Process"], ctxs: Optional[Sequence[Optional["Context"]]] = None,
                     cpus: Optional[Sequence[int]] = None) -> None:
        n = len(procs)
        if not n:
            return
        for p in procs:
            p._ensure_native()
        arr = (C.c_void_p * n)(*[p._native for p in procs])
        cx = None
        if ctxs is not None and any(_live(c) is not None for c in ctxs):
            hs = {}
            for c in ctxs:
                if _live(c) is not None and id(c) not in hs:
                    hs[id(c)] = c._device_handle()
            cx = (C.c_void_p * n)(*[hs[id(c)] if _live(c) is not None else None for c in ctxs])
        import numpy as np

        regs = (L.ProcessRegs * n)()
        ca = None
        if cpus is not None:
            ca = np.ascontiguousarray(cpus, dtype=np.int32)
        _check(self.h, self.lib.mimic_process_run_many(arr, n, ca.ctypes.data if ca is not None else None, cx, regs),
               "RunProcesses")
        a = np.ctypeslib.as_array(regs)
        r0, steps = a["r"][:, 0].tolist(), a["steps"].tolist()
        sts, pcs = a["status"].tolist(), a["pc"].tolist()
        for p, x, s, st, pc in zip(procs, r0, steps, sts, pcs):
            p.Registers.R0 = x
            p.Steps = s
            p.Status = st
            p._exited = True
            p._started = True
            p.ErrPC = pc if st else -1

    def SKBRelease(self) -> None:
        _check(self.h, self.lib.mimic_skb_release(self.h), "skb release")

    def RunXDPHost(self, prog_id: int, buf, off, lens, schedule=L.SCHED_INTERLEAVED, cpu=None, headroom: int = 0,
                   tailroom: int = 0, ingress: int = 0, rxq: int = 0, egress: int = 0, step_budget: int = 0,
                   chunks: int = 0, pkt_out=None, r0=None, status=None, ctx: Optional["Context"] = None,
                   ctx_per_packet: Optional[Sequence[Optional["Context"]]] = None):
        import numpy as np

        n = len(lens)
        off = np.ascontiguousarray(off, dtype=np.uint64)
        lens = np.ascontiguousarray(lens, dtype=np.uint32)
        r0 = np.empty(n, np.uint64) if r0 is None else r0
        status = np.empty(n, np.uint8) if status is None else status
        hb = L.XDPHostBatch()
        hb.n, hb.schedule = n, schedule
        hb.pkt_data, hb.pkt_off, hb.pkt_len = buf.ctypes.data, off.ctypes.data, lens.ctypes.data
        hb.headroom_all, hb.tailroom_all = headroom, tailroom
        hb.ingress_all, hb.rxq_all, hb.egress_all = ingress, rxq, egress
        cpu_arr = None
        if cpu is not None:
            cpu_arr = np.ascontiguousarray(cpu, dtype=np.int32)
            hb.cpu = cpu_arr.ctypes.data
        hb.step_budget = step_budget
        hb.pkt_out = pkt_out.ctypes.data if pkt_out is not None else None
        hb.r0, hb.status = r0.ctypes.data, status.ctypes.data
        h, arr, _keep = _ctx_args(ctx, ctx_per_packet, n)
        if h is not None:
            _check(self.h, self.lib.mimic_run_xdp_host_ctx(self.h, prog_id, C.byref(hb), chunks, h), "RunXDPHost")
        elif arr is not None:
            _check(self.h, self.lib.mimic_run_xdp_host_ctx_pp(self.h, prog_id, C.byref(hb), chunks, arr), "RunXDPHost")
        else:
            _check(self.h, self.lib.mimic_run_xdp_host(self.h, prog_id, C.byref(hb), chunks), "RunXDPHost")
        return r0, status

    def HostRegister(self, arr) -> None:
        _check(self.h, self.lib.mimic_host_register(arr.ctypes.data, arr.nbytes), "host register")

    def HostUnregister(self, arr) -> None:
        _check(self.h, self.lib.mimic_host_unregister(arr.ctypes.data), "host unregister")

    def LastSteps(self) -> int:
        v = C.c_uint64()
        _check(self.h, self.lib.mimic_last_steps(self.h, C.byref(v)), "last steps")
        return v.value

    def ExecMode(self) -> str:
        return {1: "interp", 2: "jit"}[self.lib.mimic_exec_mode(self.h)]

    def LastExec(self) -> str:
        return {0: "none", 1: "interp", 2: "jit", 3: "spread", 4: "spread_own"}[self.lib.mimic_last_exec(self.h)]

    def SetSpread(self, mode: int) -> None:
        _check(self.h, self.lib.mimic_set_spread(self.h, mode), "SetSpread")


def NewVM(*opts) -> VM:
    emu = None
    spread = None
    s = VMSettings(vcpus=os.cpu_count() or 1)
    for k, v in opts:
        if k == "emulator":
            emu = v
        elif k == "vcpus":
            s.vcpus = v
        elif k == "device":
            s.device = v
        elif k == "shard":
            s.vcpu_begin, s.vcpu_count = v
        elif k == "exec":
            s.exec_mode = v
        elif k == "spread":
            spread = v
    vm = VM(emu, s)
    if spread is not None:
        vm.SetSpread(spread)
    return vm


class Registers:

    def __init__(self):
        self.PC = 0
        for q in range(11):
            setattr(self, f"R{q}", 0)

    def Get(self, r: int) -> int:
        return getattr(self, f"R{r}")


class Process:

    def __init__(self, vm: VM, prog_id: int, ctx=None):
        self.VM = vm
        self.prog_id = prog_id
        self.Context = ctx
        self.Registers = Registers()
        self.cpuID = -1
        self.Steps = 0
        self.Status = None
        self.ErrPC = -1
        self.PacketAfter: Optional[bytes] = None
        self._native = None
        self._exited = False
        self._started = False
        self.Registers.R10 = vm.StackAddress() + vm.settings.stack_frame_size
        if isinstance(ctx, LinuxContextSKBuff):
            self._ensure_native()

    def CPUID(self) -> int:
        return self.cpuID

    def SetCPUID(self, i: int) -> None:
        if i < 0:
            raise MimicError("not a valid CPU ID")
        if i > self.VM.settings.vcpus:
            raise MimicError(f"vm only has {self.VM.settings.vcpus} vCPUs, max CPU ID is {self.VM.settings.vcpus - 1}")
        self.cpuID = i
        if self._native is not None:
            _check(self.VM.h, self.VM.lib.mimic_process_set_cpu(self._native, i), "SetCPUID")

    def _ensure_native(self):
        if self._native is not None:
            return
        ctx = self.Context or LinuxContextXDP()
        h = C.c_void_p()
        pkt = bytes(ctx.Packet)
        if isinstance(ctx, LinuxContextSKBuff):
            cust = skb_custom_record(ctx)
            cp = cust.ctypes.data if int(cust["flags"]) else None
            _check(self.VM.h, self.VM.lib.mimic_process_new_skb_ctx(self.VM.h, self.prog_id, pkt, len(pkt),
                                                                     ctx.Dev.IFIndex if ctx.Dev else 0, cp, C.byref(h)),
                   "NewProcess")
        else:
            _check(self.VM.h, self.VM.lib.mimic_process_new(self.VM.h, self.prog_id, pkt, len(pkt), ctx.Headroom,
                                                             ctx.Tailroom, ctx.IngessIfIndex, ctx.RxQueueIndex,
                                                             ctx.EgressIfIndex, C.byref(h)), "NewProcess")
        self._native = h
        if self.cpuID >= 0:
            _check(self.VM.h, self.VM.lib.mimic_process_set_cpu(h, self.cpuID), "SetCPUID")

    def _take(self, regs) -> None:
        for q in range(11):
            setattr(self.Registers, f"R{q}", int(regs.r[q]))
        self.Registers.PC = int(regs.pc)
        self.ProgramID = int(regs.prog_id)
        self.Steps = int(regs.steps)
        self.Status = int(regs.status)
        self._exited = bool(regs.exited)

    def Step(self) -> bool:
        self._ensure_native()
        self._started = True
        regs = L.ProcessRegs()
        rc = self.VM.lib.mimic_process_step(self._native, 1, C.byref(regs))
        if rc < 0:
            _check(self.VM.h, rc, "Step")
        self._take(regs)
        if self.Status:
            self.ErrPC = self.Registers.PC
            raise MimicError(f"inst at PC({self.Registers.PC}): {L.STATUS_NAMES[self.Status]}")
        return self._exited

    def Run(self, step_budget: int = 0, ctx: Optional["Context"] = None) -> None:
        self._ensure_native()
        self._started = True
        regs = L.ProcessRegs()
        if ctx is not None:
            rc = self.VM.lib.mimic_process_run_ctx(self._native, step_budget, ctx._device_handle(), C.byref(regs))
            if rc in (L.ECANCELED, L.EDEADLINE):
                self._take(regs)
                raise MimicError(Context._ERR[1 if rc == L.ECANCELED else 2])
            _check(self.VM.h, rc, "Run")
        else:
            _check(self.VM.h, self.VM.lib.mimic_process_run(self._native, step_budget, C.byref(regs)), "Run")
        self._take(regs)
        self.ErrPC = self.Registers.PC if self.Status else -1
        self.PacketAfter = self.Packet()
        if self.Status:
            raise MimicError(f"process encountered a fatal error: {L.STATUS_NAMES[self.Status]} at PC({self.ErrPC})")

    def Packet(self) -> bytes:
        if self._native is None:
            return self.PacketAfter or b""
        ctx = self.Context or LinuxContextXDP()
        if isinstance(ctx, LinuxContextSKBuff):
            n = 32 + len(ctx.Packet) + 64
        else:
            n = ctx.Headroom + len(ctx.Packet) + ctx.Tailroom
        buf = C.create_string_buffer(max(n, 1))
        _check(self.VM.h, self.VM.lib.mimic_process_packet(self._native, buf, max(n, 1)), "packet")
        return buf.raw[:n]

    def Cleanup(self) -> None:
        if self._native is not None and getattr(self.VM, "h", None):
            self.VM.lib.mimic_process_free(self._native)
        self._native = None

    def __del__(self):
        try:
            self.Cleanup()
        except Exception:
            pass


# ... 526 lines not shown
```

Before: 61090 Mpkts/s.

## Restructure spread_own kernel into per-wave task loop with optional dynamic dealing

Replaces the nested per-batch and per-packet loops of the spread_own JIT kernel with one flat loop over wave-sized tasks spanning all batches. Packet indices come from shared geometry helpers, and a magic-number divide maps each task to its batch. An optional mode, enabled only by an environment variable, hands out tasks dynamically through an LDS atomic counter for load balancing. By default each wave takes a static stride of four, which changes the work order and prefetch across batch boundaries. This adds per-iteration readfirstlane and batch-switch overhead.

```diff
diff --git a/include/mimic_amd.h b/include/mimic_amd.h
--- a/include/mimic_amd.h
+++ b/include/mimic_amd.h
@@ -255,6 +255,7 @@
 int mimic_exec_mode(const mimic_vm *vm);
 int mimic_set_spread(mimic_vm *vm, int32_t mode);
 int mimic_last_exec(const mimic_vm *vm);
+int mimic_last_own_deal(const mimic_vm *vm);
 long mimic_jit_source_for(const void *const *progs, const uint32_t *n_slots, uint32_t n_progs, char *buf, size_t cap);
 int mimic_jit_check(const char *src, char *log, size_t cap, size_t *code_size);
 int mimic_jit_prebuild(const void *const *progs, const uint32_t *n_slots, uint32_t n_progs);
diff --git a/mimic_amd/_lib.py b/mimic_amd/_lib.py
--- a/mimic_amd/_lib.py
+++ b/mimic_amd/_lib.py
@@ -112,6 +112,7 @@
     "mimic_host_register": (C.c_int, [C.c_void_p, C.c_size_t]),
     "mimic_host_unregister": (C.c_int, [C.c_void_p]),
     "mimic_last_exec": (C.c_int, [C.c_void_p]),
+    "mimic_last_own_deal": (C.c_int, [C.c_void_p]),
     "mimic_jit_source_for": (C.c_long, [C.POINTER(C.c_void_p), C.POINTER(C.c_uint32), C.c_uint32, C.c_char_p,
                                          C.c_size_t]),
     "mimic_jit_check": (C.c_int, [C.c_char_p, C.c_char_p, C.c_size_t, C.POINTER(C.c_size_t)]),
diff --git a/mimic_amd/csrc/engine.cpp b/mimic_amd/csrc/engine.cpp
--- a/mimic_amd/csrc/engine.cpp
+++ b/mimic_amd/csrc/engine.cpp
@@ -173,6 +173,7 @@
     int spread_mode = -1;
     bool spread_lds = false;
     int last_exec = 0;
+    int last_own_deal = 0;
     static constexpr int KP_SLOTS = 64;
     KParams *d_kp = nullptr, *h_kp = nullptr;
     hipEvent_t kp_ev[KP_SLOTS] = {};
@@ -2044,6 +2045,10 @@
             q = std::max<uint32_t>(1, std::min(q, P));
             while (q > 1 && (P % q || 256u * q / P > vm->spread_own_rows)) q--;
             kp.own_q = q;
+            const char *dv = getenv("MIMIC_SPREAD_OWN_DEAL");
+            const bool plain = !kp.headroom && !kp.tailroom && !kp.headroom_arr && !kp.tailroom_arr && !kp.ingress_arr &&
+                               !kp.rxq_arr && !kp.egress_arr;
+            kp.own_deal = vm->spread_own_state > 0 && vm->jit_info_spread_own.own_deal && plain && dv && dv[0] == '1' ? 1u : 0u;
             own = vm->spread_own_state > 0 && P % q == 0 && 256u * q / P <= vm->spread_own_rows && 256u * q / P >= 1u &&
                   mimic_jit_step_bound(vm->jit_info_spread_own, kp.max_tail_calls) <= kp.budget;
             spread = own;
@@ -2167,6 +2172,8 @@
         if (mimic_launch_hash_rebuild(vm->arena, &dm, 0, st))
             return fail(vm, MIMIC_EDEVICE, "launch: %s", hipGetErrorString(hipGetLastError()));
     }
+    if (!own) kp.own_deal = 0;
+    vm->last_own_deal = (int)kp.own_deal;
     vm->last_exec = jit ? (own ? MIMIC_EXEC_SPREAD_OWN : spread ? MIMIC_EXEC_SPREAD : MIMIC_EXEC_JIT) : MIMIC_EXEC_INTERP;
     if (jit && ji.defer) {
         if (lanes > vm->defer_cap || !vm->d_defer_any) {
@@ -2862,6 +2869,7 @@
     return 0;
 }
 int mimic_last_exec(const mimic_vm *vm) { return vm ? vm->last_exec : MIMIC_EINVAL; }
+int mimic_last_own_deal(const mimic_vm *vm) { return vm ? vm->last_own_deal : MIMIC_EINVAL; }
 
 long mimic_jit_source_for(const void *const *progs, const uint32_t *n_slots, uint32_t n_progs, char *buf, size_t cap) {
     return mimic_jit_source_for_ctx(progs, n_slots, n_progs, MIMIC_CTX_XDP, buf, cap);
@@ -2919,7 +2927,7 @@
     req.own = (lds_rows >> 31) != 0;
     JitInfo info{};
     const std::string src = mimic_jit_source(dp, all, MIMIC_CTX_XDP, &info, nullptr, false, &req);
-    if (spread_out) *spread_out = info.spread ? 1 : 0;
+    if (spread_out) *spread_out = (info.spread ? 1 : 0) | (info.spread_own && info.own_deal ? 2 : 0);
     if (buf && cap > src.size()) memcpy(buf, src.c_str(), src.size() + 1);
     return (long)src.size();
 }
diff --git a/mimic_amd/csrc/jit.cpp b/mimic_amd/csrc/jit.cpp
--- a/mimic_amd/csrc/jit.cpp
+++ b/mimic_amd/csrc/jit.cpp
@@ -148,6 +148,7 @@
     bool proc = false;
     bool spread_on = false;
     bool spread_own = false;
+    bool own_deal_ok = false;
     uint32_t spread_map = 0, spread_n = 0, spread_row = 0;
     std::map<uint32_t, uint32_t> vc_ok;
     uint32_t vc_slot = 0;
@@ -196,6 +197,7 @@
             for (auto &p : P) analyze_spec(p);
         spread_on = analyze_spread();
         spread_own = spread_on && spread_req->own;
+        own_deal_ok = spread_own && lpf_safe();
         if (spread_on) vc_on = false;
         const bool skb_lds_planned = ctx == CTX_SKB && fast_paths && skb_fields && skb_lds_knob;
         if (lds_stack_q && fast_paths && !skb_lds_planned) {
@@ -296,22 +298,21 @@
         }
         E.line("  L.lane = g;");
         if (spread_own) {
-            E.line("  const uint32_t oP_ = kp.per_lane, oQ_ = kp.own_q, oS_ = oP_ / oQ_, oR_ = 256u / oS_;");
-            E.line("  const uint32_t orow_ = threadIdx.x %% oR_, oj_ = threadIdx.x / oR_, olane_ = blockIdx.x * oR_ + orow_;");
-            E.line("  const uint32_t osh_ = olane_ >= kp.sched_shift ? olane_ - kp.sched_shift : olane_ + kp.cpu_lanes - kp.sched_shift;");
-            E.line("#define OWN_IDX_I(k_) ((oj_ < oS_ && olane_ < kp.cpu_lanes && (uint64_t)(oj_ + (k_) * oS_) * kp.cpu_lanes + osh_ < kp.n) ? (uint32_t)((uint64_t)(oj_ + (k_) * oS_) * kp.cpu_lanes + osh_) : NO_PKT)");
-            E.line("#define OWN_IDX_C(k_) ((threadIdx.x + 256u * (k_) < oR_ * oP_ && (uint64_t)blockIdx.x * oR_ * oP_ + threadIdx.x + 256u * (k_) < kp.n) ? (uint32_t)((uint64_t)blockIdx.x * oR_ * oP_ + threadIdx.x + 256u * (k_)) : NO_PKT)");
-            E.line("#define OWN_IDX(k_) (kp.sched == SCHED_CHUNKED ? OWN_IDX_C(k_) : OWN_IDX_I(k_))");
-            E.line("  const uint32_t oi_ = OWN_IDX(0u);");
-            E.line("  const bool ochk_ = kp.sched == SCHED_CHUNKED;");
-            E.line("  const uint64_t ostr64_ = ochk_ ? 256ull : (uint64_t)oS_ * kp.cpu_lanes;");
-            E.line("  const uint64_t oend_ = (uint64_t)blockIdx.x * oR_ * oP_ + (uint32_t)(oR_ * oP_);");
+            E.line("  const uint32_t oQ_ = kp.own_q, nb_ = kp.many_n ? kp.many_n : 1u;");
+            E.line("  const OwnGeo og_ = own_geo(kp.sched, kp.n, kp.cpu_lanes, kp.sched_shift, kp.per_lane, oQ_);");
+            E.line("  const uint32_t oR_ = og_.R;");
+            E.line("  const uint32_t ow_ = __builtin_amdgcn_readfirstlane(threadIdx.x >> 6), oln_ = threadIdx.x & 63u;");
+            E.line("  uint32_t o4q_ = 4u * oQ_, ont_ = nb_ * o4q_, omag_ = own_magic(o4q_), odl_ = kp.own_deal;");
+            E.line("  const BatchRef ob0_ = kp.many_n ? cget(kp.many, 0u) : BatchRef{kp.pkt_data, kp.pkt_off, kp.pkt_len, kp.r0, kp.status, kp.steps, kp.err_pc, 0};");
+            E.line("  uint8_t *bpd_ = ob0_.pkt_data; const uint64_t *bpo_ = ob0_.pkt_off; const uint32_t *bpl_ = ob0_.pkt_len;");
+            E.line("  uint32_t oni_ = own_task_pkt(og_, blockIdx.x, ow_, oln_);   // the lane's packet of the wave's current task");
+            if (ctx == CTX_XDP && prefetch) {
+                E.line("  uint64_t noff_ = 0, poff_ = 0; uint32_t nlen_ = 0, plen_ = 0;");
+                E.line("  if (oni_ != NO_PKT) { poff_ = *gp(bpo_ + oni_); plen_ = *gp(bpl_ + oni_); }");
+            }
             E.line("  uint32_t ofl_ = __builtin_amdgcn_readfirstlane((kp.headroom_arr || kp.tailroom_arr || kp.ingress_arr || kp.rxq_arr || kp.egress_arr ? 1u : 0u) | (kp.headroom | kp.tailroom ? 2u : 0u));");
-            E.line("  uint32_t ocpu_ = kp.vcpu_begin + olane_, oep_ = kp.entry_prog, or10_ = kp.static_next + kp.frame_size;");
-            E.line("  uint32_t ostr_ = ostr64_ < 0xffffffffull ? (uint32_t)ostr64_ : 0xffffffffu;");
-            E.line("  uint32_t olim_ = ochk_ && oend_ < kp.n ? (uint32_t)oend_ : kp.n;");
-            E.line("  asm volatile(\"\" : \"+s\"(ostr_), \"+s\"(olim_), \"+s\"(ofl_), \"+s\"(oep_), \"+s\"(or10_));");
-            E.line("  asm volatile(\"\" : \"+v\"(ocpu_));");
+            E.line("  uint32_t ocpu_ = kp.vcpu_begin + blockIdx.x * oR_, oep_ = kp.entry_prog, or10_ = kp.static_next + kp.frame_size;");
+            E.line("  asm volatile(\"\" : \"+s\"(ont_), \"+s\"(omag_), \"+s\"(ofl_), \"+s\"(oep_), \"+s\"(or10_), \"+s\"(ocpu_));");
             E.line("  uint32_t oin_ = (uint32_t)kp.ingress, orx_ = (uint32_t)kp.rxq, oeg_ = (uint32_t)kp.egress;");
             E.line("  asm volatile(\"\" : \"+s\"(oin_), \"+s\"(orx_), \"+s\"(oeg_));");
             E.line("%s", kOwnHoist);
@@ -320,8 +321,10 @@
             E.line("  for (uint32_t w_ = threadIdx.x; w_ < SPREAD_ROWS * SPREAD_ROWW; w_ += 256u) sacc_[w_] = 0;");
             E.line("  __shared__ BatchRef obr_[MIMIC_MANY_MAX];");
             E.line("  if (threadIdx.x < (kp.many_n ? kp.many_n : 1u)) obr_[threadIdx.x] = kp.many_n ? cget(kp.many, threadIdx.x) : BatchRef{kp.pkt_data, kp.pkt_off, kp.pkt_len, kp.r0, kp.status, kp.steps, kp.err_pc, 0};");
+            E.line("  __shared__ uint32_t otk_;");
+            E.line("  if (threadIdx.x == 0u) otk_ = 8u;");
             E.line("  __syncthreads();");
-            E.line("  uint32_t srow_ = orow_, sbase_ = 0;");
+            E.line("  uint32_t srow_ = 0, sbase_ = 0;");
             E.line("  const bool ofw_ = threadIdx.x < oR_ * SPREAD_ROWW && blockIdx.x * oR_ + threadIdx.x / SPREAD_ROWW < kp.cpu_lanes;");
             E.line("  GAS spread_t *const ofd_ = (GAS spread_t *)(kp.arena + SM_.dev_off + (size_t)(kp.vcpu_begin + blockIdx.x * oR_ + threadIdx.x / SPREAD_ROWW) * SM_.dev_stride) + threadIdx.x %% SPREAD_ROWW;");
             E.line("  const spread_t ofv_ = ofw_ ? *ofd_ : (spread_t)0;");
@@ -372,11 +375,8 @@
                  !hash_combine && lpf_safe();
         if (!lpf_on && !xpf_knob) xpf.on = false;
         if (spread_own) {
-            if (pf) E.line("  uint64_t noff_ = 0, poff_ = 0; uint32_t nlen_ = 0, plen_ = 0;");
-            E.line("  const uint32_t nb_ = kp.many_n ? kp.many_n : 1u;");
-            E.line("  bool bpre_ = false;   // this batch's first descriptor came with the previous batch's last packet");
-            E.line("  for (uint32_t bt_ = 0; bt_ < nb_; bt_++) {");
-            E.line("  const BatchRef br_ = kp.many_n ? cget(kp.many, bt_) : BatchRef{kp.pkt_data, kp.pkt_off, kp.pkt_len, kp.r0, kp.status, kp.steps, kp.err_pc, 0};");
+            E.line("  uint32_t otc_ = ow_, otn_ = ow_ + 4u, otf_ = 0u;");
+            E.line("  asm volatile(\"\" : \"+v\"(otc_), \"+v\"(otn_));");
         }
         if (lpf_on) {
             const uint32_t D = kLpfD, XW = xpf.words;
@@ -419,10 +419,7 @@
             E.line("  nidx2_ = nidx_ != NO_PKT ? pkt_next(kp, nidx_, 1u, ex_begin, ex_count) : NO_PKT;");
             E.line("  if (nidx2_ != NO_PKT) { noff2_ = *gp(kp.pkt_off + nidx2_); nlen2_ = *gp(kp.pkt_len + nidx2_); }");
         } else if (pf) {
-            if (spread_own)
-                E.line("  if (!bpre_ && oi_ != NO_PKT) { poff_ = *gp(br_.pkt_off + oi_); plen_ = *gp(br_.pkt_len + oi_); } bpre_ = false;");
-            else
-                E.line("  uint64_t noff_ = 0; uint32_t nlen_ = 0;");
+            if (!spread_own) E.line("  uint64_t noff_ = 0; uint32_t nlen_ = 0;");
             if (spread_own) {
             } else if (spread_on)
                 E.line("  { const uint32_t n_ = blo_ + threadIdx.x; if (n_ < bhi_) { noff_ = *gp(kp.pkt_off + n_); nlen_ = *gp(kp.pkt_len + n_); } }");
@@ -430,12 +427,14 @@
                 E.line("  { const uint32_t n_ = pkt_index(kp, g, 0u, ex_begin, ex_count); if (n_ != NO_PKT) { noff_ = *gp(kp.pkt_off + n_); nlen_ = *gp(kp.pkt_len + n_); } }");
         }
         if (spread_own) {
-            E.line("  uint32_t oni_ = oi_;   // the thread's next packet");
-            E.line("  for (uint32_t j = 0; j < oQ_; j++) {   // the thread's packets of its lane, in order");
+            E.line("  for (;;) {   // the wave's tasks");
+            E.line("    const uint32_t tc_ = __builtin_amdgcn_readfirstlane(otc_);");
+            E.line("    if (tc_ >= ont_) break;");
+            E.line("    const uint32_t bt_ = own_task_batch(tc_, omag_);   // the task's batch");
+            E.line("    uint32_t obx_ = bt_; asm volatile(\"\" : \"+v\"(obx_));   // (in a VGPR across the packet, for its result addresses)");
             E.line("    const uint32_t i = oni_;");
-            E.line("    if (i == NO_PKT) break;");
-            E.line("    oni_ = NO_PKT;");
-            E.line("    if (j + 1u < oQ_) { const uint64_t x_ = (uint64_t)i + ostr_; if (x_ < olim_) oni_ = (uint32_t)x_; }");
+            E.line("    const uint32_t tn_ = __builtin_amdgcn_readfirstlane(otn_), nbt_ = own_task_batch(tn_, omag_);");
+            E.line("    oni_ = nbt_ < nb_ ? own_task_pkt(og_, blockIdx.x, tn_ - nbt_ * o4q_, oln_) : NO_PKT;");
         } else if (spread_on) {
             E.line("  for (uint32_t j = 0; j < SPREAD_PPB / 256u; j++) {");
             E.line("    const uint32_t i = blo_ + j * 256u + threadIdx.x;");
@@ -471,17 +470,21 @@
         } else if (pf) {
             if (!spread_own) E.line("    const uint64_t poff_ = noff_; const uint32_t plen_ = nlen_;");
             if (spread_own) {
-                E.line("    if (j + 1u < oQ_) { if (oni_ != NO_PKT) { noff_ = *gp(br_.pkt_off + oni_); nlen_ = *gp(br_.pkt_len + oni_); } }");
-                E.line("    else if (bt_ + 1u < nb_ && oi_ != NO_PKT) { const BatchRef &nx_ = obr_[bt_ + 1u]; noff_ = *gp(nx_.pkt_off + oi_); nlen_ = *gp(nx_.pkt_len + oi_); bpre_ = true; }");
+                E.line("    if (nbt_ == bt_) { if (oni_ != NO_PKT) { noff_ = *gp(bpo_ + oni_); nlen_ = *gp(bpl_ + oni_); } }");
+                E.line("    else if (oni_ != NO_PKT) { const BatchRef &nx_ = obr_[nbt_]; noff_ = *gp(nx_.pkt_off + oni_); nlen_ = *gp(nx_.pkt_len + oni_); }");
             }
             else if (spread_on) E.line("    { const uint32_t n_ = i + 256u; if (n_ < bhi_) { noff_ = *gp(kp.pkt_off + n_); nlen_ = *gp(kp.pkt_len + n_); } }");
             else E.line("    { const uint32_t n_ = pkt_next(kp, i, j + 1, ex_begin, ex_count); if (n_ != NO_PKT) { noff_ = *gp(kp.pkt_off + n_); nlen_ = *gp(kp.pkt_len + n_); } }");
         }
+        if (spread_own) {
+            E.line("    otf_ = tn_ + 4u;");
+            E.line("    if (odl_ && oln_ == 0u) otf_ = atomicInc(&otk_, 0xffffffffu);");
+            E.line("    if (i != NO_PKT) {");
+        }
         E.line("    const KParams &kq_ = kp;");
         if (spread_own) {
-            E.line("    { const uint32_t ol_ = ochk_ ? i / oP_ : olane_;");
-            E.line("      srow_ = ol_ - blockIdx.x * oR_;");
-            E.line("      L.cpu = (int32_t)(ocpu_ - olane_ + ol_);");
+            E.line("    { srow_ = own_flat_row(og_, (tc_ - bt_ * o4q_) * 64u + oln_);");
+            E.line("      L.cpu = (int32_t)(ocpu_ + srow_);");
             E.line("      sbase_ = SM_.backing_addr + (uint32_t)L.cpu * SM_.addr_period; }");
         } else if (spread_on) {
             E.line("    { if (kp.sched == SCHED_CHUNKED) lam_ = i / kp.per_lane;");
@@ -513,10 +516,10 @@
             }
             if (pf) {
                 E.line("    const uint32_t len = plen_;");
-                E.line("    L.pkt = %s + poff_;", spread_own ? "br_.pkt_data" : "kq_.pkt_data");
+                E.line("    L.pkt = %s + poff_;", spread_own ? "bpd_" : "kq_.pkt_data");
             } else if (spread_own) {
-                E.line("    const uint32_t len = *gp(br_.pkt_len + i);");
-                E.line("    L.pkt = br_.pkt_data + *gp(br_.pkt_off + i);");
+                E.line("    const uint32_t len = *gp(bpl_ + i);");
+                E.line("    L.pkt = bpd_ + *gp(bpo_ + i);");
             } else {
                 E.line("    const uint32_t len = *gp(kq_.pkt_len + i);");
                 E.line("    L.pkt = kq_.pkt_data + *gp(kq_.pkt_off + i);");
@@ -587,7 +590,7 @@
         E.line("    {");
         {
             const char *rb = spread_own ? "lb_" : "kq_";
-            if (spread_own) E.line("    const BatchRef &lb_ = obr_[bt_];");
+            if (spread_own) E.line("    const BatchRef &lb_ = obr_[obx_];");
             if (ntres) {
                 E.line("    if (%s.r0) st_nt(%s.r0 + i, r0);", rb, rb);
                 E.line("    if (%s.status) st_nt(%s.status + i, (uint8_t)st_);", rb, rb);
@@ -607,8 +610,17 @@
             E.line("      S_->pc = epc_; S_->prog = pg_; S_->steps = steps; S_->status = st_; S_->started = 1u; S_->finished = 1u; }");
         }
         E.line("    lane_steps += steps;");
+        if (spread_own) {
+            E.line("    } else {");
+            if (pf) E.line("      poff_ = noff_; plen_ = nlen_; asm volatile(\"\" : \"+v\"(poff_), \"+v\"(plen_));");
+            E.line("    }");
+            E.line("    { const uint32_t cb_ = __builtin_amdgcn_readfirstlane(obx_), xb_ = own_task_batch(__builtin_amdgcn_readfirstlane(otn_), omag_);");
+            E.line("      if (xb_ != cb_ && xb_ < nb_) { const BatchRef nx_ = cget(kp.many, xb_); bpd_ = nx_.pkt_data; bpo_ = nx_.pkt_off; bpl_ = nx_.pkt_len; } }");
+            
+            E.line("    otc_ = otn_; otn_ = __builtin_amdgcn_readfirstlane(otf_);");
+            E.line("    asm volatile(\"\" : \"+v\"(otc_), \"+v\"(otn_));");
+        }
         E.line("  }");
-        if (spread_own) E.line("  }   // batches");
         if (vc_on) E.line("  VC_FLUSH();");
         if (spread_own) {
             E.line("  __syncthreads();");
@@ -2006,6 +2018,7 @@
         info->defer = g.defer_mode;
         info->spread = g.spread_on;
         info->spread_own = g.spread_own;
+        info->own_deal = g.own_deal_ok;
         info->hash_combine = g.hash_combine;
         info->hash_chunk = g.hash_chunk;
         info->proc = proc;
diff --git a/mimic_amd/csrc/jit.h b/mimic_amd/csrc/jit.h
--- a/mimic_amd/csrc/jit.h
+++ b/mimic_amd/csrc/jit.h
@@ -16,6 +16,7 @@
     bool defer;
     bool spread;
     bool spread_own;
+    bool own_deal;
     bool hash_combine;
     bool hash_chunk;
     bool proc, proc_ok;
diff --git a/mimic_amd/csrc/layout.h b/mimic_amd/csrc/layout.h
--- a/mimic_amd/csrc/layout.h
+++ b/mimic_amd/csrc/layout.h
@@ -193,7 +193,7 @@
     struct DeferRec *defer;
     uint32_t *defer_any;
     uint32_t defer_epoch;
-    uint32_t reserved0;
+    uint32_t own_deal;
     uint32_t *spread_bad;
     const void *skb_custom;
     const uint64_t *skb_drv;
@@ -211,8 +211,38 @@
     uint32_t *skb_rooms_state;
 };
 static_assert(sizeof(KParams) == 968, "KParams: the kernarg layout of every JIT kernel");
-static_assert(__builtin_offsetof(KParams, reserved0) == 356 && __builtin_offsetof(KParams, spread_bad) == 360,
-              "KParams: the fields around the reserved word keep their offsets");
+static_assert(__builtin_offsetof(KParams, own_deal) == 356 && __builtin_offsetof(KParams, spread_bad) == 360,
+              "KParams: the fields around the once reserved word keep their offsets");
+
+struct OwnGeo {
+    uint32_t sched, n, cpu_lanes, sched_shift;
+    uint32_t P, R, rsh;
+};
+#define OWN_NO_PKT 0xffffffffu
+HHD_LAYOUT OwnGeo own_geo(uint32_t sched, uint32_t n, uint32_t cpu_lanes, uint32_t sched_shift, uint32_t P, uint32_t Q) {
+    OwnGeo g{sched, n, cpu_lanes, sched_shift, P, 256u / (P / Q), 32u};
+    if ((g.R & (g.R - 1u)) == 0u) g.rsh = (uint32_t)__builtin_ctz(g.R);
+    return g;
+}
+HHD_LAYOUT uint32_t own_magic(uint32_t tasks_per_batch) { return 0xffffffffu / tasks_per_batch + 1u; }
+HHD_LAYOUT uint32_t own_task_batch(uint32_t tau, uint32_t magic) { return (uint32_t)(((uint64_t)tau * magic) >> 32); }
+HHD_LAYOUT uint32_t own_flat_row(const OwnGeo &g, uint32_t flat) {
+    if (g.sched == SCHED_CHUNKED) return flat / g.P;
+    return g.rsh < 32u ? flat & (g.R - 1u) : flat % g.R;
+}
+HHD_LAYOUT uint32_t own_task_pkt(const OwnGeo &g, uint32_t block, uint32_t rem, uint32_t lane) {
+    const uint32_t flat = rem * 64u + lane;
+    if (g.sched == SCHED_CHUNKED) {
+        const uint64_t i = (uint64_t)block * g.R * g.P + flat;
+        return flat < g.R * g.P && i < g.n ? (uint32_t)i : OWN_NO_PKT;
+    }
+    const uint32_t jj = g.rsh < 32u ? flat >> g.rsh : flat / g.R;
+    const uint32_t ol = block * g.R + own_flat_row(g, flat);
+    if (jj >= g.P || ol >= g.cpu_lanes) return OWN_NO_PKT;
+    const uint32_t sh = ol >= g.sched_shift ? ol - g.sched_shift : ol + g.cpu_lanes - g.sched_shift;
+    const uint64_t i = (uint64_t)jj * g.cpu_lanes + sh;
+    return i < g.n ? (uint32_t)i : OWN_NO_PKT;
+}
 
 struct DeferRec {
     uint64_t r[11];
diff --git a/mimic_amd/jit.py b/mimic_amd/jit.py
--- a/mimic_amd/jit.py
+++ b/mimic_amd/jit.py
@@ -91,6 +91,20 @@
     buf = C.create_string_buffer(n + 1)
     lib.mimic_jit_source_spread(arr, ns, len(raws), pca, len(pc), sha, len(shapes), lds_rows, C.byref(ok), buf, n + 1)
     return buf.value.decode(), bool(ok.value)
+
+
+def own_deal_allowed(raws: Sequence[bytes], pc, shapes, lds_rows: int) -> bool:
+    lib = _lib.load()
+    keep, arr, ns = _progs_args(raws)
+    pcf = [v for t in pc for v in t]
+    shf = [v for t in shapes for v in t]
+    pca = (C.c_uint32 * max(len(pcf), 1))(*pcf)
+    sha = (C.c_uint32 * max(len(shf), 1))(*shf)
+    ok = C.c_int32()
+    n = lib.mimic_jit_source_spread(arr, ns, len(raws), pca, len(pc), sha, len(shapes), lds_rows, C.byref(ok), None, 0)
+    if n < 0:
+        raise ValueError(f"cannot decode programs ({n})")
+    return bool(ok.value & 2)
 
 
 def code_object(src: str) -> bytes:
diff --git a/mimic_amd/vm.py b/mimic_amd/vm.py
--- a/mimic_amd/vm.py
+++ b/mimic_amd/vm.py
@@ -703,6 +703,9 @@
     def LastExec(self) -> str:
         return {0: "none", 1: "interp", 2: "jit", 3: "spread", 4: "spread_own"}[self.lib.mimic_last_exec(self.h)]
 
+    def LastOwnDeal(self) -> bool:
+        return self.lib.mimic_last_own_deal(self.h) == 1
+
     def SetSpread(self, mode: int) -> None:
         _check(self.h, self.lib.mimic_set_spread(self.h, mode), "SetSpread")
 
```

Result: no change. 61070 Mpkts/s (-0.0%).
